# deepsphere/deepsphere-cosmo-tf2

Hardware: AMD Instinct MI355X
Metric: Mpix*channels/s Chebyshev-conv fwd, nside=1024 K=5 F=64; HBM roofline % (higher is better)
Workload: dtype f32 (recurrence f32; contraction 3-pass split-bf16 MFMA with f32 accumulate; precision 'bf16x3' = the layer default for 64 input channels)

## Files before the change

deepsphere-cosmo-tf2_amd/csrc/cheb_fused.hip:

```cpp
#include <stdio.h>
#include <stdlib.h>
#include <string.h>

#include <algorithm>

#include "cheb_istrip_kernel.h"
#include "cheb_tiles.h"

namespace dsph {

void fused_images_begin(const dsph_plan* plan, const void* ws, uint64_t key, bool keep) {
  FusedPlan* fp = plan->fused;
  if (!fp || !ws) return;
  std::lock_guard<std::mutex> lock(fp->img_mu);
  if (fp->images.size() > 16384 && fp->images.find(ws) == fp->images.end()) fp->images.clear();
  FusedPlan::Images& im = fp->images[ws];
  if (!keep || im.key != key) { im.key = key; im.mask = 0; }
}
bool fused_images_claim(const dsph_plan* plan, const void* ws, uint32_t bit) {
  FusedPlan* fp = plan->fused;
  if (!fp || !ws) return true;
  std::lock_guard<std::mutex> lock(fp->img_mu);
  auto it = fp->images.find(ws);
  if (it == fp->images.end()) return true;
  if (it->second.mask & bit) return false;
  it->second.mask |= bit;
  return true;
}
void fused_images_forget(const dsph_plan* plan, const void* ws) {
  FusedPlan* fp = plan->fused;
  if (!fp || !ws) return;
  std::lock_guard<std::mutex> lock(fp->img_mu);
  fp->images.erase(ws);
}
uint64_t fused_images_key(int32_t Fin, int32_t Fin_w, int32_t Fout, int32_t K, int32_t ld, int32_t precision, bool cheb, bool many, bool pack) {
  return ((uint64_t)(Fin & 0xfff)) | ((uint64_t)(Fin_w & 0xfff) << 12) | ((uint64_t)(Fout & 0xff) << 24) | ((uint64_t)(K & 0x3f) << 32) |
         ((uint64_t)(ld & 0xffff) << 38) | ((uint64_t)(precision & 3) << 54) | ((uint64_t)cheb << 56) | ((uint64_t)many << 57) |
         ((uint64_t)pack << 58) | (1ull << 63);
}

static bool side_stream_ready(const dsph_plan* plan, FusedPlan* fp, hipStream_t caller, bool may_create) {
  if (fp->side) return true;
  if (fp->side_failed || !may_create) return false;
  if (caller != nullptr) {
    hipStreamCaptureStatus cs = hipStreamCaptureStatusNone;
    if (hipStreamIsCapturing(caller, &cs) != hipSuccess || cs != hipStreamCaptureStatusNone) return false;
  }
  DeviceGuard guard(plan->device);
  hipStream_t st = nullptr;
  hipEvent_t e0 = nullptr, e1 = nullptr;
  if (!guard.ok || hipStreamCreateWithFlags(&st, hipStreamNonBlocking) != hipSuccess) { fp->side_failed = true; return false; }
  if (hipEventCreateWithFlags(&e0, hipEventDisableTiming) != hipSuccess ||
      hipEventCreateWithFlags(&e1, hipEventDisableTiming) != hipSuccess) {
    if (e0) (void)hipEventDestroy(e0);
    (void)hipStreamDestroy(st);
    fp->side_failed = true;
    return false;
  }
  fp->ev_fork = e0;
  fp->ev_join = e1;
  fp->side = st;
  return true;
}

static int plane_rows_for(int rmax, int emax, int wt) {
  if (rmax <= 576 && emax <= 512) return 576;
  if (rmax <= 768 && emax <= 768) return 768;
  if (rmax <= 928 && emax <= 928) return 928;
  if (rmax <= 1024 && emax <= 1024) return 1024;
  return (rmax <= 1168 && emax <= 1024 && wt == 9) ? 1168 : 0;
}

static int bfs_packs(int32_t Fin, int32_t Fout) { return Fin == 4 && Fout <= 16 ? 4 : (Fin == 8 && Fout <= 32 ? 2 : 0); }

struct WeightImages {
  size_t bfs = 0, structured, strip, istrip, qstrip, qstrip8, total;
  size_t bfs_bytes;
  WeightImages(int32_t Fin, int32_t Fout, int32_t K) {
    const int C = (Fin + FUSED_CH - 1) / FUSED_CH, NB = bfs_packs(Fin, Fout) ? 2 : (Fout + 31) / 32;
    bfs_bytes = (size_t)K * C * NB * 2048;
    structured = bfs + bfs_bytes;
    strip = structured + struct_wfrag_bytes(Fin, Fout, K);
    istrip = strip + strip_wimg_bytes(Fin, Fout, K);
    qstrip = istrip + 2 * istrip_wimg_bytes(K, DSPH_PREC_BF16X6);
    qstrip8 = qstrip + (qstrip_shape_ok(Fin, Fout, K) ? qstrip_wimg_bytes() : 0);
    total = qstrip8 + (qstrip8_shape_ok(Fin, Fout, K) ? qstrip8_wimg_bytes() : 0);
  }
};

struct LayerWorkspace {
  size_t block, padded_x, total;
  LayerWorkspace(const dsph_plan* plan, int64_t N, int32_t Fin, int32_t Fout, int32_t K) {
    const int32_t Fp = pad4(Fin);
    block = WeightImages(Fp, std::min(Fout, 64), K).total;
    padded_x = (size_t)((Fout + 63) / 64) * block;
    total = padded_x + (Fp != Fin ? (size_t)N * (size_t)plan->n_cols * (size_t)Fp * 4 : 0);
  }
};
size_t fused_workspace_bytes(const dsph_plan* plan, int64_t N, int32_t Fin, int32_t Fout, int32_t K, int32_t) {
  return LayerWorkspace(plan, N, Fin, Fout, K).total;
}

static bool want_full(const dsph_plan* plan, int32_t Fin, bool full) {
  return full || (uint64_t)plan->n_cols * (uint64_t)Fin * 4ull >= (1ull << 32);
}
static bool has_struct_tiles(const FusedTiles& ft) { return ft.r.n + ft.t.tiles.n > 0; }

static const FusedTiles* tiles_for(const dsph_plan* plan, int32_t Fin, int32_t Fout, int32_t K, bool full) {
  if (!plan->fused || plan->fused->wide) return nullptr;
  if (K < 2 || K - 1 > FUSED_DMAX) return nullptr;
  if (Fin % 4 != 0 || Fin < 4 || Fout < 1) return nullptr;
  const FusedTiles& ft = get_tiles(plan, K - 1, want_full(plan, Fin, full));
  if (!ft.ok) return nullptr;
  if (has_struct_tiles(ft) && !struct_shape_ok(Fin, std::min(Fout, 64), K)) return nullptr;
  if (ft.part.n == 0) return &ft;
  const int pr = plane_rows_for(ft.rmax, ft.emax, ft.width);
  if (pr == 0) return nullptr;
  return (size_t)2 * pr * FUSED_CH * 4 + FUSED_BIAS_BYTES <= (size_t)LDS_BYTES ? &ft : nullptr;
}

int fused_dmax() { return FUSED_DMAX; }
int fused_num_cu(const dsph_plan* plan) { return plan->fused ? plan->fused->num_cu : 256; }

bool fused_tstep_tables(const dsph_plan* plan, TStepTables* out) {
  if (!plan->fused || !plan->fused->wide || plan->n_cols != plan->n_rows || !plan->levels.empty()) return false;
  const FusedTiles& ft = get_tiles(plan, 1, true);
  if (!ft.ok || ft.rmax > 768 || ft.part.n != ft.ntiles) return false;
  out->tile_off = ft.d_tile_off;
  out->ring_end = ft.d_ring_end;
  out->ell_off = ft.d_ell_off;
  out->region = ft.d_region;
  out->lcols = ft.d_lcols;
  out->lvals = ft.d_lvals;
  out->ntiles = ft.ntiles;
  out->width = ft.width;
  return true;
}

bool fused_supported(const dsph_plan* plan, int32_t Fin, int32_t Fout, int32_t K) {
  return Fin >= 1 && tiles_for(plan, pad4(Fin), Fout, K, false) != nullptr;
}

bool fused_weights_resident(const dsph_plan* plan, int32_t Fin, int32_t Fout, int32_t K) {
  const FusedTiles* ft = Fin >= 1 ? tiles_for(plan, pad4(Fin), Fout, K, false) : nullptr;
  if (!ft) return false;
  if (ft->part.n == 0) return true;
  const int pr = plane_rows_for(ft->rmax, ft->emax, ft->width);
  return (size_t)2 * pr * FUSED_CH * 4 + WeightImages(pad4(Fin), std::min(Fout, 64), K).bfs_bytes + FUSED_BIAS_BYTES <= (size_t)LDS_BYTES;
}

int fused_prepare(const dsph_plan* plan, int32_t K, int32_t Fin, int32_t flags) {
  FusedPlan* fp = plan->fused;
  if (fp && fp->wide) {
    TStepTables tb;
    if (K >= 2) (void)fused_tstep_tables(plan, &tb);
  } else {
    if (!fp || K < 2 || K - 1 > FUSED_DMAX) return DSPH_OK;
    const FusedTiles& ftp = get_tiles(plan, K - 1, want_full(plan, pad4(std::max(Fin, 1)), false));
    if (ftp.ok && plan->opt.fork && has_struct_tiles(ftp) && ftp.part.n > 0) {
      std::lock_guard<std::mutex> lock(fp->fork_mu);
      (void)side_stream_ready(plan, fp, nullptr, true);
    }
    if (flags & DSPH_PREPARE_BACKWARD) {
      (void)get_tiles(plan, K - 1, true);
      (void)fused_symmetric(plan);
    }
  }
  if (flags & DSPH_PREPARE_RELEASE_HOST) {
    std::lock_guard<std::mutex> lock(fp->mu);
    std::vector<int32_t>().swap(fp->h_cols);
    std::vector<float>().swap(fp->h_vals);
    fp->host_released = true;
  }
  return DSPH_OK;
}


enum class Mode { forward, planes, wgrad };
enum class Strips { none, pairs, quad, input };

struct FusedRequest {
  Mode mode = Mode::forward;
  int64_t N = 1;
  int32_t Fin = 0;
  int32_t Fin_w = 0;
  int32_t Fout = 0;
  int32_t ld = 0;
  int32_t K = 0, precision = DSPH_PREC_BF16X3, act = DSPH_ACT_NONE, part = 0;
  float alpha_rest = 2.f, beta_rest = 1.f;
  const FusedPool* pool = nullptr;
  const TileList* only_tiles = nullptr;
  const dsph_plan* plan = nullptr;
  const float* x = nullptr; const float* w = nullptr; const float* bias = nullptr; float* y = nullptr;
  unsigned char* ws = nullptr;
  hipStream_t stream = nullptr;
};

struct Route {
  const FusedTiles& ft;
  bool has_struct, has_bfs;
  Strips strips;
  bool run_strips;
  const TileList* r;
  const TileTables* t;
  bool q8;
  const int32_t* bfs_tiles;
  int bfs_n;
  int pack;
  int pr;
};

static bool use_qstrips(const dsph_plan* plan, const FusedTiles& ft, const FusedRequest& q) {
  return plan->opt.strip_form == 0 && ft.q5.n > 0 && qstrip_shape_ok(q.Fin, q.Fout, q.K);
}
static bool strips_apply(const dsph_plan* plan, const FusedTiles& ft, const FusedRequest& q, bool quad) {
  if (!((quad || ft.n_pairs > 0) && (q.precision == DSPH_PREC_BF16X3 || (q.precision == DSPH_PREC_F16X3 && quad)) &&
        strip_shape_ok(q.Fin, q.Fout, q.K) && q.ld % 4 == 0 && plan->n_cols * (int64_t)std::max(q.Fin, q.ld) * 4 < (1ll << 32)))
    return false;
  if (ft.strip_forced) return true;
  FusedPlan* fp = plan->fused;
  const int64_t N = q.N;
  if (quad) {
    if (N < 1) return false;
    const int64_t span = qstrip_split(fp->num_cu, ft.q5.tape_rows, N, ft.q5.tape_rows / std::max(1, ft.q5.n), nullptr, nullptr, nullptr);
    return span * 28 * 103 < ft.q5.n_tiles * N * 187 / fp->num_cu * 100;
  }
  const std::vector<int32_t>& steps = ft.strip_steps;
  if (N < 1 || (int64_t)steps.size() * N > (1ll << 24)) return false;
  int64_t span;
  {
    std::lock_guard<std::mutex> lock(fp->mu);
    auto it = ft.strip_span.find(N);
    if (it == ft.strip_span.end()) it = ft.strip_span.emplace(N, strip_makespan(steps, N, fp->num_cu)).first;
    span = it->second;
  }
  return span * 30 * 103 < ft.n_strip_tiles * N * 187 / fp->num_cu * 100;
}

static bool q8_applies(const dsph_plan* plan, const FusedTiles& ft, const FusedRequest& q) {
  if (ft.q8.n == 0 || !qstrip8_shape_ok(q.Fin, q.Fout, q.K) || (q.precision != DSPH_PREC_BF16X3 && q.precision != DSPH_PREC_F16X3) ||
      q.ld != q.Fout || q.N < 1)
    return false;
  if (plan->opt.strips == 1) return true;
  const int64_t span = qstrip8_split(plan->fused->num_cu, ft.q8.tape_rows, q.N, ft.q8.tape_rows / std::max(1, ft.q8.n), nullptr, nullptr, nullptr);
  return span * 26 * 103 < ft.q8.n_tiles * q.N * 275 / plan->fused->num_cu * 100;
}

static bool istrips_apply(const dsph_plan* plan, const FusedTiles& ft, const FusedRequest& q) {
  return ft.n_ipairs > 0 && plan->opt.strips != 2 && istrip_shape_ok(q.Fin, q.K) && q.Fout % 4 == 0 && q.ld % 4 == 0;
}
static int istrip_nseg(const dsph_plan* plan, const FusedTiles& ft, int64_t N, int D, bool narrow) {
  FusedPlan* fp = plan->fused;
  std::lock_guard<std::mutex> lock(fp->mu);
  const int64_t key = 2 * N + (narrow ? 1 : 0);
  auto it = ft.iseg.find(key);
  if (it == ft.iseg.end()) it = ft.iseg.emplace(key, istrip_segments(ft.ipair_h, ft.ipair_second, N, fp->num_cu, D, narrow)).first;
  return it->second;
}

static Route make_route(const dsph_plan* plan, const FusedTiles& ft, const FusedRequest& q, bool forked) {
  const bool fwd = q.mode == Mode::forward, y_aligned = (reinterpret_cast<uintptr_t>(q.y) & 15) == 0;
  const bool plain_epilogue = q.act == DSPH_ACT_NONE || q.act == DSPH_ACT_RELU;
  Route rt{ft};
  rt.has_struct = fwd && has_struct_tiles(ft);
  rt.has_bfs = ft.part.count(q.part) > 0;
  const bool quad = use_qstrips(plan, ft, q);
  rt.strips = Strips::none;
  if (fwd && strips_apply(plan, ft, q, quad) && q.Fin_w == q.Fin && y_aligned) rt.strips = quad ? Strips::quad : Strips::pairs;
  else if (fwd && istrips_apply(plan, ft, q) && y_aligned) rt.strips = Strips::input;
  rt.run_strips = rt.strips != Strips::none && q.part != 2;
  rt.r = rt.strips == Strips::quad ? &ft.qrrest : (rt.strips != Strips::none ? &ft.rrest : &ft.r);
  rt.t = rt.strips == Strips::quad ? &ft.qt : &ft.t;
  rt.q8 = fwd && q.part != 2 && !q.pool && !forked && q.Fin_w == q.Fin && q.beta_rest != 0.f && plain_epilogue && y_aligned && q8_applies(plan, ft, q);
  rt.bfs_tiles = q.part == 0 && ft.part.n == ft.ntiles ? nullptr : ft.part.ptr(q.part);
  rt.bfs_n = ft.part.count(q.part);
  if (rt.q8) {
    rt.bfs_tiles = ft.q8rest.ptr(q.part);
    rt.bfs_n = ft.q8rest.count(q.part);
  }
  if (q.only_tiles) {
    rt.bfs_tiles = q.only_tiles->d;
    rt.bfs_n = q.only_tiles->n;
  }
  rt.pack = (plan->opt.pack && fwd && q.N >= 2) ? bfs_packs(q.Fin, q.Fout) : 0;
  rt.pr = plane_rows_for(ft.rmax, ft.emax, ft.width);
  return rt;
}

bool fused_pool_ok(const dsph_plan* plan, int64_t N, int32_t Fin, int32_t Fout, int32_t K, int32_t act) {
  if (!plan->fused || N < 1 || !(act == DSPH_ACT_NONE || act == DSPH_ACT_RELU)) return false;
  if (!plan->levels.empty() || plan->n_cols != plan->n_rows || plan->n_rows % FUSED_P != 0 || K < 2 || K - 1 > FUSED_DMAX) return false;
  const FusedTiles* ft = Fin >= 1 ? tiles_for(plan, pad4(Fin), Fout, K, false) : nullptr;
  if (!ft || Fout % 4 != 0) return false;
  FusedRequest q;
  q.N = N; q.Fin = q.Fin_w = pad4(Fin); q.Fout = std::min(Fout, 64); q.ld = Fout; q.K = K; q.precision = DSPH_PREC_BF16X3;
  const Strips s = make_route(plan, *ft, q, false).strips;
  return s != Strips::pairs && s != Strips::quad;
}

int64_t fused_strip_tiles(const dsph_plan* plan, int64_t N, int32_t Fin, int32_t Fout, int32_t K, int32_t precision) {
  if (!plan->fused || K < 2 || K - 1 > FUSED_DMAX) return 0;
  const FusedTiles& ft = get_tiles(plan, K - 1, want_full(plan, pad4(Fin), false));
  if (!ft.ok) return 0;
  FusedRequest q;
  q.N = N; q.Fin = pad4(Fin); q.Fin_w = Fin; q.Fout = std::min(Fout, 64); q.ld = Fout; q.K = K; q.precision = precision;
  const Route rt = make_route(plan, ft, q, false);
  if (rt.q8) return ft.q8.n_tiles;
  return rt.strips == Strips::quad ? ft.q5.n_tiles : (rt.strips != Strips::none ? ft.n_strip_tiles : 0);
}


__global__ __launch_bounds__(256) void fused_pad_kernel(const float* __restrict__ x, float4* __restrict__ out, int64_t rows,
                                                        int Fin, int Q) {
  for (int64_t i = (int64_t)blockIdx.x * 256 + threadIdx.x; i < rows * Q; i += (int64_t)gridDim.x * 256) {
    const int64_t r = i / Q;
    const int c = 4 * (int)(i - r * Q);
    const float* __restrict__ src = x + r * Fin + c;
    float4 v;
    v.x = src[0];
    v.y = c + 1 < Fin ? src[1] : 0.f;
    v.z = c + 2 < Fin ? src[2] : 0.f;
    v.w = c + 3 < Fin ? src[3] : 0.f;
    out[i] = v;
  }
}

__global__ __launch_bounds__(256) void fused_wprep_kernel(const float* __restrict__ w,
                                                          unsigned char* __restrict__ out, int Fin,
                                                          int Fout, int K, int C, int NB, int prec, int ld, int pack) {
  const int blk = blockIdx.x;
  const int nb = blk % NB, c = (blk / NB) % C, k = blk / (NB * C);
  for (int e = threadIdx.x; e < WF_ELEMS; e += 256) {
    const WfElem p = wf_elem32(e);
    wf_put(out + (size_t)blk * 2 * WF_FRAG, prec == DSPH_PREC_BF16X3 ? WF_BF16X3 : WF_FP32_STEPS, p.l, p.j,
           wf_gather_pack(w, c * FUSED_CH + p.inner, 32 * nb + p.col, Fin, Fout, K, k, ld, pack));
  }
}

__global__ __launch_bounds__(256) void fused_wgrad_reduce_kernel(const float* __restrict__ slabs, float* __restrict__ dw,
                                                                 int nslabs, int Fin, int Fout, int K, int C, int ld, int mirror_grid) {
  __shared__ float part[16][17];
  const int el = threadIdx.x & 15, p = threadIdx.x >> 4;
  const int e = blockIdx.x * 16 + el;
  const bool live = e < Fin * K * Fout;
  const int o = live ? e % Fout : 0, fk = live ? e / Fout : 0, k = fk % K, f = fk / K;
  const size_t slab = (size_t)C * K * 16 * 64;
  const size_t off = ((size_t)((f >> 4) * K + k) * 16 + (f & 15)) * 64 + o;
  float s = 0.f;
  if (live)
    for (int i = p; i < nslabs; i += 16) {
      const float v = slabs[(size_t)i * slab + off];
      s += (mirror_grid > 0 && (((i >> 1) % mirror_grid) & 1)) ? -v : v;
    }
  part[p][el] = s;
  __syncthreads();
  if (p == 0 && live) {
    float v[16];
#pragma unroll
    for (int q = 0; q < 16; ++q) v[q] = part[q][el];
#pragma unroll
    for (int h = 8; h >= 1; h >>= 1)
#pragma unroll
      for (int q = 0; q < h; ++q) v[q] += v[q + h];
    dw[(size_t)fk * ld + o] = v[0];
  }
}

int launch_fused_pad(const float* x, float* xp, int64_t rows, int32_t Fin, int32_t Fp, hipStream_t stream) {
  const int64_t work = rows * (Fp / 4);
  hipLaunchKernelGGL(fused_pad_kernel, dim3((unsigned)std::min<int64_t>((work + 255) / 256, 65536)), dim3(256), 0, stream, x,
                     reinterpret_cast<float4*>(xp), rows, (int)Fin, (int)(Fp / 4));
  DSPH_HIP(hipGetLastError());
  return DSPH_OK;
}


static int32_t struct_arithmetic(int32_t precision) { return precision == DSPH_PREC_F16X3 ? DSPH_PREC_BF16X6 : precision; }
static int32_t bfs_arithmetic(int32_t precision) {
  return struct_arithmetic(precision) == DSPH_PREC_BF16X6 ? DSPH_PREC_FP32 : precision;
}

static int check_request(const FusedRequest& rq, const FusedTiles* ft, size_t ws_bytes, size_t ws_need, const void* out) {
  if (!ft) {
    set_error("cheb_fused: plan/shape not supported");
    return DSPH_E_UNSUPPORTED;
  }
  if (ws_need > 0 && (!rq.ws || ws_bytes < ws_need)) {
    set_error("cheb_fused: workspace %zu < %zu", ws_bytes, ws_need);
    return DSPH_E_WORKSPACE;
  }
  if ((reinterpret_cast<uintptr_t>(rq.x) & 15) || (reinterpret_cast<uintptr_t>(rq.ws) & 15) || (reinterpret_cast<uintptr_t>(out) & 15)) {
    set_error("cheb_fused: x, workspace and planes must be 16-byte aligned");
    return DSPH_E_BADARG;
  }
  return DSPH_OK;
}

static LaunchBase launch_base(const FusedRequest& rq) {
  LaunchBase b;
  b.x = rq.x; b.w = rq.w; b.bias = rq.bias; b.y = rq.y;
  b.gvals8 = rq.plan->fused->d_gvals8;
  b.gdiag = rq.plan->fused->d_gdiag;
  b.x_rows = rq.plan->n_cols; b.y_rows = out_rows(rq.plan); b.N = rq.N;
  b.act = rq.act; b.ld = rq.ld; b.num_cu = rq.plan->fused->num_cu;
  b.cheb = rq.beta_rest != 0.f;
  if (rq.pool != nullptr) {
    b.pool = rq.pool->type;
    b.ypool = rq.pool->y;
    b.ypool_rows = rq.plan->n_rows / 4;
  }
  return b;
}

static int launch_strips(const FusedRequest& rq, const Route& rt, const WeightImages& img, const LaunchBase& base) {
  const dsph_plan* plan = rq.plan;
  const FusedTiles& ft = rt.ft;
  if (rt.strips == Strips::quad) {
    QStripLaunch qs;
    static_cast<LaunchBase&>(qs) = base;
    qs.wimg = rq.ws + img.qstrip;
    qs.strips = ft.q5.d_strips;
    qs.tab = ft.q5.d_tab;
    qs.prefix = ft.q5.d_prefix;
    qs.tape_rows = ft.q5.tape_rows;
    qs.nstrips = ft.q5.n; qs.Fin = rq.Fin; qs.Fout = rq.Fout;
    qs.f16 = rq.precision == DSPH_PREC_F16X3;
    qs.f16_xexp = plan->opt.f16_xexp;
    qs.prep_weights = fused_images_claim(plan, rq.ws, IMG_QSTRIP);
    return launch_cheb_qstrip(qs, rq.stream);
  }
  if (rt.strips == Strips::pairs) {
    StripLaunch st;
    static_cast<LaunchBase&>(st) = base;
    st.wimg = rq.ws + img.strip;
    st.pairs = ft.d_pairs;
    st.npairs = ft.n_pairs; st.Fin = rq.Fin; st.Fout = rq.Fout; st.K = rq.K; st.precision = struct_arithmetic(rq.precision);
    st.prep_weights = fused_images_claim(plan, rq.ws, IMG_STRIP);
    return launch_cheb_strip(st, rq.stream);
  }
  IStripLaunch is;
  static_cast<LaunchBase&>(is) = base;
  is.wimg = rq.ws + img.istrip;
  is.pairs = ft.d_ipairs;
  is.npairs = ft.n_ipairs; is.Fin = rq.Fin; is.Fin_w = rq.Fin_w; is.Fout = rq.Fout; is.K = rq.K; is.precision = struct_arithmetic(rq.precision);
  is.nseg = istrip_nseg(plan, ft, istrip_pairs(rq.Fin_w, rq.Fout) ? (rq.N + 1) / 2 : rq.N, rq.K - 1, istrip_narrow(rq.Fin_w));
  is.prep_weights = fused_images_claim(plan, rq.ws, IMG_ISTRIP);
  return launch_cheb_istrip(is, rq.stream);
}

static int forward_structured(const FusedRequest& rq, const Route& rt, const WeightImages& img) {
  const dsph_plan* plan = rq.plan;
  const LaunchBase base = launch_base(rq);
  if (rt.run_strips) {
    const int rc = launch_strips(rq, rt, img, base);
    if (rc != DSPH_OK) return rc;
  }
  StructLaunch sl;
  static_cast<LaunchBase&>(sl) = base;
  sl.wfrag = rq.ws + img.structured;
  sl.Fin = rq.Fin; sl.Fin_w = rq.Fin_w; sl.Fout = rq.Fout; sl.K = rq.K; sl.precision = struct_arithmetic(rq.precision);
  sl.allow_pack = plan->opt.pack;
  bool struct_prep = true;
  if (rt.r->count(rq.part) > 0) {
    sl.tiles = rt.r->ptr(rq.part);
    sl.ntiles = rt.r->count(rq.part);
    sl.prep_weights = fused_images_claim(plan, rq.ws, IMG_STRUCT);
    struct_prep = false;
    const int rc = launch_cheb_struct(sl, rq.stream);
    if (rc != DSPH_OK) return rc;
  }
  if (rt.t->tiles.count(rq.part) > 0) {
    sl.tiles = rt.t->tiles.ptr(rq.part);
    sl.tabrow = rt.t->rows(rq.part);
    sl.tabvals = rt.t->vals(rq.part);
    sl.ntiles = rt.t->tiles.count(rq.part);
    sl.prep_weights = struct_prep && fused_images_claim(plan, rq.ws, IMG_STRUCT);
    const int rc = launch_cheb_struct(sl, rq.stream);
    if (rc != DSPH_OK) return rc;
  }
  return DSPH_OK;
}

static int fused_grid(const dsph_plan* plan, int ntiles) { return std::max(8, std::min(plan->fused->num_cu, (ntiles + 7) / 8 * 8)); }

static FusedArgs fused_args(const FusedRequest& rq, const Route& rt) {
  const dsph_plan* plan = rq.plan;
  const FusedTiles& ft = rt.ft;
  const int C = (rq.Fin + FUSED_CH - 1) / FUSED_CH;
  FusedArgs args{};
  args.c_count = C;
  args.prow_stride = plan->n_cols;
  args.plane_stride = rq.N * plan->n_cols * (int64_t)rq.Fin;
  args.x = rq.x;
  args.bias = rq.bias;
  args.y = rq.y;
  args.wfrag = rq.ws;
  args.tile_off = ft.d_tile_off;
  args.ring_end = ft.d_ring_end;
  args.ell_off = ft.d_ell_off;
  args.region = ft.d_region;
  args.lcols = ft.d_lcols;
  args.lvals = ft.d_lvals;
  args.x_rows = plan->n_cols;
  args.y_rows = out_rows(plan);
  args.N = rt.pack ? (int)((rq.N + rt.pack - 1) / rt.pack) : (int)rq.N;
  args.n_maps = (int)rq.N;
  args.pack = rt.pack;
  args.num_cu = plan->fused->num_cu;
  args.pool = rq.pool ? rq.pool->type : 0;
  args.ypool = rq.pool ? rq.pool->y : nullptr;
  args.ypool_rows = plan->n_rows / 4;
  args.Fin = rq.Fin;
  args.Fout = rq.Fout;
  args.ld = rq.ld;
  args.K = rq.K;
  args.tile_list = rt.bfs_tiles;
  args.ntiles = rt.bfs_n;
  args.nchunks = C;
  args.act = rq.act;
  args.alpha_rest = rq.alpha_rest;
  args.beta_rest = rq.beta_rest;
  return args;
}

static int launch_fused_variant(int pr, int wt, const FusedArgs& a, int nb, int prec, int grid, size_t lds, hipStream_t stream) {
#define DSPH_FUSED_CASE(PR, WT) \
  if (pr == PR && wt == WT) return launch_fused_##PR##_##WT(a, nb, prec, grid, lds, stream);
  DSPH_FUSED_CASE(576, 9)
  DSPH_FUSED_CASE(768, 9)
  DSPH_FUSED_CASE(928, 9)
  DSPH_FUSED_CASE(1024, 9)
  DSPH_FUSED_CASE(1168, 9)
  DSPH_FUSED_CASE(576, 12)
  DSPH_FUSED_CASE(768, 12)
  DSPH_FUSED_CASE(928, 12)
  DSPH_FUSED_CASE(1024, 12)
#undef DSPH_FUSED_CASE
  set_error("cheb_fused: no kernel for plane rows %d, width %d", pr, wt);
  return DSPH_E_UNSUPPORTED;
}

static int launch_bfs_tiles(const FusedRequest& rq, const Route& rt, FusedArgs& args, int nb, size_t wfrag_bytes) {
  if (args.ntiles == 0) return DSPH_OK;
  args.wfrag_bytes = (int)wfrag_bytes;
  const size_t lds = (size_t)2 * rt.pr * FUSED_CH * 4 + wfrag_bytes;
  return launch_fused_variant(rt.pr, rt.ft.width, args, nb, bfs_arithmetic(rq.precision), fused_grid(rq.plan, args.ntiles), lds, rq.stream);
}

static int forward_bfs(const FusedRequest& rq, const Route& rt, const WeightImages& img) {
  const dsph_plan* plan = rq.plan;
  const int C = (rq.Fin + FUSED_CH - 1) / FUSED_CH;
  const int NB = rt.pack ? 2 : (rq.Fout + 31) / 32;
  if (fused_images_claim(plan, rq.ws, IMG_BFS)) {
    hipLaunchKernelGGL(fused_wprep_kernel, dim3(rq.K * C * NB), dim3(256), 0, rq.stream, rq.w, rq.ws + img.bfs, (int)rq.Fin_w, (int)rq.Fout,
                       (int)rq.K, C, NB, (int)bfs_arithmetic(rq.precision), (int)rq.ld, rt.pack);
    DSPH_HIP(hipGetLastError());
  }
  if (rt.q8) {
    QStrip8Launch q;
    static_cast<LaunchBase&>(q) = launch_base(rq);
    q.wimg = rq.ws + img.qstrip8;
    q.strips = rt.ft.q8.d_strips; q.tab = rt.ft.q8.d_tab; q.prefix = rt.ft.q8.d_prefix; q.tape_rows = rt.ft.q8.tape_rows;
    q.nstrips = rt.ft.q8.n; q.ld_w = rq.ld;
    q.f16 = rq.precision == DSPH_PREC_F16X3;
    q.f16_xexp = plan->opt.f16_xexp;
    q.prep_weights = fused_images_claim(plan, rq.ws, IMG_Q8);
    const int rc = launch_cheb_qstrip8(q, rq.stream);
    if (rc != DSPH_OK) return rc;
  }
  FusedArgs args = fused_args(rq, rt);
  return launch_bfs_tiles(rq, rt, args, NB, img.bfs_bytes);
}

static int forward_block(const FusedRequest& rq, const FusedTiles* ft, size_t ws_bytes) {
  const WeightImages img(rq.Fin, rq.Fout, rq.K);
  const int rc = check_request(rq, ft, ws_bytes, img.total, nullptr);
  if (rc != DSPH_OK) return rc;
  const Route rt = make_route(rq.plan, *ft, rq, false);
  if (rt.has_struct) {
    const int rc_s = forward_structured(rq, rt, img);
// ... 251 lines not shown
```

deepsphere-cosmo-tf2_amd/csrc/cheb_qstrip.hip:

```cpp
#include <math.h>
#include <stdio.h>
#include <stdlib.h>

#include <algorithm>
#include <vector>

#include "cheb_qstrip_kernel.h"
#include "dsphere_wfrag.h"

namespace dsph {

__global__ __launch_bounds__(256) void qstrip_wprep_kernel(const float* __restrict__ w, unsigned char* __restrict__ out, int Fin,
                                                           int Fout, int cheb, int ld, int f16) {
  constexpr int K = 5;
  const int blk = blockIdx.x;
  const int kb = blk & 1, lev = (blk >> 1) % 3, oq = ((blk >> 1) / 3) & 3, role = (blk >> 1) / 12;
  const int j = role == 0 ? K - 1 - lev : 1 - lev;
  const bool have = role == 0 || lev < 2;
  float sc = qs_wsign(cheb != 0, j) * ((cheb != 0 && j == 0) ? 2.f : 1.f);
  if (f16) {
    const float pw = qt_wimg_pow2(w, Fin * K, Fout, ld);
    sc *= pw;
    if (blk == 0 && threadIdx.x == 0) *reinterpret_cast<float*>(out + (size_t)2 * 4 * 3 * 2 * 2 * QS_FRAG) = 1.f / pw;
  }
  unsigned char* base = out + (size_t)blk * 2 * QS_FRAG;
  for (int e = threadIdx.x; e < WF_ELEMS; e += 256) {
    const WfElem p = wf_elem16(e);
    wf_put(base, f16 ? WF_F16X3 : WF_BF16X3, p.l, p.j, have ? wf_gather(w, 32 * kb + p.inner, 16 * oq + p.col, Fin, Fout, K, j, ld, sc) : 0.f);
  }
}

bool qstrip_shape_ok(int32_t Fin, int32_t Fout, int32_t K) { return K == 5 && Fin == 64 && Fout == 64; }

int64_t qtape_split(int num_cu, int64_t tape_rows, int64_t N, int64_t mean_height, int run_in, int* grid, int* pieces, int* wg_per_piece) {
  const int g = (int)std::max<int64_t>(8, std::min<int64_t>(num_cu / 8 * 8, tape_rows * N / 64 / 8 * 8));
  auto span_of = [&](int64_t w) {
    const int64_t P = std::max<int64_t>(1, g / w), share = (tape_rows + P - 1) / P, maps = (N + w - 1) / w;
    const int64_t runs = share / std::max<int64_t>(1, mean_height) + 2;
    return (share + runs * (run_in + 1)) * maps;
  };
  int64_t best_w = 1, best = -1;
  if (N <= g) { best_w = N; best = span_of(N); }
  else
    for (int64_t w = 1; w <= g; w *= 2) {
      const int64_t sp = span_of(w);
      if (best < 0 || sp < best) { best = sp; best_w = w; }
    }
  if (grid) *grid = g;
  if (pieces) *pieces = (int)std::max<int64_t>(1, g / best_w);
  if (wg_per_piece) *wg_per_piece = (int)best_w;
  return best;
}
int64_t qstrip_split(int num_cu, int64_t tape_rows, int64_t N, int64_t mean_height, int* grid, int* pieces, int* wg_per_piece) {
  return qtape_split(num_cu, tape_rows, N, mean_height, QS_RUNIN, grid, pieces, wg_per_piece);
}

size_t qstrip_wimg_bytes() { return (size_t)2 * 4 * 3 * 2 * 2 * QS_FRAG + 256; }

int launch_cheb_qstrip(const QStripLaunch& s, hipStream_t stream) {
  if (s.prep_weights) {
    hipLaunchKernelGGL(qstrip_wprep_kernel, dim3(2 * 4 * 3 * 2), dim3(256), 0, stream, s.w, s.wimg, (int)s.Fin, (int)s.Fout, s.cheb ? 1 : 0,
                       (int)s.ld, s.f16 ? 1 : 0);
    DSPH_HIP(hipGetLastError());
  }
  QStripArgs a;
  a.Fin = s.Fin;
  a.Fout = s.Fout;
  const int grid = qtape_forward_args(a, s, QS_RUNIN);
  void (*kern)(QStripArgs) = s.f16 ? (s.cheb ? cheb_qstrip5_kernel<true, true> : cheb_qstrip5_kernel<false, true>)
                                   : (s.cheb ? cheb_qstrip5_kernel<true, false> : cheb_qstrip5_kernel<false, false>);
#ifdef DSPH_QS_STAMPS
  static unsigned* d_stamps = nullptr;
  constexpr size_t NST = 8 * 4 * 10;
  if (!d_stamps) DSPH_HIP(hipMalloc(&d_stamps, NST * 4));
  DSPH_HIP(hipMemsetAsync(d_stamps, 0, NST * 4, stream));
  a.stamps = d_stamps;
#endif
  hipLaunchKernelGGL(kern, dim3(grid), dim3(QS_THREADS), 0, stream, a);
  DSPH_HIP(hipGetLastError());
#ifdef DSPH_QS_STAMPS
  if (getenv("DSPH_STAMPS_DUMP")) {
    std::vector<unsigned> h(NST);
    if (hipStreamSynchronize(stream) == hipSuccess && hipMemcpy(h.data(), d_stamps, NST * 4, hipMemcpyDeviceToHost) == hipSuccess)
      for (int w = 0; w < 8; ++w)
        for (int it = 0; it < 4; ++it) {
          const unsigned* r = &h[((size_t)w * 4 + it) * 10];
          fprintf(stderr, "QSSTAMP wave %d step %2d:", w, it);
          unsigned prev = r[0];
          for (int i = 1; i <= 8; ++i) {
            if (r[i] == 0) { fprintf(stderr, "      -"); continue; }
            fprintf(stderr, " %6u", r[i] - prev);
            prev = r[i];
          }
          fprintf(stderr, " | step %u | t0 %u\n", r[8] - r[0], r[0]);
        }
  }
#endif
  return DSPH_OK;
}

}
```

deepsphere-cosmo-tf2_amd/csrc/cheb_qstrip_kernel.h:

```cpp
#pragma once

#include <type_traits>

#include "cheb_qtape.h"

namespace dsph {

constexpr int QS_PX = 64;
constexpr int QS_D = 4;
constexpr int QS_USE = QS_PX - 2 * QS_D;
constexpr int QS_THREADS = 512;
constexpr int QS_RUNIN = 2 * QS_D + 1;

struct QStripArgs {
  const float* x;
  const float* bias;
  float* y;
  const unsigned char* wimg;
  const float* gvals8;
  const float* gdiag;
  const QStrip* strips;
  const int32_t* tab;
  const int32_t* prefix;
  int64_t x_rows, y_rows;
  int nstrips, N, Fin, Fout, ld, act;
  int pieces, wg_per_piece;
  float xsc, xsc_inv;
#ifdef DSPH_QS_STAMPS
  unsigned* stamps;
#endif
};

#ifdef DSPH_QS_STAMPS
#define QS_STAMP(id)                                                                                          \
  do {                                                                                                        \
    if (stamp_on) {                                                                                           \
      unsigned long long t_;                                                                                  \
      asm volatile("s_memtime %0\n\ts_waitcnt lgkmcnt(0)" : "=s"(t_)::"memory");                              \
      if (lane == 0) a.stamps[(wave * 4 + (stamp_step & 3)) * 10 + (id)] = (unsigned)t_;                      \
    }                                                                                                         \
  } while (0)
#define QS_STAMP_DECL                                                                                         \
  const int stamp_step = ytop - (st.y0 - D) - 60;                                                             \
  const bool stamp_on = blockIdx.x == 72 && stamp_step >= 0 && stamp_step < 4;
#else
#define QS_STAMP(id)
#define QS_STAMP_DECL
#endif

#ifdef DSPH_QS_ABL
#define QS_ABL DSPH_QS_ABL
#else
#define QS_ABL 0
#endif

#if QS_ABL & 64
#define QS_FD "v_fmac_f32_e32 "
#define QS_DPPL "\n\t"
#define QS_DPPR "\n\t"
#else
#define QS_FD "v_fmac_f32_dpp "
#define QS_DPPL " row_shr:1 row_mask:0xf bank_mask:0xf bound_ctrl:1\n\t"
#define QS_DPPR " row_shl:1 row_mask:0xf bank_mask:0xf bound_ctrl:1\n\t"
#endif

template <bool F16> __device__ __forceinline__ void qs_m(qs_f4& acc, const qs_bf8& wa, const qs_bf8& bb) {
  if (QS_ABL & 2) { asm volatile("" : "+v"(acc) : "v"(wa), "v"(bb) : "memory"); return; }
  if (F16) asm volatile("v_mfma_f32_16x16x32_f16 %0, %1, %2, %0" : "+v"(acc) : "v"(wa), "v"(bb) : "memory");
  else asm volatile("v_mfma_f32_16x16x32_bf16 %0, %1, %2, %0" : "+v"(acc) : "v"(wa), "v"(bb) : "memory");
}
template <bool F16> __device__ __forceinline__ void qs_m0(qs_f4& acc, const qs_bf8& wa, const qs_bf8& bb) {
  if (QS_ABL & 2) { acc = qs_f4{0.f, 0.f, 0.f, 0.f}; asm volatile("" : "+v"(acc) : "v"(wa), "v"(bb) : "memory"); return; }
  if (F16) asm volatile("v_mfma_f32_16x16x32_f16 %0, %1, %2, 0" : "=&v"(acc) : "v"(wa), "v"(bb) : "memory");
  else asm volatile("v_mfma_f32_16x16x32_bf16 %0, %1, %2, 0" : "=&v"(acc) : "v"(wa), "v"(bb) : "memory");
}
template <int N> __device__ __forceinline__ void qs_settle(QRow& r) {
  if (N == 9) asm volatile("s_nop 9" : "+v"(r.t[0]), "+v"(r.t[1]), "+v"(r.t[2]), "+v"(r.t[3]) : : "memory");
  else asm volatile("s_nop 1" : "+v"(r.t[0]), "+v"(r.t[1]), "+v"(r.t[2]), "+v"(r.t[3]) : : "memory");
}

template <bool INIT, bool NEG>
__device__ __forceinline__ void qs_u12(float& a0, float& a1, float& a2, float& a3, float s0, float s1, float s2, float s3,
                                       const qs_f4& cw, const qs_f4& cc, const qs_f4& ce) {
  if ((QS_ABL & 64) && NEG) { qs_u12<INIT, false>(a0, a1, a2, a3, s0, s1, s2, s3, cw, cc, ce); return; }
  const float w0 = cw[0], w1 = cw[1], w2 = cw[2], w3 = cw[3], c0 = cc[0], c1 = cc[1], c2 = cc[2], c3 = cc[3], e0 = ce[0], e1 = ce[1],
              e2 = ce[2], e3 = ce[3];
#define QS_OPS_IN "v"(s0), "v"(s1), "v"(s2), "v"(s3), "v"(w0), "v"(w1), "v"(w2), "v"(w3), "v"(c0), "v"(c1), "v"(c2), "v"(c3), "v"(e0), "v"(e1), "v"(e2), "v"(e3)
  if (!INIT && !NEG)
    asm volatile(
        "v_fmac_f32_e32 %0, %4, %12\n\tv_fmac_f32_e32 %1, %5, %13\n\tv_fmac_f32_e32 %2, %6, %14\n\tv_fmac_f32_e32 %3, %7, %15\n\t"
        "v_fmac_f32_e32 %1, %4, %9\n\tv_fmac_f32_e32 %2, %5, %10\n\tv_fmac_f32_e32 %3, %6, %11\n\t"
        "v_fmac_f32_e32 %0, %5, %16\n\tv_fmac_f32_e32 %1, %6, %17\n\tv_fmac_f32_e32 %2, %7, %18\n\t"
        QS_FD "%0, %7, %8" QS_DPPL QS_FD "%3, %4, %19" QS_DPPR
        : "+v"(a0), "+v"(a1), "+v"(a2), "+v"(a3)
        : QS_OPS_IN
        : "memory");
  else if (!INIT && NEG)
    asm volatile(
        "v_fma_f32 %0, %4, -%12, %0\n\tv_fma_f32 %1, %5, -%13, %1\n\tv_fma_f32 %2, %6, -%14, %2\n\tv_fma_f32 %3, %7, -%15, %3\n\t"
        "v_fma_f32 %1, %4, -%9, %1\n\tv_fma_f32 %2, %5, -%10, %2\n\tv_fma_f32 %3, %6, -%11, %3\n\t"
        "v_fma_f32 %0, %5, -%16, %0\n\tv_fma_f32 %1, %6, -%17, %1\n\tv_fma_f32 %2, %7, -%18, %2\n\t"
        QS_FD "%0, %7, -%8" QS_DPPL QS_FD "%3, %4, -%19" QS_DPPR
        : "+v"(a0), "+v"(a1), "+v"(a2), "+v"(a3)
        : QS_OPS_IN
        : "memory");
  else if (INIT && !NEG)
    asm volatile(
        "v_mul_f32_e32 %0, %4, %12\n\tv_mul_f32_e32 %1, %5, %13\n\tv_mul_f32_e32 %2, %6, %14\n\tv_mul_f32_e32 %3, %7, %15\n\t"
        "v_fmac_f32_e32 %1, %4, %9\n\tv_fmac_f32_e32 %2, %5, %10\n\tv_fmac_f32_e32 %3, %6, %11\n\t"
        "v_fmac_f32_e32 %0, %5, %16\n\tv_fmac_f32_e32 %1, %6, %17\n\tv_fmac_f32_e32 %2, %7, %18\n\t"
        QS_FD "%0, %7, %8" QS_DPPL QS_FD "%3, %4, %19" QS_DPPR
        : "=&v"(a0), "=&v"(a1), "=&v"(a2), "=&v"(a3)
        : QS_OPS_IN
        : "memory");
  else
    asm volatile(
        "v_mul_f32_e64 %0, %4, -%12\n\tv_mul_f32_e64 %1, %5, -%13\n\tv_mul_f32_e64 %2, %6, -%14\n\tv_mul_f32_e64 %3, %7, -%15\n\t"
        "v_fma_f32 %1, %4, -%9, %1\n\tv_fma_f32 %2, %5, -%10, %2\n\tv_fma_f32 %3, %6, -%11, %3\n\t"
        "v_fma_f32 %0, %5, -%16, %0\n\tv_fma_f32 %1, %6, -%17, %1\n\tv_fma_f32 %2, %7, -%18, %2\n\t"
        QS_FD "%0, %7, -%8" QS_DPPL QS_FD "%3, %4, -%19" QS_DPPR
        : "=&v"(a0), "=&v"(a1), "=&v"(a2), "=&v"(a3)
        : QS_OPS_IN
        : "memory");
#undef QS_OPS_IN
}
template <bool INIT, bool NEG>
__device__ __forceinline__ void qs_unit(QRow& acc, const QRow& src, int e, const qs_f4& cw, const qs_f4& cc, const qs_f4& ce) {
  if ((QS_ABL & 4) && !INIT) {
    asm volatile("" : "+v"(acc.t[0]), "+v"(acc.t[1]), "+v"(acc.t[2]), "+v"(acc.t[3]) : "v"(src.t[0]), "v"(src.t[3]), "v"(cw), "v"(cc), "v"(ce) : "memory");
    return;
  }
#define QS_UE(E)                                                                                                          \
  {                                                                                                                       \
    float a0 = 0.f, a1 = 0.f, a2 = 0.f, a3 = 0.f;                                                                         \
    if (!INIT) { a0 = acc.t[0][E]; a1 = acc.t[1][E]; a2 = acc.t[2][E]; a3 = acc.t[3][E]; }                                \
    qs_u12<INIT, NEG>(a0, a1, a2, a3, src.t[0][E], src.t[1][E], src.t[2][E], src.t[3][E], cw, cc, ce);                    \
    acc.t[0][E] = a0; acc.t[1][E] = a1; acc.t[2][E] = a2; acc.t[3][E] = a3;                                               \
  }
  if (e == 0) QS_UE(0)
  else if (e == 1) QS_UE(1)
  else if (e == 2) QS_UE(2)
  else QS_UE(3)
#undef QS_UE
}

#define QS_UPR 4
#define QS_UNIT qs_unit

__host__ __device__ constexpr float qs_wsign(bool cheb, int j) { return cheb && ((j & 3) >= 2) ? -1.f : 1.f; }

template <bool CHEB, bool F16>
__global__ __launch_bounds__(QS_THREADS, 2) void cheb_qstrip5_kernel(QStripArgs a) {
  constexpr int K = 5, D = QS_D, RING = K + 2;
#ifdef DSPH_QS_NOH1
  constexpr bool H1 = false;
#else
  constexpr bool H1 = CHEB;
#endif
  constexpr int ROWB = 2 * 2 * 4 * QS_FRAG;
  constexpr int RINGB = RING * ROWB;
  constexpr int HAND1 = 2 * 4 * QS_FRAG;
  constexpr int HANDB = 4 * HAND1;
  constexpr int CRING = K + 1;
  constexpr int CRINGB = CRING * QS_CROWB;
  constexpr int LDS_HAND = RINGB, LDS_C = RINGB + HANDB, LDS_FLAG = LDS_C + CRINGB;
  __shared__ __attribute__((aligned(16))) unsigned char smem[LDS_FLAG + 64];

  const int tid = threadIdx.x, lane = tid & 63;
  const int wave = __builtin_amdgcn_readfirstlane(tid >> 6);
  const bool roleL = wave >= 4;
  const int oq = wave & 3;
  const int p = lane & 15, q4 = lane >> 4;
  const unsigned lane16 = (unsigned)lane * 16u;
  const unsigned hand = (unsigned)LDS_HAND + (unsigned)oq * HAND1 + lane16;
  const unsigned flag_addr = (unsigned)LDS_FLAG + 4u * (unsigned)oq;
  auto flag_set = [&](int v) __attribute__((always_inline)) { qt_flag_set(flag_addr, v); };
  auto flag_get = [&]() __attribute__((always_inline)) -> int { return qt_flag_get(flag_addr); };
  for (int i = tid; i < (LDS_FLAG + 64) / 16; i += QS_THREADS) reinterpret_cast<qs_f4*>(smem)[i] = qs_f4{0.f, 0.f, 0.f, 0.f};

  const QTapePiece wg = qt_piece(a.wg_per_piece);
  if (wg.piece >= a.pieces) return;
  const QTapeRange tape = qt_tape_range(a.prefix, a.nstrips, wg.piece, a.pieces);
  auto locate = [&](int64_t r, int64_t r_end, QStrip& st) __attribute__((always_inline)) -> int {
    return qt_locate(a.prefix, a.strips, a.nstrips, r, r_end, st);
  };
  const unsigned xrowb = (unsigned)a.Fin * 4u, yrowb = (unsigned)a.ld * 4u;

#if defined(DSPH_QS_XALL)
  constexpr bool X_BY_H = false;
#elif defined(DSPH_QS_XBYH)
  constexpr bool X_BY_H = true;
#else
  constexpr bool X_BY_H = !H1;
#endif
  constexpr int XN = X_BY_H ? 4 : 2;
  const int xt = wave & 3, xpix = X_BY_H ? ((lane >> 1) & 15) : (((lane >> 1) & 7) + 8 * (wave >> 2));
  const unsigned x_goff = X_BY_H ? (unsigned)(2 * (lane >> 5) + (lane & 1)) * 16u
                                 : (unsigned)(lane >> 5) * 64u + (unsigned)(2 * ((lane >> 4) & 1) + (lane & 1)) * 16u;
  const unsigned x_loff = (unsigned)xt * QS_FRAG + (unsigned)(lane & 1) * 8u +
                          (X_BY_H ? (unsigned)(xpix + 16 * (lane >> 5)) * 16u : (unsigned)(xpix + 16 * (2 * (lane >> 5) + ((lane >> 4) & 1))) * 16u);
  auto tab_lane = [&](const QStrip& st, unsigned ci, int yrow) __attribute__((always_inline)) -> unsigned {
    return qt_tab_lane(a.tab, st, ci, min(max(yrow, st.ylo), st.yhi));
  };
  auto my_of = [&](int yrow) __attribute__((always_inline)) -> unsigned { return st_spread((unsigned)yrow & 15u) << 1; };
  auto my_next = [&](unsigned m) __attribute__((always_inline)) -> unsigned { return ((m | 0x55u) + 1u) & 0xaau; };
  auto xfetch = [&](const char* xmap, unsigned xrow, qs_f4 (&xv)[XN]) __attribute__((always_inline)) {
    if (QS_ABL & 8) {
#pragma unroll
      for (int i = 0; i < XN; ++i) xv[i] = qs_f4{0.f, 0.f, 0.f, 0.f};
      return;
    }
    const char* src = xmap + (size_t)(xrow * xrowb + x_goff);
#pragma unroll
    for (int i = 0; i < XN; ++i) xv[i] = *reinterpret_cast<const qs_f4*>(src + (X_BY_H ? 64 : 128) * i);
  };
  auto xw_wait = [&](qs_f4 (&xv)[XN]) __attribute__((always_inline)) {
    if (X_BY_H) asm volatile("" : "+v"(xv[0]), "+v"(xv[1]), "+v"(xv[XN - 2]), "+v"(xv[XN - 1]) : : "memory");
    else asm volatile("" : "+v"(xv[0]), "+v"(xv[1]) : : "memory");
  };
  auto xstore = [&](int slot, const qs_f4 (&xv)[XN]) __attribute__((always_inline)) {
    if (QS_ABL & 4096) {
#pragma unroll
      for (int i = 0; i < XN; ++i) asm volatile("" : : "v"(xv[i]));
      return;
    }
    unsigned char* q = smem + (unsigned)slot * ROWB + x_loff;
#pragma unroll
    for (int i = 0; i < XN; ++i) {
      const unsigned fo = X_BY_H ? (unsigned)(i >> 1) * (2 * 4 * QS_FRAG) + (unsigned)(i & 1) * (32u * 16u) : (unsigned)i * (2 * 4 * QS_FRAG);
      qs_u2 hi, lo;
#pragma unroll
      for (int j = 0; j < 2; ++j) {
        const float a0 = F16 ? xv[i][2 * j] * a.xsc : xv[i][2 * j], a1 = F16 ? xv[i][2 * j + 1] * a.xsc : xv[i][2 * j + 1];
        const qs_u2 hl = qt_split<F16>(a0, a1);
        hi[j] = hl[0];
        lo[j] = hl[1];
      }
      *reinterpret_cast<qs_u2*>(q + fo) = hi;
      *reinterpret_cast<qs_u2*>(q + fo + 4 * QS_FRAG) = lo;
    }
  };
  auto cfetch = [&](unsigned rid, qs_f4& cv, float& cd) __attribute__((always_inline)) { qt_cfetch(a.gvals8, a.gdiag, rid, q4, cv, cd); };
  auto cw_wait = [&](qs_f4& cv, float& cd) __attribute__((always_inline)) {
    asm volatile("" : "+v"(cv), "+v"(cd) : : "memory");
  };
  auto cstore = [&](int slot, qs_f4 cv, float cd) __attribute__((always_inline)) {
    if (CHEB) { cv = cv + cv; cd = cd + cd; }
    unsigned char* q = smem + LDS_C + (unsigned)slot * QS_CROWB + (unsigned)p * 16u + (unsigned)oq * 4u;
    if (q4 < 2) {
#pragma unroll
      for (int d = 0; d < 4; ++d) *reinterpret_cast<float*>(q + (unsigned)(1 + 4 * q4 + d) * 256u) = cv[d];
    }
    if (q4 == 2) *reinterpret_cast<float*>(q) = cd;
  };
  constexpr bool C_OFF = (QS_ABL & 1024) != 0;
  auto clo_read = [&](int slot) __attribute__((always_inline)) -> QCoefLo { return qt_clo_read<C_OFF>(smem + LDS_C, slot, p); };
  auto chi_read = [&](int slot) __attribute__((always_inline)) -> QCoefHi { return qt_chi_read<C_OFF>(smem + LDS_C, slot, p); };

#if QS_ABL & 512
#define QS_FRLOAD(P) (wr[0][0][0])
#else
#define QS_FRLOAD(P) (*reinterpret_cast<const qs_bf8*>(P))
#endif
#define QS_ORD_A(j) ((j) == 1 ? 1 : 0)
#define QS_ORD_B(j) ((j) == 0 ? 1 : 0)
#define QS_FR0(FADDR)                                                                                                     \
  _Pragma("unroll") for (int u = 0; u < 2; ++u) {                                                                         \
    fr[0][u][0] = QS_FRLOAD(smem + (FADDR) + (unsigned)u * QS_FRAG);                                                      \
    fr[0][u][1] = QS_FRLOAD(smem + (FADDR) + (unsigned)(4 + u) * QS_FRAG);                                                \
  }
#define QS_SETS(S0, S1, ROW, ZERO, WLEV, FADDR, NU, ...)                                                                  \
  _Pragma("unroll") for (int s = (S0); s < (S1); ++s) {                 \
    if (s + 1 < 4) {                                                                                                      \
      _Pragma("unroll") for (int u = 0; u < 2; ++u) {                                                                     \
        const unsigned fo = (unsigned)(((s + 1) >> 1) * 8 + ((s + 1) & 1) * 2 + u) * QS_FRAG;                             \
        fr[(s + 1) & 1][u][0] = QS_FRLOAD(smem + (FADDR) + fo);                                                           \
        fr[(s + 1) & 1][u][1] = QS_FRLOAD(smem + (FADDR) + fo + 4 * QS_FRAG);                                             \
      }                                                                                                                   \
    }                                                                                                                     \
    _Pragma("unroll") for (int j = 0; j < 3; ++j) {                                                                       \
      _Pragma("unroll") for (int u = 0; u < 2; ++u) {                                                                     \
        const int m = (s * 3 + j) * 2 + u;                                                                                \
        const int tt = (s & 1) * 2 + u;                                                                                   \
        const qs_bf8& wa_ = wr[WLEV][s >> 1][QS_ORD_A(j)];                                                                \
        const qs_bf8& bb_ = fr[s & 1][u][QS_ORD_B(j)];                                                                    \
        if ((ZERO) && s < 2 && j == 0) qs_m0<F16>((ROW).t[tt], wa_, bb_);                                                 \
        else qs_m<F16>((ROW).t[tt], wa_, bb_);                                                                            \
        _Pragma("unroll") for (int qq = (m * (NU)) / 18; qq < ((m + 1) * (NU)) / 18 && m < 18; ++qq) { __VA_ARGS__; }     \
      }                                                                                                                   \
    }                                                                                                                     \
  }
#define QS_CHAIN(ROW, ZERO, WLEV, FADDR, NU, TAIL, ...)                                                                   \
  {                                                                                                                       \
    QS_SETS(0, 3, ROW, ZERO, WLEV, FADDR, NU, __VA_ARGS__)                                                                \
    TAIL;                                                                                                                 \
    QS_SETS(3, 4, ROW, ZERO, WLEV, FADDR, NU, __VA_ARGS__)                                                                \
  }

  __syncthreads();

  if (!roleL) {
    qs_bf8 wr[4][2][2];
    if (H1) {
      const unsigned char* wp1 = a.wimg + ((size_t)(1 * 4 + oq) * 3) * (2 * 2 * QS_FRAG) + lane16;
#pragma unroll
      for (int kb = 0; kb < 2; ++kb)
#pragma unroll
        for (int h = 0; h < 2; ++h) wr[3][kb][h] = *reinterpret_cast<const qs_bf8*>(wp1 + (size_t)(kb * 2 + h) * QS_FRAG);
    }
    {
      const unsigned char* wp = a.wimg + ((size_t)(0 * 4 + oq) * 3) * (2 * 2 * QS_FRAG) + lane16;
#pragma unroll
      for (int l = 0; l < 3; ++l)
#pragma unroll
        for (int kb = 0; kb < 2; ++kb)
#pragma unroll
          for (int h = 0; h < 2; ++h) wr[l][kb][h] = *reinterpret_cast<const qs_bf8*>(wp + ((size_t)(l * 2 + kb) * 2 + h) * QS_FRAG);
    }
    int handed = 0;
    for (int64_t tr = tape.begin; tr < tape.end;) {
      QStrip st;
      tr += locate(tr, tape.end, st);
      for (int nq = wg.map0; nq < a.N; nq += a.wg_per_piece) {
      const int Xc = min(max(st.xs + 4 * p + oq, st.xlo), st.xhi);
      const int Xf = min(max(st.xs + 4 * xpix + xt, st.xlo), st.xhi);
      const int tc0 = max(st.xs, st.xlo) >> 4;
      const unsigned ciC = (unsigned)((Xc >> 4) - tc0), mXc = st_spread((unsigned)Xc & 15u);
      const unsigned ciF = (unsigned)((Xf >> 4) - tc0), mXf = st_spread((unsigned)Xf & 15u);
      const int T3 = ((st.y1 - st.y0) + 2 * D + 1 + 3) / 3;
      const char* __restrict__ xmap = reinterpret_cast<const char*>(a.x) + (size_t)nq * a.x_rows * xrowb;
      QRow R[2][3];
#pragma unroll
      for (int i = 0; i < 2; ++i)
#pragma unroll
        for (int s = 0; s < 3; ++s)
#pragma unroll
          for (int t = 0; t < 4; ++t) R[i][s].t[t] = qs_f4{0.f, 0.f, 0.f, 0.f};
      int ytop = st.y0 - D, slot_top = 0, cs_top = 0;
      qt_step_barrier();
      {
        qs_f4 cv, xv[XN];
        float cd;
        cfetch(qt_row_in(st, tab_lane(st, ciC, ytop - 1), mXc, ytop - 1), cv, cd);
        xfetch(xmap, qt_row_in(st, tab_lane(st, ciF, ytop), mXf, ytop), xv);
        cw_wait(cv, cd);
        cstore(CRING - 1, cv, cd);
        xw_wait(xv);
        xstore(0, xv);
      }
      unsigned bXf = tab_lane(st, ciF, ytop + 1), bXc = tab_lane(st, ciC, ytop);
      unsigned myX = my_of(ytop + 1), myC = my_of(ytop);
      qt_step_barrier();
      auto step = [&](auto ph_c) __attribute__((always_inline)) {
        constexpr int PH = decltype(ph_c)::value;
        constexpr int L0 = PH % 3, L1 = (PH + 1) % 3, L2 = (PH + 2) % 3;
        int snew = slot_top + 1;
        snew = snew == RING ? 0 : snew;
        auto slot_ix = [&](int back) __attribute__((always_inline)) -> int {
          int s = slot_top - back;
          s += s < 0 ? RING : 0;
          return s;
        };
        auto cslot_ix = [&](int back) __attribute__((always_inline)) -> int {
          int s = cs_top - back;
          s += s < 0 ? CRING : 0;
          return s;
        };
        QS_STAMP_DECL
        QS_STAMP(0);
        qs_f4 xv[XN];
        constexpr bool XLATE = H1;
        if (myX == 0) bXf = tab_lane(st, ciF, ytop + 1);
        if (myC == 0) bXc = tab_lane(st, ciC, ytop);
        if (!XLATE) xfetch(xmap, bXf + (mXf | myX), xv);
        const unsigned f0 = (unsigned)slot_top * ROWB + lane16, f1 = (unsigned)slot_ix(1) * ROWB + lane16, f2 = (unsigned)slot_ix(2) * ROWB + lane16;
        const unsigned f3 = (unsigned)slot_ix(3) * ROWB + lane16;
        constexpr bool N3 = CHEB;
        qs_bf8 fr[2][2][2];
        QCoefLo c3 = clo_read(cslot_ix(1));
        QS_FR0(f0)
        QCoefLo c2;
        QCoefHi c3h, c2h;
        qs_f4 cv;
        float cd;
        QS_CHAIN(R[0][L2], true, 0, f0, 2 * QS_UPR, { c2 = clo_read(cslot_ix(2)); QS_FR0(f1) },
                 { if (qq < QS_UPR) QS_UNIT<true, N3>(R[1][L2], R[0][L0], qq, QS_LO0(c3)); else QS_UNIT<false, N3>(R[1][L2], R[0][L1], qq - QS_UPR, QS_LO1(c3)); })
        qs_settle<9>(R[0][L2]);
        qs_settle<1>(R[1][L2]);
        QS_STAMP(1);
        QS_CHAIN(R[1][L2], false, 1, f1, 2 * QS_UPR, { c3h = chi_read(cslot_ix(1)); QS_FR0(f2) },
                 { if (qq < QS_UPR) QS_UNIT<!CHEB, false>(R[0][L0], R[1][L0], qq, QS_LO0(c2)); else QS_UNIT<false, false>(R[0][L0], R[1][L1], qq - QS_UPR, QS_LO1(c2)); })
        qs_settle<9>(R[1][L2]);
        qs_settle<1>(R[0][L0]);
        if (XLATE) xfetch(xmap, bXf + (mXf | myX), xv);
        QS_STAMP(2);
        QS_CHAIN(R[0][L0], false, 2, f2, QS_UPR, { c2h = chi_read(cslot_ix(2)); cfetch(bXc + (mXc | myC), cv, cd); if (H1) { QS_FR0(f3) } },
                 { QS_UNIT<false, N3>(R[1][L2], R[0][L2], qq, QS_HI(c3h)); })
        qs_settle<9>(R[0][L0]);
        qs_settle<1>(R[1][L2]);
        QS_STAMP(3);
        if (H1) {
          QS_CHAIN(R[1][L0], false, 3, f3, QS_UPR, {}, { QS_UNIT<false, false>(R[0][L0], R[1][L2], qq, QS_HI(c2h)); })
          qs_settle<9>(R[1][L0]);
        } else {
#pragma unroll
          for (int qq = 0; qq < QS_UPR; ++qq) QS_UNIT<false, false>(R[0][L0], R[1][L2], qq, QS_HI(c2h));
        }
        QS_STAMP(4);
        for (int spin = 0; flag_get() <= handed && spin < (1 << 22); ++spin) {}
        if (!(QS_ABL & 2048)) {
          unsigned char* hp = smem + hand;
#pragma unroll
          for (int t = 0; t < 4; ++t) {
            *reinterpret_cast<qs_f4*>(hp + t * QS_FRAG) = R[0][L0].t[t];
            if (CHEB) *reinterpret_cast<qs_f4*>(hp + (4 + t) * QS_FRAG) = R[1][L0].t[t];
          }
        }
        ++handed;
        QS_STAMP(5);
        xw_wait(xv);
        cw_wait(cv, cd);
        QS_STAMP(6);
        cstore(cs_top, cv, cd);
        xstore(snew, xv);
        QS_STAMP(7);
        slot_top = snew;
        cs_top = cs_top + 1 == CRING ? 0 : cs_top + 1;
        ++ytop;
        myX = my_next(myX);
        myC = my_next(myC);
        qt_step_barrier();
        QS_STAMP(8);
      };
      for (int t3 = 0; t3 < T3; ++t3) {
        step(std::integral_constant<int, 0>{});
        step(std::integral_constant<int, 1>{});
        step(std::integral_constant<int, 2>{});
      }
      }
    }
  } else {
    qs_bf8 wr[2][2][2];
    {
      const unsigned char* wp = a.wimg + ((size_t)(1 * 4 + oq) * 3) * (2 * 2 * QS_FRAG) + lane16;
#pragma unroll
      for (int l = 0; l < 2; ++l)
#pragma unroll
        for (int kb = 0; kb < 2; ++kb)
#pragma unroll
          for (int h = 0; h < 2; ++h) wr[l][kb][h] = *reinterpret_cast<const qs_bf8*>(wp + ((size_t)(l * 2 + kb) * 2 + h) * QS_FRAG);
    }
    const float floor_v = a.act == DSPH_ACT_RELU ? 0.f : -__builtin_huge_valf();
    const float ysc = (CHEB ? 0.5f : 1.f) * (F16 ? *reinterpret_cast<const float*>(a.wimg + 2 * 4 * 3 * 2 * 2 * QS_FRAG) * a.xsc_inv : 1.f);
#ifdef DSPH_QS_LPRIO
#define QS_STR2(x) #x
#define QS_STR(x) QS_STR2(x)
    asm volatile("s_setprio " QS_STR(DSPH_QS_LPRIO));
#endif
    qs_f4 bv = qs_f4{0.f, 0.f, 0.f, 0.f};
    if (a.bias != nullptr) bv = *reinterpret_cast<const qs_f4*>(a.bias + 16 * oq + 4 * q4);
    int taken = 0;
    for (int64_t tr = tape.begin; tr < tape.end;) {
      QStrip st;
      tr += locate(tr, tape.end, st);
      for (int nq = wg.map0; nq < a.N; nq += a.wg_per_piece) {
      const int Xf = min(max(st.xs + 4 * xpix + xt, st.xlo), st.xhi);
      const int tc0 = max(st.xs, st.xlo) >> 4;
      const unsigned ciF = (unsigned)((Xf >> 4) - tc0), mXf = st_spread((unsigned)Xf & 15u);
      const int Xg = st.xs + 4 * p;
      const unsigned ciY = (unsigned)((min(max(Xg, st.xlo), st.xhi) >> 4) - tc0), mXg = st_spread((unsigned)Xg & 12u);
      const int cfirst = st.x0 - st.xs, clast = cfirst + st.w;
      const int T3 = ((st.y1 - st.y0) + 2 * D + 1 + 3) / 3;
      const char* __restrict__ xmap = reinterpret_cast<const char*>(a.x) + (size_t)nq * a.x_rows * xrowb;
      char* __restrict__ ymap = reinterpret_cast<char*>(a.y) + (size_t)nq * a.y_rows * yrowb;
      QRow R[2][3], Y;
#pragma unroll
      for (int i = 0; i < 2; ++i)
#pragma unroll
        for (int s = 0; s < 3; ++s)
#pragma unroll
          for (int t = 0; t < 4; ++t) R[i][s].t[t] = qs_f4{0.f, 0.f, 0.f, 0.f};
#pragma unroll
      for (int t = 0; t < 4; ++t) Y.t[t] = qs_f4{0.f, 0.f, 0.f, 0.f};
      int ytop = st.y0 - D, slot_top = 0, cs_top = 0;
      qt_step_barrier();
      if (!X_BY_H) {
        qs_f4 xv[XN];
        xfetch(xmap, qt_row_in(st, tab_lane(st, ciF, ytop), mXf, ytop), xv);
        xw_wait(xv);
        xstore(0, xv);
      }
      unsigned bXf = X_BY_H ? 0u : tab_lane(st, ciF, ytop + 1), bY = tab_lane(st, ciY, st.y0);
      unsigned myX = my_of(ytop + 1), myY = my_of(ytop - K);
      qt_step_barrier();
      auto step = [&](auto ph_c) __attribute__((always_inline)) {
        constexpr int PH = decltype(ph_c)::value;
        constexpr int L0 = PH % 3, L1 = (PH + 1) % 3, L2 = (PH + 2) % 3;
        int snew = slot_top + 1;
        snew = snew == RING ? 0 : snew;
        auto slot_ix = [&](int back) __attribute__((always_inline)) -> int {
          int s = slot_top - back;
          s += s < 0 ? RING : 0;
          return s;
        };
        auto cslot_ix = [&](int back) __attribute__((always_inline)) -> int {
          int s = cs_top - back;
          s += s < 0 ? CRING : 0;
          return s;
        };
        QS_STAMP_DECL
        QS_STAMP(0);
        qs_f4 xv[XN];
        if (!X_BY_H && myX == 0) bXf = tab_lane(st, ciF, ytop + 1);
        if (myY == 0) bY = tab_lane(st, ciY, ytop - K);
        if (!X_BY_H) xfetch(xmap, bXf + (mXf | myX), xv);
#ifdef DSPH_QS_LEARLY
        constexpr bool LE = CHEB && H1;
#else
        constexpr bool LE = false;
#endif
        QCoefLo c0;
        QCoefHi c0h;
        if (LE) c0 = clo_read(cslot_ix(5));
        if (!(QS_ABL & 2048)) {
          const unsigned char* hp = smem + hand;
#pragma unroll
          for (int t = 0; t < 4; ++t) {
            R[0][L2].t[t] = *reinterpret_cast<const qs_f4*>(hp + t * QS_FRAG);
            if (CHEB) R[1][L2].t[t] = *reinterpret_cast<const qs_f4*>(hp + (4 + t) * QS_FRAG);
          }
        }
        ++taken;
        flag_set(taken);
        const unsigned f1 = (unsigned)slot_ix(4) * ROWB + lane16, f0 = (unsigned)slot_ix(5) * ROWB + lane16;
        constexpr bool N1 = CHEB;
        QS_STAMP(1);
        qs_bf8 fr[2][2][2];
        if (LE) {
#pragma unroll
          for (int t = 0; t < 4; ++t) Y.t[t] = R[0][L0].t[t] + R[0][L0].t[t];
          qs_settle<1>(Y);
#pragma unroll
          for (int qq = 0; qq < 2 * QS_UPR; ++qq) {
            if (qq < QS_UPR) QS_UNIT<false, false>(Y, R[1][L0], qq, QS_LO0(c0)); else QS_UNIT<false, false>(Y, R[1][L1], qq - QS_UPR, QS_LO1(c0));
          }
          qs_settle<1>(Y);
        }
        const QCoefLo c1 = clo_read(cslot_ix(4));
        const QCoefHi c1h = chi_read(cslot_ix(4));
        QS_FR0(f0)
#ifdef DSPH_QS_LBARE
        if (CHEB && H1) {
          c0 = clo_read(cslot_ix(5));
          c0h = chi_read(cslot_ix(5));
#pragma unroll
          for (int qq = 0; qq < 3 * QS_UPR; ++qq) {
            if (qq < QS_UPR) QS_UNIT<false, N1>(R[1][L2], R[0][L0], qq, QS_LO0(c1));
            else if (qq < 2 * QS_UPR) QS_UNIT<false, N1>(R[1][L2], R[0][L1], qq - QS_UPR, QS_LO1(c1));
            else QS_UNIT<false, N1>(R[1][L2], R[0][L2], qq - 2 * QS_UPR, QS_HI(c1h));
          }
#pragma unroll
          for (int t = 0; t < 4; ++t) Y.t[t] = R[0][L0].t[t] + R[0][L0].t[t];
          qs_settle<1>(Y);
#pragma unroll
          for (int qq = 0; qq < 2 * QS_UPR; ++qq) {
            if (qq < QS_UPR) QS_UNIT<false, false>(Y, R[1][L0], qq, QS_LO0(c0)); else QS_UNIT<false, false>(Y, R[1][L1], qq - QS_UPR, QS_LO1(c0));
          }
          qs_settle<1>(R[1][L2]);
#pragma unroll
          for (int qq = 0; qq < QS_UPR; ++qq) QS_UNIT<false, false>(Y, R[1][L2], qq, QS_HI(c0h));
          qs_settle<1>(Y);
          QS_STAMP(2);
          QS_CHAIN(Y, false, 1, f0, 0, {}, {})
          qs_settle<9>(Y);
          QS_STAMP(3);
        } else
// ... 78 lines not shown
```

deepsphere-cosmo-tf2_amd/csrc/cheb_qtape.h:

```cpp
#pragma once

#include <algorithm>

#include "cheb_struct_kernel.h"
#include "dsphere_common.h"

namespace dsph {

constexpr int QS_FRAG = 1024;
constexpr int QS_CROWB = 2304;

typedef float qs_f4 __attribute__((ext_vector_type(4)));
typedef int qs_i4 __attribute__((ext_vector_type(4)));
typedef __bf16 qs_bf8 __attribute__((ext_vector_type(8)));
typedef unsigned qs_u2 __attribute__((ext_vector_type(2)));

struct QRow {
  qs_f4 t[4];
};

struct QStrip {
  int32_t x0, w;
  int32_t xs;
  int32_t y0, y1;
  int32_t xlo, xhi;
  int32_t ylo, yhi;
  int32_t tab, tws;
  int32_t pad[1];
};

struct QTapePiece {
  int ord, piece, map0;
};
__device__ __forceinline__ QTapePiece qt_piece(int wg_per_piece) {
  QTapePiece c;
  const int G = gridDim.x;
  c.ord = (blockIdx.x & 7) * (G >> 3) + (blockIdx.x >> 3);
  c.piece = c.ord / wg_per_piece;
  c.map0 = c.ord - c.piece * wg_per_piece;
  return c;
}
struct QTapeRange {
  int64_t begin, end;
};
__device__ __forceinline__ QTapeRange qt_tape_range(const int32_t* prefix, int nstrips, int piece, int pieces) {
  const int64_t tape = (int64_t)prefix[nstrips];
  QTapeRange r;
  r.begin = piece < pieces ? tape * piece / pieces : 0;
  r.end = piece < pieces ? tape * (piece + 1) / pieces : 0;
  return r;
}
__device__ __forceinline__ int qt_locate(const int32_t* prefix, const QStrip* strips, int nstrips, int64_t r, int64_t r_end, QStrip& st) {
  int lo = 0, hi = nstrips;
  while (hi - lo > 1) {
    const int mid = (lo + hi) >> 1;
    if ((int64_t)prefix[mid] <= r) lo = mid; else hi = mid;
  }
  {
    const QStrip g = strips[lo];
#define QS_U(f) st.f = __builtin_amdgcn_readfirstlane(g.f)
    QS_U(x0); QS_U(w); QS_U(xs); QS_U(y0); QS_U(y1); QS_U(xlo); QS_U(xhi); QS_U(ylo); QS_U(yhi); QS_U(tab); QS_U(tws);
#undef QS_U
  }
  const int h = st.y1 - st.y0;
  const int off = (int)(r - (int64_t)prefix[lo]);
  const int len = (int)(((int64_t)(h - off) < r_end - r) ? (int64_t)(h - off) : r_end - r);
  st.y0 += off;
  st.y1 = st.y0 + len;
  return len;
}

__device__ __forceinline__ unsigned qt_tab_lane(const int32_t* tab, const QStrip& st, unsigned ci, int yc) {
  const int32_t* trow = tab + __builtin_amdgcn_readfirstlane(st.tab + (yc >> 4) * st.tws + (max(st.xs, st.xlo) >> 4));
  qs_i4 b;
  int b4;
  asm volatile("s_load_dwordx4 %0, %2, 0x0\n\ts_load_dword %1, %2, 0x10\n\ts_waitcnt lgkmcnt(0)" : "=&s"(b), "=&s"(b4) : "s"(trow) : "memory");
  return (unsigned)(ci == 0 ? b[0] : ci == 1 ? b[1] : ci == 2 ? b[2] : ci == 3 ? b[3] : b4);
}
__device__ __forceinline__ unsigned qt_row_in(const QStrip& st, unsigned base, unsigned mX, int yrow) {
  const int yc = min(max(yrow, st.ylo), st.yhi);
  return base + (mX | (st_spread((unsigned)yc & 15u) << 1));
}

__device__ __forceinline__ void qt_step_barrier() { asm volatile("s_waitcnt lgkmcnt(0)\n\ts_barrier" ::: "memory"); }
__device__ __forceinline__ void qt_flag_set(unsigned addr, int v) { asm volatile("ds_write_b32 %0, %1" : : "v"(addr), "v"(v) : "memory"); }
__device__ __forceinline__ int qt_flag_get(unsigned addr) {
  int v;
  asm volatile("ds_read_b32 %0, %1\n\ts_waitcnt lgkmcnt(0)" : "=v"(v) : "v"(addr) : "memory");
  return v;
}

template <bool F16> __device__ __forceinline__ qs_u2 qt_split(float a0, float a1) {
  typedef __bf16 bf16x2 __attribute__((ext_vector_type(2)));
  typedef _Float16 f16x2 __attribute__((ext_vector_type(2)));
  typedef float f32x2 __attribute__((ext_vector_type(2)));
  qs_u2 r;
  if (F16) {
    const f16x2 h = __builtin_convertvector(f32x2{a0, a1}, f16x2);
    const f32x2 hf = __builtin_convertvector(h, f32x2);
    const f16x2 l = __builtin_convertvector(f32x2{a0 - hf[0], a1 - hf[1]}, f16x2);
    r[0] = __builtin_bit_cast(unsigned, h);
    r[1] = __builtin_bit_cast(unsigned, l);
  } else {
    const bf16x2 h = __builtin_convertvector(f32x2{a0, a1}, bf16x2);
    const unsigned hu = __builtin_bit_cast(unsigned, h);
    const float h0 = __builtin_bit_cast(float, hu << 16), h1 = __builtin_bit_cast(float, hu & 0xffff0000u);
    const bf16x2 l = __builtin_convertvector(f32x2{a0 - h0, a1 - h1}, bf16x2);
    r[0] = hu;
    r[1] = __builtin_bit_cast(unsigned, l);
  }
  return r;
}

struct QCoef3 {
  qs_f4 w, c, e;
};
struct QCoefLo {
  qs_f4 sw, s, se, w, dg, e;
};
struct QCoefHi {
  qs_f4 nw, n, ne;
};
#define QS_LO0(c) (c).sw, (c).s, (c).se
#define QS_LO1(c) (c).w, (c).dg, (c).e
#define QS_HI(c) (c).nw, (c).n, (c).ne

__device__ __forceinline__ void qt_cfetch(const float* gvals8, const float* gdiag, size_t rid, int q4, qs_f4& cv, float& cd) {
  const char* pv = reinterpret_cast<const char*>(gvals8) + rid * 32u + (unsigned)(q4 & 1) * 16u;
  const char* pd = reinterpret_cast<const char*>(gdiag) + rid * 4u;
  cv = *reinterpret_cast<const qs_f4*>(pv);
  cd = *reinterpret_cast<const float*>(pd);
}
template <bool DOUBLE>
__device__ __forceinline__ void qt_cstore(unsigned char* ring, int slot, int p, int q4, int res, qs_f4 cv, float cd) {
  if (DOUBLE) { cv = cv + cv; cd = cd + cd; }
  unsigned char* q = ring + (unsigned)slot * QS_CROWB + (unsigned)p * 16u + (unsigned)res * 4u;
  if (q4 < 2) {
#pragma unroll
    for (int d = 0; d < 4; ++d) *reinterpret_cast<float*>(q + (unsigned)(1 + 4 * q4 + d) * 256u) = cv[d];
  }
  if (q4 == 2) *reinterpret_cast<float*>(q) = cd;
}
__device__ __forceinline__ const unsigned char* qt_crow(const unsigned char* ring, int slot, int p) {
  return ring + (unsigned)slot * QS_CROWB + (unsigned)p * 16u;
}
template <bool NOREAD = false> __device__ __forceinline__ qs_f4 qt_cvec(const unsigned char* q, int v) {
  if (NOREAD) { qs_f4 c = qs_f4{0.1f, 0.1f, 0.1f, 0.1f}; asm volatile("" : "+v"(c)); return c; }
  return *reinterpret_cast<const qs_f4*>(q + (unsigned)v * 256u);
}
template <bool NOREAD = false> __device__ __forceinline__ QCoef3 qt_cvec3(const unsigned char* q, int which) {
  QCoef3 r;
  if (which == 0) { r.w = qt_cvec<NOREAD>(q, 8); r.c = qt_cvec<NOREAD>(q, 7); r.e = qt_cvec<NOREAD>(q, 6); }
  else if (which == 1) { r.w = qt_cvec<NOREAD>(q, 1); r.c = qt_cvec<NOREAD>(q, 0); r.e = qt_cvec<NOREAD>(q, 5); }
  else { r.w = qt_cvec<NOREAD>(q, 2); r.c = qt_cvec<NOREAD>(q, 3); r.e = qt_cvec<NOREAD>(q, 4); }
  return r;
}
template <bool NOREAD = false> __device__ __forceinline__ QCoefLo qt_clo_read(const unsigned char* ring, int slot, int p) {
  const unsigned char* q = qt_crow(ring, slot, p);
  QCoefLo c;
  c.sw = qt_cvec<NOREAD>(q, 8); c.s = qt_cvec<NOREAD>(q, 7); c.se = qt_cvec<NOREAD>(q, 6);
  c.w = qt_cvec<NOREAD>(q, 1); c.dg = qt_cvec<NOREAD>(q, 0); c.e = qt_cvec<NOREAD>(q, 5);
  return c;
}
template <bool NOREAD = false> __device__ __forceinline__ QCoefHi qt_chi_read(const unsigned char* ring, int slot, int p) {
  const unsigned char* q = qt_crow(ring, slot, p);
  QCoefHi c;
  c.nw = qt_cvec<NOREAD>(q, 2); c.n = qt_cvec<NOREAD>(q, 3); c.ne = qt_cvec<NOREAD>(q, 4);
  return c;
}

__device__ __forceinline__ float qt_wimg_pow2(const float* __restrict__ w, int nrows, int ncols, int ld) {
  __shared__ float smax[256];
  float m = 0.f;
  for (int e = threadIdx.x; e < nrows * ncols; e += 256) m = fmaxf(m, fabsf(w[(int64_t)(e / ncols) * ld + e % ncols]));
  smax[threadIdx.x] = m;
  __syncthreads();
  for (int st = 128; st > 0; st >>= 1) {
    if ((int)threadIdx.x < st) smax[threadIdx.x] = fmaxf(smax[threadIdx.x], smax[threadIdx.x + st]);
    __syncthreads();
  }
  int ex = 0;
  const float mx = smax[0];
  float pw = 1.f;
  if (mx > 0.f && mx < 3.0e38f) { (void)frexpf(mx, &ex); pw = ldexpf(1.f, 12 - ex); }
  return pw;
}

template <class Args, class Launch> int qtape_args(Args& a, const Launch& s, int run_in) {
  a.x = s.x;
  a.gvals8 = s.gvals8;
  a.gdiag = s.gdiag;
  a.strips = s.strips;
  a.tab = s.tab;
  a.prefix = s.prefix;
  a.x_rows = s.x_rows;
  a.nstrips = s.nstrips;
  a.N = (int)s.N;
  int grid;
  (void)qtape_split(s.num_cu, s.tape_rows, s.N, s.tape_rows / std::max(1, s.nstrips), run_in, &grid, &a.pieces, &a.wg_per_piece);
  return grid;
}
template <class Args> int qtape_forward_args(Args& a, const QTapeLaunch& s, int run_in) {
  a.bias = s.bias;
  a.y = s.y;
  a.wimg = s.wimg;
  a.y_rows = s.y_rows;
  a.ld = s.ld;
  a.act = s.act;
  a.xsc = s.f16 ? ldexpf(1.f, s.f16_xexp) : 1.f;
  a.xsc_inv = s.f16 ? ldexpf(1.f, -s.f16_xexp) : 1.f;
  return qtape_args(a, s, run_in);
}

}
```

deepsphere-cosmo-tf2_amd/csrc/cheb_tiles.h:

```cpp
#pragma once

#include <map>
#include <mutex>
#include <unordered_map>
#include <vector>

#include "cheb_fused_kernel.h"
#include "cheb_qstrip8_kernel.h"
#include "cheb_qstrip_kernel.h"
#include "cheb_strip_kernel.h"
#include "cheb_struct_kernel.h"

namespace dsph {

struct TileList {
  int32_t* d = nullptr;
  int n = 0, n_interior = 0;
  const int32_t* ptr(int part) const { return part == 2 ? d + n_interior : d; }
  int count(int part) const { return part == 0 ? n : (part == 1 ? n_interior : n - n_interior); }
};

struct TileTables {
  TileList tiles;
  int32_t* d_row = nullptr;
  float* d_vals = nullptr;
  size_t first(int part) const { return part == 2 ? (size_t)tiles.n_interior : 0; }
  const int32_t* rows(int part) const { return d_row + first(part) * ST_CELLS; }
  const float* vals(int part) const { return d_vals + first(part) * ST_CELLS * ST_TABV; }
};

struct QStripSet {
  QStrip* d_strips = nullptr;
  int32_t* d_prefix = nullptr;
  int32_t* d_tab = nullptr;
  int n = 0;
  int64_t tape_rows = 0;
  int64_t n_tiles = 0;
  std::vector<QStrip> h_strips;
  std::vector<int32_t> h_tab;
};

struct FusedTiles {
  int D = 0;
  int width = 0;
  int ntiles = 0;
  int rmax = 0;
  int emax = 0;
  bool ok = false;
  int32_t* d_tile_off = nullptr;
  int32_t* d_ring_end = nullptr;
  int64_t* d_ell_off = nullptr;
  int32_t* d_region = nullptr;
  uint16_t* d_lcols = nullptr;
  float* d_lvals = nullptr;
  TileList part;
  TileList r;
  TileTables t;
  StripPair* d_pairs = nullptr;
  int n_pairs = 0;
  int64_t n_strip_tiles = 0;
  std::vector<int32_t> strip_steps;
  std::vector<StripPair> h_pairs;
  mutable std::map<int64_t, int64_t> strip_span;
  bool strip_forced = false;
  TileList rrest;
  QStripSet q5;
  TileList qrrest;
  TileTables qt;
  QStripSet q8;
  TileList q8rest;
  StripPair* d_ipairs = nullptr;
  int n_ipairs = 0;
  std::vector<int32_t> ipair_h;
  std::vector<unsigned char> ipair_second;
  mutable std::map<int64_t, int> iseg;
  TileList all;
  TileList nonq;
  std::vector<void*> dev;
  void release();
};

struct FusedPlan {
  std::vector<int32_t> h_cols;
  std::vector<float> h_vals;
  std::mutex mu;
  std::map<int, FusedTiles> by_depth;
  int num_cu = 256;
  float* d_gvals8 = nullptr;
  float* d_gdiag = nullptr;
  unsigned char* d_rowflag = nullptr;
  bool rows_tried = false;
  bool host_released = false;
  int symmetric = -1;
  bool wide = false;
  hipStream_t side = nullptr;
  hipEvent_t ev_fork = nullptr, ev_join = nullptr;
  bool side_failed = false;
  std::mutex fork_mu;
  struct Images { uint64_t key = 0; uint32_t mask = 0; };
  std::mutex img_mu;
  std::unordered_map<const void*, Images> images;
};

const FusedTiles& get_tiles(const dsph_plan* plan, int D, bool full = false);
bool fused_symmetric(const dsph_plan* plan);
int64_t strip_makespan(const std::vector<int32_t>& steps, int64_t N, int num_cu);

}
```

deepsphere-cosmo-tf2_amd/csrc/cheb_tiles.hip:

```cpp
#include <stdio.h>
#include <stdlib.h>
#include <string.h>

#include <algorithm>
#include <initializer_list>

#include "cheb_tiles.h"

namespace dsph {

static const int ddx[8] = {-1, -1, 0, 1, 1, 1, 0, -1}, ddy[8] = {0, 1, 1, 1, 0, -1, -1, -1};

static int template_width(int w) {
  if (w <= 9) return 9;
  if (w <= 12) return 12;
  return 0;
}

void FusedTiles::release() {
  for (void* p : dev) (void)hipFree(p);
  *this = FusedTiles();
}

FusedPlan* fused_plan_build(const dsph_plan* plan, const int32_t* h_cols, const float* h_vals) {
  if (template_width(plan->width) == 0 && tstep_width(plan->width) == 0) return nullptr;
  FusedPlan* fp = new FusedPlan();
  fp->wide = template_width(plan->width) == 0;
  const size_t nnz = (size_t)plan->n_rows * plan->width;
  fp->h_cols.assign(h_cols, h_cols + nnz);
  fp->h_vals.assign(h_vals, h_vals + nnz);
  hipDeviceProp_t prop;
  if (hipGetDeviceProperties(&prop, plan->device) == hipSuccess && prop.multiProcessorCount > 0)
    fp->num_cu = prop.multiProcessorCount;
  return fp;
}

void fused_plan_destroy(FusedPlan* fp) {
  if (!fp) return;
  for (auto& kv : fp->by_depth) kv.second.release();
  if (fp->d_gvals8) (void)hipFree(fp->d_gvals8);
  if (fp->d_gdiag) (void)hipFree(fp->d_gdiag);
  if (fp->d_rowflag) (void)hipFree(fp->d_rowflag);
  if (fp->side) {
    (void)hipStreamSynchronize(fp->side);
    (void)hipEventDestroy(fp->ev_fork);
    (void)hipEventDestroy(fp->ev_join);
    (void)hipStreamDestroy(fp->side);
  }
  delete fp;
}

bool fused_host_released(FusedPlan* fp) {
  std::lock_guard<std::mutex> lock(fp->mu);
  return fp->host_released;
}

void fused_plan_invalidate(FusedPlan* fp) {
  if (!fp) return;
  std::lock_guard<std::mutex> lock(fp->mu);
  for (auto& kv : fp->by_depth) kv.second.release();
  fp->by_depth.clear();
}

static bool embed_tile(const dsph_plan* plan, const int32_t* cols, const float* vals, int W, int t, int D, int64_t out_rows,
                       int32_t* row, float* val, bool* interior, std::vector<int32_t>& key, std::vector<int32_t>& slot) {
  const int64_t r0 = (int64_t)t * FUSED_P;
  if (r0 + FUSED_P > out_rows) return false;
  constexpr int S = ST_S;
  int32_t A[S][S];
  for (int y = 0; y < S; ++y)
    for (int x = 0; x < S; ++x) A[x][y] = -1;
  constexpr int HN = 2048;
  key.assign(HN, -1);
  slot.assign(HN, 0);
  auto hput = [&](int32_t r, int cell) {
    unsigned h = ((unsigned)r * 2654435761u) >> 21;
    while (key[h] != -1) h = (h + 1) & (HN - 1);
    key[h] = r;
    slot[h] = cell;
  };
  auto hget = [&](int32_t r) -> int {
    unsigned h = ((unsigned)r * 2654435761u) >> 21;
    while (key[h] != -1) {
      if (key[h] == r) return slot[h];
      h = (h + 1) & (HN - 1);
    }
    return -1;
  };
  for (unsigned y = 0; y < 16; ++y)
    for (unsigned x = 0; x < 16; ++x) {
      const int32_t r = (int32_t)(r0 + st_morton(x, y));
      A[ST_DMAX + x][ST_DMAX + y] = r;
      hput(r, (ST_DMAX + x) + S * (ST_DMAX + y));
    }
  auto propose = [&](int x, int y) -> int32_t {
    int32_t cand[16];
    int nc = -1;
    for (int dy = -1; dy <= 1; ++dy)
      for (int dx = -1; dx <= 1; ++dx) {
        const int ax = x + dx, ay = y + dy;
        if ((dx == 0 && dy == 0) || ax < 0 || ay < 0 || ax >= S || ay >= S || A[ax][ay] < 0) continue;
        const int32_t ar = A[ax][ay];
        if (ar >= plan->n_rows) continue;
        const int32_t* c = cols + (size_t)ar * W;
        const float* v = vals + (size_t)ar * W;
        if (nc < 0) {
          nc = 0;
          for (int j = 0; j < W; ++j)
            if (v[j] != 0.f && c[j] != ar && hget(c[j]) < 0 && nc < 16) cand[nc++] = c[j];
        } else {
          int m = 0;
          for (int i = 0; i < nc; ++i) {
            bool in = false;
            for (int j = 0; j < W && !in; ++j) in = v[j] != 0.f && c[j] == cand[i];
            if (in) cand[m++] = cand[i];
          }
          nc = m;
        }
      }
    return nc == 1 ? cand[0] : (nc > 1 ? -1 : -2);
  };
  auto place = [&](int x, int y) -> bool {
    const int32_t r = propose(x, y);
    if (r == -1) return false;
    if (r == -2) { A[x][y] = -2; return true; }
    A[x][y] = r;
    hput(r, x + S * y);
    return true;
  };
  for (int rho = 1; rho <= D; ++rho) {
    const int lo = ST_DMAX - rho, hi = ST_DMAX + ST_TILE - 1 + rho;
    const int mid = (lo + hi) / 2;
    for (int k = 0; k <= hi - lo; ++k) {
      const int off = (k + 1) / 2 * ((k & 1) ? 1 : -1);
      const int u = mid + off;
      if (u <= lo || u >= hi) continue;
      if (!place(u, hi) || !place(u, lo) || !place(lo, u) || !place(hi, u)) return false;
    }
    if (!place(lo, lo) || !place(hi, lo) || !place(lo, hi) || !place(hi, hi)) return false;
  }
  const int blo = ST_DMAX - D, bhi = ST_DMAX + ST_TILE - 1 + D;
  for (int p = 0; p < ST_CELLS; ++p) {
    row[p] = (int32_t)r0;
    for (int j = 0; j < ST_TABV; ++j) val[(size_t)p * ST_TABV + j] = 0.f;
  }
  *interior = true;
  for (int y = blo; y <= bhi; ++y)
    for (int x = blo; x <= bhi; ++x) {
      const int32_t r = A[x][y];
      const unsigned p = st_cell_off((unsigned)x, (unsigned)y) / 64u;
      if (r < 0) continue;
      row[p] = r;
      if (r >= out_rows) *interior = false;
      if (x == blo || x == bhi || y == blo || y == bhi) continue;
      if (r >= plan->n_rows) return false;
      const int32_t* c = cols + (size_t)r * W;
      const float* v = vals + (size_t)r * W;
      float* o = val + (size_t)p * ST_TABV;
      unsigned seen = 0;
      for (int j = 0; j < W; ++j) {
        if (v[j] == 0.f) continue;
        int d = -1;
        if (c[j] == r) d = 0;
        else {
          const int cell = hget(c[j]);
          if (cell < 0) return false;
          const int dx = cell % S - x, dy = cell / S - y;
          for (int q = 0; q < 8; ++q)
            if (ddx[q] == dx && ddy[q] == dy) d = q + 1;
          if (d < 0) return false;
        }
        if (seen & (1u << d)) return false;
        seen |= 1u << d;
        o[d] = v[j];
      }
    }
  return true;
}

static int strip_grid(int num_cu, int64_t n_items) { return (int)std::max<int64_t>(8, std::min<int64_t>(num_cu, (n_items + 7) / 8 * 8)); }
int64_t strip_makespan(const std::vector<int32_t>& steps, int64_t N, int num_cu) {
  const int64_t Q = (int64_t)steps.size() * N;
  const int G = strip_grid(num_cu, Q);
  int64_t worst = 0;
  std::vector<int64_t> load;
  for (int xcd = 0; xcd < 8; ++xcd) {
    const int nslots = (G + 7 - xcd) / 8;
    const int64_t q0 = Q * xcd / 8, q1 = Q * (xcd + 1) / 8;
    if (nslots <= 0 || q1 <= q0) continue;
    load.assign((size_t)nslots, 0);
    for (int64_t q = q0; q < q1; ++q) load[(size_t)((q - q0) % nslots)] += steps[(size_t)(q / N)];
    for (int64_t v : load) worst = std::max(worst, v);
  }
  return worst;
}

struct TileRect { int tx, ty, wt, ht; };
static void cut_strip_pairs(const std::vector<TileRect>& take, int D, int h, std::vector<StripPair>& out) {
  out.clear();
  for (const TileRect& r : take) {
    const int X0 = 16 * r.tx, X1 = 16 * (r.tx + r.wt), Y0 = 16 * r.ty, Y1 = 16 * (r.ty + r.ht);
    const int ns = (X1 - X0 + SP_USE - 1) / SP_USE;
    const int H = Y1 - Y0, nseg = (H + h - 1) / h;
    for (int sg = 0; sg < nseg; ++sg) {
      const int ya = Y0 + (int)((int64_t)H * sg / nseg), yb = Y0 + (int)((int64_t)H * (sg + 1) / nseg);
      for (int s0 = 0; s0 < ns; s0 += 2) {
        StripPair p;
        for (int e = 0; e < 2; ++e) {
          const int s = s0 + e;
          if (s < ns) {
            p.x0[e] = X0 + SP_USE * s;
            p.w[e] = std::min(SP_USE, X1 - p.x0[e]);
          } else {
            p.x0[e] = p.x0[0];
// ... 540 lines not shown
      continue;
    }
    if (try_tables && em.run(g, t, D)) {
      (em.interior ? c.t_in : c.t_bd).add(t, em.row.data(), em.val.data());
      continue;
    }
    bool inner = false;
    if (!bfs_tile(g, t, D, WT, wide, b, &inner)) return false;
    (inner ? c.g_in : c.g_bd).push_back(t);
  }
  b.tile_off[g.ntiles] = (int32_t)b.region.size();
  return true;
}

static void merge_small_map(const Graph& g, int D, int num_cu, Embedding& em, Classes& c) {
  if ((c.r_in.empty() && c.r_bd.empty()) ||
      c.r_in.size() + c.r_bd.size() + c.t_in.tiles.size() + c.t_bd.tiles.size() > (size_t)SMALL_MAP_TILES)
    return;
  int64_t taken = 0;
  if (g.plan->opt.strips != 2) {
    std::vector<StripPair> p0, ip0;
    std::vector<int32_t> rest0, steps0;
    build_strips(c.r_in, D, num_cu, g.plan->opt, p0, rest0, &taken, steps0, ip0);
  }
  if (taken != 0) return;
  std::vector<int32_t> keep_i, keep_b;
  for (int pass = 0; pass < 2; ++pass)
    for (int32_t t : pass == 0 ? c.r_in : c.r_bd) {
      if (em.run(g, t, D)) (pass == 0 ? c.t_in : c.t_bd).add(t, em.row.data(), em.val.data());
      else (pass == 0 ? keep_i : keep_b).push_back(t);
    }
  c.r_in.swap(keep_i);
  c.r_bd.swap(keep_b);
}

static void pair_strips(const Graph& g, int D, int num_cu, bool full, const Classes& c, FusedTiles& ft, HostTables& h) {
  std::vector<int32_t> rest = c.r_in;
  ft.strip_forced = g.plan->opt.strips == 1;
  if (!full && D <= SP_DMAX && g.plan->opt.strips != 2)
    build_strips(c.r_in, D, num_cu, g.plan->opt, h.pairs, rest, &ft.n_strip_tiles, ft.strip_steps, h.ipairs);
  h.rrest = joined(std::move(rest), c.r_bd);
  ft.n_pairs = (int)h.pairs.size();
  ft.h_pairs = h.pairs;
  ft.n_ipairs = (int)h.ipairs.size();
  for (const StripPair& ip : h.ipairs) {
    ft.ipair_h.push_back(ip.y1 - ip.y0);
    ft.ipair_second.push_back(ip.w[1] > 0 ? 1 : 0);
  }
}

static QCand morton_cand(int32_t t, int ntiles) {
  QCand c{};
  c.tile = t; c.tix = -1; c.taken = false;
  const int tx = (int)st_compress((unsigned)t), ty = (int)st_compress((unsigned)t >> 1);
  for (int d = 0; d < 8; ++d) {
    const int nx = tx + ddx[d], ny = ty + ddy[d];
    const int64_t nt = nx < 0 || ny < 0 ? -1 : (int64_t)st_morton((unsigned)nx, (unsigned)ny);
    c.nbr[d] = nt >= 0 && nt < ntiles ? (int32_t)nt : -1;
  }
  return c;
}

static void quad_strips5(const Graph& g, int D, const Classes& c, FusedTiles& ft, HostTables& h) {
  std::vector<QCand> cands;
  cands.reserve(c.r_in.size() + c.t_in.tiles.size());
  for (int32_t t : c.r_in) cands.push_back(morton_cand(t, g.ntiles));
  const size_t n_rc = cands.size();
  const int32_t ragged = g.out_rows % FUSED_P != 0 ? g.ntiles - 1 : -1;
  auto beside_ragged = [&](const QCand& q) {
    if (ragged < 0) return false;
    if (q.tile == ragged) return true;
    for (int d = 0; d < 8; ++d)
      if (q.nbr[d] == ragged) return true;
    return false;
  };
  for (size_t i = 0; i < c.t_in.tiles.size(); ++i) {
    QCand q{};
    q.tile = c.t_in.tiles[i]; q.tix = (int32_t)i; q.taken = false;
    if (links_from_table(&c.t_in.rows[i * ST_CELLS], D, g.ntiles, q.nbr)) cands.push_back(q);
  }
  for (QCand& q : cands) q.barred = beside_ragged(q);
  build_qtstrips(cands, g.ntiles, D, ft.q5.h_strips, ft.q5.h_tab, &ft.q5.n_tiles);
  std::vector<int32_t> r_rest;
  std::vector<unsigned char> t_taken(c.t_in.tiles.size(), 0);
  for (size_t i = 0; i < cands.size(); ++i) {
    if (i < n_rc) { if (!cands[i].taken) r_rest.push_back(cands[i].tile); }
    else if (cands[i].taken) t_taken[(size_t)cands[i].tix] = 1;
  }
  h.qrrest = joined(std::move(r_rest), c.r_bd);
  TTabs t_rest;
  for (size_t i = 0; i < c.t_in.tiles.size(); ++i) {
    if (!t_taken[i]) {
      t_rest.add(c.t_in, i);
      continue;
    }
    const int blo = ST_DMAX - D + 1, bhi = ST_DMAX + ST_TILE - 1 + D - 1;
    for (int y = blo; y <= bhi; ++y)
      for (int x = blo; x <= bhi; ++x) {
        const size_t cell = i * ST_CELLS + st_cell_off((unsigned)x, (unsigned)y) / 64u;
        h.patch_rows.push_back(c.t_in.rows[cell]);
        h.patch_vals.insert(h.patch_vals.end(), c.t_in.vals.begin() + cell * ST_TABV, c.t_in.vals.begin() + cell * ST_TABV + 9);
      }
  }
  h.qt = joined(std::move(t_rest), c.t_bd);
}

static void quad_strips8(const Graph& g, int D, const std::vector<unsigned char>& cls8, FusedTiles& ft, HostTables& h) {
  std::vector<QCand> cands;
  for (int32_t t = 0; t < g.ntiles; ++t)
    if ((cls8[(size_t)t] & 3) == 3) cands.push_back(morton_cand(t, g.ntiles));
  build_qtstrips(cands, g.ntiles, D, ft.q8.h_strips, ft.q8.h_tab, &ft.q8.n_tiles);
  std::vector<unsigned char> took((size_t)g.ntiles, 0);
  for (const QCand& q : cands)
    if (q.taken) took[(size_t)q.tile] = 1;
  std::vector<int32_t> rest[2];
  for (size_t i = 0; i < h.part.v.size(); ++i)
    if (!took[(size_t)h.part.v[i]]) rest[i < (size_t)h.part.n_interior ? 0 : 1].push_back(h.part.v[i]);
  h.q8rest = joined(std::move(rest[0]), rest[1]);
}

static std::vector<int32_t> cat(std::initializer_list<const std::vector<int32_t>*> lists) {
  std::vector<int32_t> v;
  for (const std::vector<int32_t>* l : lists) v.insert(v.end(), l->begin(), l->end());
  return v;
}

static void complements(const Classes& c, const FusedTiles& ft, HostTables& h) {
  h.all = joined(cat({&c.r_in, &c.t_in.tiles, &c.g_in}), cat({&c.r_bd, &c.t_bd.tiles, &c.g_bd}));
  h.nonq.v = ft.q5.n_tiles == 0 ? cat({&c.r_in, &c.r_bd, &c.t_in.tiles, &c.t_bd.tiles, &h.part.v}) : cat({&h.qrrest.v, &h.qt.tiles, &h.part.v});
}

template <class T> static bool upload(FusedTiles& ft, T*& dst, std::vector<T>& v) {
  if (v.empty()) v.emplace_back();
  void* p = nullptr;
  if (hipMalloc(&p, v.size() * sizeof(T)) != hipSuccess) return false;
  ft.dev.push_back(p);
  dst = static_cast<T*>(p);
  return hipMemcpy(p, v.data(), v.size() * sizeof(T), hipMemcpyHostToDevice) == hipSuccess;
}
static bool upload(FusedTiles& ft, TileList& dst, HostList& h) {
  dst.n = (int)h.v.size();
  dst.n_interior = h.n_interior;
  return upload(ft, dst.d, h.v);
}
static bool upload(FusedTiles& ft, TileTables& dst, TTabs& h) {
  dst.tiles.n = (int)h.tiles.size();
  dst.tiles.n_interior = h.n_interior;
  return upload(ft, dst.tiles.d, h.tiles) && upload(ft, dst.d_row, h.rows) && upload(ft, dst.d_vals, h.vals);
}
static bool upload(FusedTiles& ft, QStripSet& s) {
  std::vector<QStrip> strips = s.h_strips;
  std::vector<int32_t> prefix(1, 0), tab = s.h_tab;
  for (const QStrip& q : strips) prefix.push_back(prefix.back() + (q.y1 - q.y0));
  s.n = (int)strips.size();
  s.tape_rows = prefix.back();
  tab.resize(tab.size() + 8, 0);
  return upload(ft, s.d_strips, strips) && upload(ft, s.d_prefix, prefix) && upload(ft, s.d_tab, tab);
}
static bool upload_tables(FusedTiles& ft, HostTables& h) {
  BfsTables& b = h.bfs;
  return upload(ft, ft.t, h.t) && upload(ft, ft.d_tile_off, b.tile_off) && upload(ft, ft.d_ring_end, b.ring_end) &&
         upload(ft, ft.d_ell_off, b.ell_off) && upload(ft, ft.d_region, b.region) && upload(ft, ft.d_lcols, b.lcols) &&
         upload(ft, ft.d_lvals, b.lvals) && upload(ft, ft.part, h.part) && upload(ft, ft.r, h.r) && upload(ft, ft.rrest, h.rrest) &&
         upload(ft, ft.nonq, h.nonq) && upload(ft, ft.all, h.all) && upload(ft, ft.d_pairs, h.pairs) && upload(ft, ft.q5) &&
         upload(ft, ft.q8) && upload(ft, ft.q8rest, h.q8rest) && upload(ft, ft.qrrest, h.qrrest) && upload(ft, ft.qt, h.qt) &&
         upload(ft, ft.d_ipairs, h.ipairs);
}

static bool build_tiles(const dsph_plan* plan, FusedPlan* fp, int D, bool full, FusedTiles& ft) {
  const int64_t out_rows = plan->levels.empty() ? plan->n_rows : plan->levels[0];
  const int64_t nt64 = (out_rows + FUSED_P - 1) / FUSED_P;
  if (D < 1 || D > FUSED_DMAX || nt64 > (1 << 30)) return false;
  const Graph g{plan, fp->h_cols.data(), fp->h_vals.data(), plan->width, out_rows, (int)nt64};
  std::vector<unsigned char> cls, cls8;
  classify(g, fp, D, full, cls, cls8);
  const bool try_tables = !full && D <= ST_DMAX && plan->opt.use_struct && plan->opt.use_tables && fp->d_rowflag != nullptr;
  Embedding em;
  Classes c;
  HostTables h;
  if (!sort_tiles(g, D, ft.width, fp->wide, cls, try_tables, em, c, h.bfs)) return false;
  ft.ntiles = g.ntiles;
  ft.rmax = std::max((h.bfs.rmax + 15) / 16 * 16, FUSED_P);
  ft.emax = h.bfs.emax;
  if (try_tables && D <= SP_DMAX) merge_small_map(g, D, fp->num_cu, em, c);
  h.part = joined(c.g_in, c.g_bd);
  pair_strips(g, D, fp->num_cu, full, c, ft, h);
  if (!full && D == QS_D && plan->opt.strips != 2 && plan->opt.strip_form == 0 && fp->d_gvals8 != nullptr)
    quad_strips5(g, D, c, ft, h);
  if (!cls8.empty()) quad_strips8(g, D, cls8, ft, h);
  complements(c, ft, h);
  h.r = joined(c.r_in, c.r_bd);
  h.t = joined(c.t_in, c.t_bd);
  bool good = upload_tables(ft, h);
  if (good && !h.patch_rows.empty())
    good = struct_patch_rows(plan, fp->d_gvals8, fp->d_gdiag, h.patch_rows.data(), h.patch_vals.data(), (int64_t)h.patch_rows.size()) == DSPH_OK;
  if (!good) {
    ft.release();
    ft.D = D;
  }
  return good;
}

const FusedTiles& get_tiles(const dsph_plan* plan, int D, bool full) {
  FusedPlan* fp = plan->fused;
  std::lock_guard<std::mutex> lock(fp->mu);
  DeviceGuard guard(plan->device);
  const int key = 2 * D + (full ? 1 : 0);
  auto it = fp->by_depth.find(key);
  if (it != fp->by_depth.end()) return it->second;
  static const FusedTiles none;
  if (fp->host_released || (fp->wide && !(D == 1 && full))) return none;
  FusedTiles& ft = fp->by_depth[key];
  ft.D = D;
  ft.width = fp->wide ? tstep_width(plan->width) : template_width(plan->width);
  ft.ok = build_tiles(plan, fp, D, full, ft);
  return ft;
}

bool fused_tile_counts(const dsph_plan* plan, int32_t K, int64_t* n_struct, int64_t* n_bfs) {
  if (!plan->fused || K < 2 || K - 1 > FUSED_DMAX) return false;
  const FusedTiles& ft = get_tiles(plan, K - 1, false);
  if (!ft.ok) return false;
  *n_struct = ft.r.n + ft.t.tiles.n;
  *n_bfs = ft.part.n;
  return true;
}

static const QStripSet* record_strips(const dsph_plan* plan, const FusedTiles& ft, int32_t K) {
  const QStripSet* s = K == 5 ? &ft.q5 : (K == Q8_K ? &ft.q8 : nullptr);
  return plan->opt.strip_form == 0 && s && !s->h_strips.empty() ? s : nullptr;
}

int64_t fused_strip_pairs(const dsph_plan* plan, int32_t K, int32_t* out, int64_t cap) {
  if (!plan->fused || K < 2 || K - 1 > FUSED_DMAX) return -1;
  const FusedTiles& ft = get_tiles(plan, K - 1, false);
  if (!ft.ok) return -1;
  static_assert(sizeof(StripPair) == 12 * sizeof(int32_t), "StripPair is twelve int32");
  if (const QStripSet* s = record_strips(plan, ft, K)) {
    const int64_t n = (int64_t)s->h_strips.size();
    for (int64_t i = 0; i < n && i < cap; ++i) {
      const QStrip& q = s->h_strips[(size_t)i];
      const int32_t rec[12] = {q.x0, q.x0, q.w, 0, q.xs, q.xs, q.y0, q.y1, q.xlo, q.xhi, q.ylo, q.yhi};
      memcpy(out + 12 * i, rec, sizeof(rec));
    }
    return n;
  }
  const int64_t n = (int64_t)ft.h_pairs.size();
  for (int64_t i = 0; i < n && i < cap; ++i) memcpy(out + 12 * i, &ft.h_pairs[(size_t)i], sizeof(StripPair));
  return n;
}

int64_t fused_strip_rows(const dsph_plan* plan, int32_t K, int64_t strip, int64_t n, const int32_t* xy, int64_t* rows) {
  if (!plan->fused || K < 2 || K - 1 > FUSED_DMAX) return -1;
  const FusedTiles& ft = get_tiles(plan, K - 1, false);
  if (!ft.ok || strip < 0) return -1;
  if (const QStripSet* s = record_strips(plan, ft, K)) {
    if (strip >= (int64_t)s->h_strips.size()) return -1;
    const QStrip& q = s->h_strips[(size_t)strip];
    const int ya = K == 5 ? q.ylo - 1 : q.ylo, yb = K == 5 ? q.yhi + 6 : q.yhi;
    for (int64_t i = 0; i < n; ++i) {
      const int x = std::min(std::max(xy[2 * i], q.xlo), q.xhi), y = std::min(std::max(xy[2 * i + 1], ya), yb);
      rows[i] = (int64_t)s->h_tab[(size_t)(q.tab + (y >> 4) * q.tws + (x >> 4))] + (int64_t)st_morton((unsigned)x & 15u, (unsigned)y & 15u);
    }
    return n;
  }
  if (strip >= (int64_t)ft.h_pairs.size()) return -1;
  for (int64_t i = 0; i < n; ++i) rows[i] = (int64_t)st_morton((unsigned)xy[2 * i], (unsigned)xy[2 * i + 1]);
  return n;
}

bool fused_strip_split(const dsph_plan* plan, int64_t N, int32_t* grid, int32_t* pieces, int32_t* wg_per_piece, int64_t* tape_rows) {
  if (!plan->fused || N < 1) return false;
  const FusedTiles& ft = get_tiles(plan, QS_D, false);
  if (!ft.ok || ft.q5.n == 0) return false;
  int g = 0, p = 0, w = 0;
  (void)qstrip_split(plan->fused->num_cu, ft.q5.tape_rows, N, ft.q5.tape_rows / std::max(1, ft.q5.n), &g, &p, &w);
  *grid = g; *pieces = p; *wg_per_piece = w; *tape_rows = ft.q5.tape_rows;
  return true;
}

bool fused_symmetric(const dsph_plan* plan) {
  FusedPlan* fp = plan->fused;
  std::lock_guard<std::mutex> lock(fp->mu);
  if (fp->symmetric >= 0) return fp->symmetric == 1;
  if (fp->host_released || plan->n_rows != plan->n_cols) return false;
  const int W = plan->width;
  const int64_t n = plan->n_rows;
  const int32_t* cols = fp->h_cols.data();
  const float* vals = fp->h_vals.data();
  bool sym = true;
  for (int64_t r = 0; r < n && sym; ++r)
    for (int j = 0; j < W; ++j) {
      const int64_t c = cols[r * W + j];
      const float v = vals[r * W + j];
      if (v == 0.f || c == r) continue;
      if (c < 0 || c >= n) { sym = false; break; }
      float back = 0.f;
      for (int i = 0; i < W; ++i)
        if (cols[c * W + i] == r) back += vals[c * W + i];
      if (fabsf(back - v) > 2.4e-7f * fmaxf(fabsf(back), fabsf(v))) { sym = false; break; }
    }
  fp->symmetric = sym ? 1 : 0;
  return sym;
}

}
```

deepsphere-cosmo-tf2_amd/csrc/dsphere_api.hip:

```cpp
#include <stdarg.h>
#include <stdio.h>
#include <string.h>

#include <new>

#include "dsphere_common.h"

namespace dsph {

static thread_local char g_err[512] = "";

void set_error(const char* fmt, ...) {
  va_list ap;
  va_start(ap, fmt);
  vsnprintf(g_err, sizeof(g_err), fmt, ap);
  va_end(ap);
}

int hip_fail(hipError_t e, const char* what) {
  set_error("HIP error %d (%s) in %s", (int)e, hipGetErrorString(e), what);
  return DSPH_E_HIP;
}

static size_t align_up(size_t v, size_t a) { return (v + a - 1) / a * a; }

static int64_t step_rows(const dsph_plan* p, int K, int k) {
  if (p->levels.empty()) return p->n_rows;
  const int lvl = K - 1 - k;
  const int last = (int)p->levels.size() - 1;
  return p->levels[lvl < last ? lvl : last];
}

struct Recurrence { float alpha_rest, beta_rest; };
static Recurrence recurrence_of(int32_t basis) {
  return basis == DSPH_BASIS_CHEBYSHEV ? Recurrence{2.f, 1.f} : Recurrence{1.f, 0.f};
}

}

using namespace dsph;

extern "C" {

int dsph_abi_version(void) { return DSPH_ABI_VERSION; }

const char* dsph_last_error(void) { return g_err; }

int dsph_plan_create(dsph_plan** out, int64_t n_rows, int64_t n_cols, int32_t ell_width,
                     const int32_t* cols, const float* vals, int device) {
  if (!out) { set_error("plan_create: out is NULL"); return DSPH_E_BADARG; }
  *out = nullptr;
  if (n_rows <= 0 || n_cols < n_rows || ell_width <= 0 || !cols || !vals) {
    set_error("plan_create: bad shape n_rows=%lld n_cols=%lld width=%d or NULL arrays",
              (long long)n_rows, (long long)n_cols, (int)ell_width);
    return DSPH_E_BADARG;
  }
  if (n_cols > 0x7fffffffLL) {
    set_error("plan_create: n_cols=%lld exceeds int32 column indices", (long long)n_cols);
    return DSPH_E_UNSUPPORTED;
  }
  const int64_t nnz = n_rows * (int64_t)ell_width;
  for (int64_t i = 0; i < nnz; ++i) {
    if (cols[i] < 0 || (int64_t)cols[i] >= n_cols) {
      set_error("plan_create: column %d at row %lld slot %lld outside [0, %lld)", (int)cols[i],
                (long long)(i / ell_width), (long long)(i % ell_width), (long long)n_cols);
      return DSPH_E_BADARG;
    }
  }
  int ndev = 0;
  DSPH_HIP(hipGetDeviceCount(&ndev));
  if (device < 0 || device >= ndev) {
    set_error("plan_create: device %d not in [0, %d)", device, ndev);
    return DSPH_E_BADARG;
  }
  DeviceGuard guard(device);
  if (!guard.ok) { set_error("plan_create: cannot select device %d", device); return DSPH_E_HIP; }
  dsph_plan* p = new (std::nothrow) dsph_plan();
  if (!p) { set_error("plan_create: out of host memory"); return DSPH_E_BADARG; }
  p->device = device;
  p->n_rows = n_rows;
  p->n_cols = n_cols;
  p->width = ell_width;
  hipError_t e = hipMalloc((void**)&p->d_cols, (size_t)nnz * sizeof(int32_t));
  if (e == hipSuccess) e = hipMalloc((void**)&p->d_vals, (size_t)nnz * sizeof(float));
  if (e == hipSuccess) e = hipMemcpy(p->d_cols, cols, (size_t)nnz * sizeof(int32_t), hipMemcpyHostToDevice);
  if (e == hipSuccess) e = hipMemcpy(p->d_vals, vals, (size_t)nnz * sizeof(float), hipMemcpyHostToDevice);
  if (e != hipSuccess) {
    dsph_plan_destroy(p);
    return hip_fail(e, "plan_create upload");
  }
  p->fused = fused_plan_build(p, cols, vals);
  *out = p;
  return DSPH_OK;
}

void dsph_plan_destroy(dsph_plan* p) {
  if (!p) return;
  DeviceGuard guard(p->device);
  if (p->fused) fused_plan_destroy(p->fused);
  if (p->d_cols) (void)hipFree(p->d_cols);
  if (p->d_vals) (void)hipFree(p->d_vals);
  delete p;
}

int dsph_plan_set_levels(dsph_plan* p, int32_t n_levels, const int64_t* rows_at_level) {
  if (!p || n_levels <= 0 || !rows_at_level) { set_error("set_levels: bad arguments"); return DSPH_E_BADARG; }
  int64_t prev = 0;
  for (int i = 0; i < n_levels; ++i) {
    if (rows_at_level[i] < prev || rows_at_level[i] > p->n_rows || rows_at_level[i] <= 0) {
      set_error("set_levels: level %d = %lld not in non-decreasing (0, %lld]", i,
                (long long)rows_at_level[i], (long long)p->n_rows);
      return DSPH_E_BADARG;
    }
    prev = rows_at_level[i];
  }
  if (p->fused && fused_host_released(p->fused)) {
    set_error("set_levels: the plan's host copy of L~ was released (DSPH_PREPARE_RELEASE_HOST); set the levels before preparing");
    return DSPH_E_UNSUPPORTED;
  }
  p->levels.assign(rows_at_level, rows_at_level + n_levels);
  if (p->fused) {
    DeviceGuard guard(p->device);
    fused_plan_invalidate(p->fused);
  }
  return DSPH_OK;
}

int dsph_plan_set_option(dsph_plan* p, int32_t option, int64_t value) {
  if (!p) { set_error("plan_set_option: plan is NULL"); return DSPH_E_BADARG; }
  PlanOptions o = p->opt;
  bool tables = true;
  switch (option) {
    case DSPH_OPT_STRIPS:
      if (value < 0 || value > 2) { set_error("plan_set_option: DSPH_OPT_STRIPS takes 0 (cost rule), 1 (always), 2 (never)"); return DSPH_E_BADARG; }
      o.strips = (int)value;
      break;
    case DSPH_OPT_STRUCT: o.use_struct = value != 0; break;
    case DSPH_OPT_TABLES: o.use_tables = value != 0; break;
    case DSPH_OPT_FORK: o.fork = value != 0; tables = false; break;
    case DSPH_OPT_STRIP_MINROWS:
      if (value < 4 || value > (1 << 20)) { set_error("plan_set_option: DSPH_OPT_STRIP_MINROWS takes tiles, at least 4"); return DSPH_E_BADARG; }
      o.strip_min_rows = (int)value;
      break;
    case DSPH_OPT_SPLIT:
      if (value < 0 || value > 2) { set_error("plan_set_option: DSPH_OPT_SPLIT takes 0 (automatic), 1 (always), 2 (never)"); return DSPH_E_BADARG; }
      o.split_order = (int)value;
      tables = false;
      break;
    case DSPH_OPT_TSTEP: o.tstep = value != 0; tables = false; break;
    case DSPH_OPT_PACK: o.pack = value != 0; tables = false; break;
    case DSPH_OPT_STRIP_FORM:
      if (value < 0 || value > 1) { set_error("plan_set_option: DSPH_OPT_STRIP_FORM takes 0 (quad strips) or 1 (strip pairs)"); return DSPH_E_BADARG; }
      o.strip_form = (int)value;
      break;
    case DSPH_OPT_F16_XEXP:
      if (value < -100 || value > 100) { set_error("plan_set_option: DSPH_OPT_F16_XEXP takes a binary exponent in [-100, 100]"); return DSPH_E_BADARG; }
      o.f16_xexp = (int)value;
      tables = false;
      break;
    default: set_error("plan_set_option: unknown option %d", (int)option); return DSPH_E_BADARG;
  }
  if (tables && p->fused) {
    if (fused_host_released(p->fused)) {
      set_error("plan_set_option: the plan's host copy of L~ was released (DSPH_PREPARE_RELEASE_HOST); set options before preparing");
      return DSPH_E_UNSUPPORTED;
    }
    DeviceGuard guard(p->device);
    fused_plan_invalidate(p->fused);
  }
  p->opt = o;
  return DSPH_OK;
}

int dsph_plan_strip_pairs(const dsph_plan* p, int32_t K, int32_t* out, int64_t capacity, int64_t* n_pairs) {
  if (!p || !n_pairs || capacity < 0 || (capacity > 0 && !out)) { set_error("plan_strip_pairs: bad arguments"); return DSPH_E_BADARG; }
  const int64_t n = fused_strip_pairs(p, K, out, capacity);
  if (n < 0) { *n_pairs = 0; set_error("plan_strip_pairs: the plan has no fused tables for K = %d", (int)K); return DSPH_E_UNSUPPORTED; }
  *n_pairs = n;
  return DSPH_OK;
}

int dsph_plan_strip_rows(const dsph_plan* p, int32_t K, int64_t strip, int64_t n, const int32_t* xy, int64_t* rows) {
  if (!p || n < 0 || (n > 0 && (!xy || !rows))) { set_error("plan_strip_rows: bad arguments"); return DSPH_E_BADARG; }
  DeviceGuard guard(p->device);
  if (fused_strip_rows(p, K, strip, n, xy, rows) < 0) { set_error("plan_strip_rows: no strip record %lld for K = %d", (long long)strip, (int)K); return DSPH_E_UNSUPPORTED; }
  return DSPH_OK;
}

static bool use_split(const dsph_plan* p, int32_t Fin, int32_t Fout, int32_t K, int32_t algo, int32_t part);

int dsph_plan_strip_split(const dsph_plan* p, int64_t N, int32_t* grid, int32_t* pieces, int32_t* wg_per_piece, int64_t* tape_rows) {
  if (!p || !grid || !pieces || !wg_per_piece || !tape_rows) { set_error("plan_strip_split: NULL argument"); return DSPH_E_BADARG; }
  *grid = *pieces = *wg_per_piece = 0;
  *tape_rows = 0;
  DeviceGuard guard(p->device);
  if (!fused_strip_split(p, N, grid, pieces, wg_per_piece, tape_rows)) { set_error("plan_strip_split: the plan holds no quad strips"); return DSPH_E_UNSUPPORTED; }
  return DSPH_OK;
}

int dsph_plan_prepare_layer(dsph_plan* p, int32_t K, int32_t Fin, int32_t Fout, int32_t flags) {
  if (!p || K <= 0 || Fin <= 0 || Fout <= 0 || (flags & ~(DSPH_PREPARE_BACKWARD | DSPH_PREPARE_RELEASE_HOST))) {
    set_error("plan_prepare: bad arguments (plan %p, K %d, Fin %d, Fout %d, flags %d)", (void*)p, K, Fin, Fout, flags);
    return DSPH_E_BADARG;
  }
  DeviceGuard guard(p->device);
  if (!guard.ok) { set_error("plan_prepare: cannot select device %d", p->device); return DSPH_E_HIP; }
  if (use_split(p, Fin, Fout, K, DSPH_ALGO_AUTO, DSPH_PART_ALL)) return split_prepare(p, K, Fin, Fout, flags);
  return fused_prepare(p, K, Fin, flags);
}

int dsph_plan_prepare(dsph_plan* p, int32_t K, int32_t Fin, int32_t flags) { return dsph_plan_prepare_layer(p, K, Fin, Fin, flags); }

static bool needs_levels(const dsph_plan* p, int32_t K) { return p->n_cols > p->n_rows && K > 2 && p->levels.empty(); }
static bool levels_ok(const dsph_plan* p, int32_t K, const char* who) {
  if (!p->levels.empty() && (int)p->levels.size() < K - 1) {
    set_error("%s: plan has %d levels, K = %d needs %d", who, (int)p->levels.size(), K, K - 1);
    return false;
  }
  if (needs_levels(p, K)) set_error("%s: the plan has halo columns and no levels: K = %d is not computable", who, K);
  return !needs_levels(p, K);
}

int64_t dsph_plan_rows(const dsph_plan* p) { return p ? p->n_rows : 0; }
int64_t dsph_plan_cols(const dsph_plan* p) { return p ? p->n_cols : 0; }
int32_t dsph_plan_ell_width(const dsph_plan* p) { return p ? p->width : 0; }
int64_t dsph_plan_out_rows(const dsph_plan* p, int32_t K) { (void)K; return p ? out_rows(p) : 0; }

int dsph_plan_fused_ok(const dsph_plan* p, int32_t Fin, int32_t Fout, int32_t K) {
  return (p && (fused_supported(p, Fin, Fout, K) || use_split(p, Fin, Fout, K, DSPH_ALGO_AUTO, DSPH_PART_ALL))) ? 1 : 0;
}

int dsph_plan_uses_chain(const dsph_plan* p, int32_t Fin, int32_t Fout, int32_t K) {
  return (p && Fin >= 1 && Fout >= 1 && use_split(p, Fin, Fout, K, DSPH_ALGO_AUTO, DSPH_PART_ALL)) ? 1 : 0;
}

int dsph_plan_tile_counts(const dsph_plan* p, int32_t K, int64_t* n_struct, int64_t* n_bfs) {
  if (!p || !n_struct || !n_bfs) { set_error("plan_tile_counts: NULL argument"); return DSPH_E_BADARG; }
  *n_struct = *n_bfs = 0;
  if (!fused_tile_counts(p, K, n_struct, n_bfs)) { set_error("plan_tile_counts: the fused kernels cannot run this plan with K = %d", K); return DSPH_E_UNSUPPORTED; }
  return DSPH_OK;
}

int dsph_plan_strip_tiles(const dsph_plan* p, int64_t N, int32_t Fin, int32_t Fout, int32_t K, int32_t precision, int64_t* n_tiles) {
  if (!p || !n_tiles) { set_error("plan_strip_tiles: NULL argument"); return DSPH_E_BADARG; }
  *n_tiles = fused_supported(p, Fin, Fout, K) ? fused_strip_tiles(p, N, Fin, Fout, K, precision) : 0;
  return DSPH_OK;
}

static bool use_split(const dsph_plan* p, int32_t Fin, int32_t Fout, int32_t K, int32_t algo, int32_t part) {
  if (K <= 5 || algo == DSPH_ALGO_UNFUSED || part != DSPH_PART_ALL || p->opt.split_order == 2) return false;
  if (p->opt.split_order == 0 && K - 1 <= fused_dmax() && fused_weights_resident(p, Fin, Fout, K)) return false;
  if (p->opt.split_order == 0 && K - 1 == fused_dmax() && fused_supported(p, Fin, Fout, K)) return false;
  return split_applicable(p, Fin, Fout, K);
}

static int resolve_algo(const dsph_plan* p, int32_t Fin, int32_t Fout, int32_t K, int32_t algo) {
  if (algo == DSPH_ALGO_UNFUSED) return DSPH_ALGO_UNFUSED;
  if (fused_supported(p, Fin, Fout, K)) return DSPH_ALGO_FUSED;
  return algo == DSPH_ALGO_FUSED ? -1 : DSPH_ALGO_UNFUSED;
}

int dsph_plan_pool_fusable(const dsph_plan* p, int64_t N, int32_t Fin, int32_t Fout, int32_t K, int32_t act) {
  if (!p || N <= 0 || Fin <= 0 || Fout <= 0 || K <= 0) return 0;
  DeviceGuard guard(p->device);
  return (!use_split(p, Fin, Fout, K, DSPH_ALGO_AUTO, DSPH_PART_ALL) && fused_pool_ok(p, N, Fin, Fout, K, act)) ? 1 : 0;
}

int dsph_poly_forward_pool(const dsph_plan* p, const float* x, const float* w, const float* bias, float* y_scratch,
                           float* y_pooled, int64_t N, int32_t Fin, int32_t Fout, int32_t K, int32_t basis, int32_t act,
                           int32_t precision, int32_t pool_type, int32_t flags, void* workspace, size_t workspace_bytes,
                           void* hip_stream) {
  if (flags & ~DSPH_FWD_KEEP_WEIGHTS) { set_error("poly_forward_pool: unknown flags %d", flags); return DSPH_E_BADARG; }
  if (basis != DSPH_BASIS_CHEBYSHEV && basis != DSPH_BASIS_MONOMIAL) { set_error("poly_forward_pool: unknown basis %d", basis); return DSPH_E_BADARG; }
  if (pool_type != DSPH_POOL_MAX && pool_type != DSPH_POOL_AVG) { set_error("poly_forward_pool: unknown pool type %d", pool_type); return DSPH_E_BADARG; }
  if (!p || !x || !w || !y_pooled || N <= 0 || Fin <= 0 || Fout <= 0 || K <= 0) {
    set_error("poly_forward_pool: bad arguments (NULL pointer or non-positive size)");
    return DSPH_E_BADARG;
  }
  if (precision < DSPH_PREC_FP32 || precision > DSPH_PREC_F16X3) { set_error("poly_forward_pool: unknown precision %d", precision); return DSPH_E_BADARG; }
  if (precision == DSPH_PREC_F16X3) precision = DSPH_PREC_BF16X6;
  if (!dsph_plan_pool_fusable(p, N, Fin, Fout, K, act)) {
    set_error("poly_forward_pool: no fused pooling for this plan / shape (dsph_plan_pool_fusable)");
    return DSPH_E_UNSUPPORTED;
  }
  const size_t need = dsph_workspace_bytes(p, N, Fin, Fout, K, precision, DSPH_ALGO_FUSED);
  if (need > 0 && (!workspace || workspace_bytes < need)) {
    set_error("poly_forward_pool: workspace %zu bytes, need %zu", workspace_bytes, need);
    return DSPH_E_WORKSPACE;
  }
  DeviceGuard guard(p->device);
  const FusedPool fp{y_pooled, pool_type == DSPH_POOL_MAX ? 1 : 2};
  const Recurrence rec = recurrence_of(basis);
  return launch_cheb_fused(p, x, w, bias, y_scratch, N, Fin, Fout, K, act, precision, rec.alpha_rest, rec.beta_rest, workspace, workspace_bytes,
                           (hipStream_t)hip_stream, DSPH_PART_ALL, (flags & DSPH_FWD_KEEP_WEIGHTS) != 0, &fp);
}

size_t dsph_workspace_bytes(const dsph_plan* p, int64_t N, int32_t Fin, int32_t Fout, int32_t K,
                            int32_t precision, int32_t algo) {
  if (!p || N <= 0 || Fin <= 0 || K <= 0) return 0;
  if (use_split(p, Fin, Fout, K, algo, DSPH_PART_ALL)) return split_workspace_bytes(p, N, Fin, Fout, K, precision);
  const int a = resolve_algo(p, Fin, Fout, K, algo);
  if (a == DSPH_ALGO_FUSED) return fused_workspace_bytes(p, N, Fin, Fout, K, precision);
  const size_t plane = align_up((size_t)N * (size_t)p->n_cols * (size_t)Fin * sizeof(float), 256);
  return plane * (size_t)(K > 1 ? K - 1 : 0);
}

int dsph_cheb_step(const dsph_plan* p, const float* in, const float* prev, float* out, int64_t N,
                   int32_t F, float alpha, float beta, int64_t rows, void* hip_stream) {
  if (!p || !in || !out || N < 0 || F <= 0) { set_error("cheb_step: bad arguments"); return DSPH_E_BADARG; }
  if (rows <= 0) rows = p->n_rows;
  if (rows > p->n_rows) { set_error("cheb_step: rows %lld > plan rows %lld", (long long)rows, (long long)p->n_rows); return DSPH_E_BADARG; }
  DeviceGuard guard(p->device);
  return launch_cheb_step(p, in, p->n_cols, prev, p->n_cols, out, p->n_cols, N, F, alpha, beta,
                          rows, (hipStream_t)hip_stream);
}

int dsph_cheb_contract(const float* const* planes, int64_t plane_rows, const float* w,
                       const float* bias, float* y, int64_t N, int64_t rows, int32_t Fin,
                       int32_t Fout, int32_t K, int32_t act, int32_t precision, int device,
                       void* hip_stream) {
  if (!planes || !w || !y || N < 0 || rows < 0 || rows > plane_rows || Fin <= 0 || Fout <= 0 || K <= 0) {
    set_error("cheb_contract: bad arguments");
    return DSPH_E_BADARG;
  }
  for (int k = 0; k < K; ++k)
    if (!planes[k]) { set_error("cheb_contract: plane %d is NULL", k); return DSPH_E_BADARG; }
  DeviceGuard guard(device);
  return launch_cheb_contract(planes, plane_rows, w, bias, y, N, rows, Fin, Fout, K, act,
                              precision == DSPH_PREC_F16X3 ? DSPH_PREC_BF16X6 : precision, (hipStream_t)hip_stream);
}

int dsph_cheb_forward(const dsph_plan* p, const float* x, const float* w, const float* bias,
                      float* y, int64_t N, int32_t Fin, int32_t Fout, int32_t K, int32_t act,
                      int32_t precision, int32_t algo, void* workspace, size_t workspace_bytes,
                      void* hip_stream) {
  return dsph_poly_forward(p, x, w, bias, y, N, Fin, Fout, K, DSPH_BASIS_CHEBYSHEV, act, precision, algo,
                           workspace, workspace_bytes, hip_stream);
}
// ... 240 lines not shown
```

deepsphere-cosmo-tf2_amd/csrc/dsphere_common.h:

```cpp
#pragma once

#include <hip/hip_runtime.h>
#include <stdint.h>

#include <vector>

#include "dsphere.h"

namespace dsph {

void set_error(const char* fmt, ...);
int hip_fail(hipError_t e, const char* what);

#define DSPH_HIP(call)                                           \
  do {                                                           \
    hipError_t e__ = (call);                                     \
    if (e__ != hipSuccess) return ::dsph::hip_fail(e__, #call);  \
  } while (0)

struct DeviceGuard {
  int prev = -1;
  bool ok = true;
  explicit DeviceGuard(int dev) {
    if (hipGetDevice(&prev) != hipSuccess) { ok = false; return; }
    if (prev != dev && hipSetDevice(dev) != hipSuccess) ok = false;
  }
  ~DeviceGuard() {
    if (prev >= 0) (void)hipSetDevice(prev);
  }
};

struct FusedPlan;

struct PlanOptions {
  int strips = 0;
  bool use_struct = true;
  bool use_tables = true;
  bool fork = true;
  int strip_min_rows = 4;
  int split_order = 0;
  bool tstep = true;
  int strip_form = 0;
  bool pack = true;
  int f16_xexp = 0;
};

}

struct dsph_plan {
  int device = 0;
  int64_t n_rows = 0;
  int64_t n_cols = 0;
  int32_t width = 0;
  int32_t* d_cols = nullptr;
  float* d_vals = nullptr;
  std::vector<int64_t> levels;
  dsph::PlanOptions opt;
  dsph::FusedPlan* fused = nullptr;
};

namespace dsph {

inline int64_t out_rows(const dsph_plan* p) { return p->levels.empty() ? p->n_rows : p->levels[0]; }
inline int32_t pad4(int32_t Fin) { return (Fin + 3) & ~3; }

int launch_cheb_step(const dsph_plan* plan, const float* in, int64_t in_rows, const float* prev,
                     int64_t prev_rows, float* out, int64_t out_rows, int64_t N, int32_t F,
                     float alpha, float beta, int64_t rows, hipStream_t stream);

int launch_cheb_contract(const float* const* planes, int64_t plane_rows, const float* w,
                         const float* bias, float* y, int64_t N, int64_t rows, int32_t Fin,
                         int32_t Fout, int32_t K, int32_t act, int32_t precision,
                         hipStream_t stream);

bool launch_cheb_tcontract(const float* const* planes, int64_t plane_rows, const float* w, const float* bias, float* y, int64_t N,
                           int64_t rows, int32_t Fin, int32_t Fout, int32_t K, int32_t act, int32_t precision, int num_cu,
                           hipStream_t stream, int* rc);

size_t wgrad_workspace_bytes(int64_t N, int64_t rows, int32_t Fin, int32_t Fout, int32_t K);
int launch_cheb_wgrad(const float* const* planes, int64_t plane_rows, const float* dy, float* dw,
                      int64_t N, int64_t rows, int32_t Fin, int32_t Fout, int32_t K, void* workspace,
                      size_t workspace_bytes, hipStream_t stream);

int launch_rows_pack(const float* src, int64_t src_rows, const int32_t* idx, int64_t n_idx,
                     float* buf, int64_t N, int32_t F, bool unpack, hipStream_t stream);

FusedPlan* fused_plan_build(const dsph_plan* plan, const int32_t* h_cols, const float* h_vals);
void fused_plan_destroy(FusedPlan* fp);
void fused_plan_invalidate(FusedPlan* fp);
bool fused_host_released(FusedPlan* fp);
int fused_prepare(const dsph_plan* plan, int32_t K, int32_t Fin, int32_t flags);
bool fused_supported(const dsph_plan* plan, int32_t Fin, int32_t Fout, int32_t K);
bool fused_weights_resident(const dsph_plan* plan, int32_t Fin, int32_t Fout, int32_t K);
bool fused_tile_counts(const dsph_plan* plan, int32_t K, int64_t* n_struct, int64_t* n_bfs);
int64_t fused_strip_tiles(const dsph_plan* plan, int64_t N, int32_t Fin, int32_t Fout, int32_t K, int32_t precision);
int64_t fused_strip_pairs(const dsph_plan* plan, int32_t K, int32_t* out, int64_t cap);
int64_t fused_strip_rows(const dsph_plan* plan, int32_t K, int64_t strip, int64_t n, const int32_t* xy, int64_t* rows);
bool fused_strip_split(const dsph_plan* plan, int64_t N, int32_t* grid, int32_t* pieces, int32_t* wg_per_piece, int64_t* tape_rows);
struct FusedPool {
  float* y;
  int32_t type;
};
bool fused_pool_ok(const dsph_plan* plan, int64_t N, int32_t Fin, int32_t Fout, int32_t K, int32_t act);
int launch_cheb_fused(const dsph_plan* plan, const float* x, const float* w, const float* bias,
                      float* y, int64_t N, int32_t Fin, int32_t Fout, int32_t K, int32_t act,
                      int32_t precision, float alpha_rest, float beta_rest, void* workspace,
                      size_t workspace_bytes, hipStream_t stream, int32_t part = 0, bool keep_weights = false,
                      const FusedPool* pool = nullptr);
bool fused_planes_supported(const dsph_plan* plan, int32_t Fin, int32_t K);
int launch_cheb_fused_planes(const dsph_plan* plan, const float* x, float* planes_out, int64_t N, int32_t Fin,
                             int32_t K, float alpha_rest, float beta_rest, hipStream_t stream);
bool fused_wgrad_supported(const dsph_plan* plan, int32_t Fin, int32_t Fout, int32_t K);
size_t fused_wgrad_workspace_bytes(const dsph_plan* plan, int32_t Fin, int32_t Fout, int32_t K);
int launch_fused_pad(const float* x, float* xp, int64_t rows, int32_t Fin, int32_t Fp, hipStream_t stream);
bool fused_qwgrad_applies(const dsph_plan* plan, int64_t N, int32_t Fin, int32_t Fout, int32_t K, int32_t precision);
size_t fused_qwgrad_workspace_bytes(const dsph_plan* plan);
int launch_cheb_fused_qwgrad(const dsph_plan* plan, const float* x, const float* dy, float* dw, int64_t N, int32_t Fin, int32_t Fout,
                             int32_t K, float alpha_rest, float beta_rest, void* workspace, size_t bfs_slab_bytes, hipStream_t stream);
int launch_cheb_fused_wgrad(const dsph_plan* plan, const float* x, const float* dy, float* dw, int64_t N,
                            int32_t Fin, int32_t Fout, int32_t K, int32_t precision, float alpha_rest, float beta_rest,
                            void* workspace, size_t workspace_bytes, hipStream_t stream, int32_t Fin_w = 0);
size_t fused_workspace_bytes(const dsph_plan* plan, int64_t N, int32_t Fin, int32_t Fout, int32_t K,
                             int32_t precision);
enum : uint32_t { IMG_BFS = 1, IMG_STRUCT = 2, IMG_STRIP = 4, IMG_ISTRIP = 8, IMG_QSTRIP = 16, IMG_SPLIT = 32, IMG_Q8 = 64 };
void fused_images_begin(const dsph_plan* plan, const void* ws, uint64_t key, bool keep);
bool fused_images_claim(const dsph_plan* plan, const void* ws, uint32_t bit);
void fused_images_forget(const dsph_plan* plan, const void* ws);
uint64_t fused_images_key(int32_t Fin, int32_t Fin_w, int32_t Fout, int32_t K, int32_t ld, int32_t precision, bool cheb, bool many, bool pack);

int fused_dmax();
bool split_applicable(const dsph_plan* plan, int32_t Fin, int32_t Fout, int32_t K);
size_t split_workspace_bytes(const dsph_plan* plan, int64_t N, int32_t Fin, int32_t Fout, int32_t K, int32_t precision);
int split_prepare(const dsph_plan* plan, int32_t K, int32_t Fin, int32_t Fout, int32_t flags);
int launch_split_forward(const dsph_plan* plan, const float* x, const float* w, const float* bias, float* y, int64_t N, int32_t Fin,
                         int32_t Fout, int32_t K, int32_t basis, int32_t act, int32_t precision, void* workspace,
                         size_t workspace_bytes, hipStream_t stream, bool keep_weights = false);

struct TStepTables {
  const int32_t* tile_off; const int32_t* ring_end; const int64_t* ell_off; const int32_t* region;
  const uint16_t* lcols; const float* lvals;
  int ntiles = 0, width = 0;
};
int tstep_width(int ell_width);
bool fused_tstep_tables(const dsph_plan* plan, TStepTables* out);
int launch_cheb_tstep(const TStepTables& tb, const float* in, const float* prev, float* out, int64_t rows, int64_t N, int32_t F, float alpha,
                      float beta, int num_cu, hipStream_t stream);
int fused_num_cu(const dsph_plan* plan);

struct LaunchBase {
  const float* x; const float* w; const float* bias; float* y;
  const float* gvals8; const float* gdiag;
  int64_t x_rows, y_rows, N;
  int32_t act, ld, num_cu;
  bool cheb;
  float* ypool = nullptr;
  int64_t ypool_rows = 0;
  int32_t pool = 0;
};

struct StructLaunch : LaunchBase {
  unsigned char* wfrag;
  const int32_t* tiles;
  int32_t ntiles, Fin, Fout, K, precision;
  int32_t Fin_w;
  const int32_t* tabrow = nullptr;
  const float* tabvals = nullptr;
  bool prep_weights = true;
  bool allow_pack = true;
};
int struct_build_rows(const dsph_plan* plan, float** gvals8, float** gdiag, unsigned char** flag);
int struct_patch_rows(const dsph_plan* plan, float* gvals8, float* gdiag, const int32_t* rows, const float* vals, int64_t n);
int struct_classify_tiles(const dsph_plan* plan, const unsigned char* d_flag, int ntiles, int D, int64_t out_rows,
                          unsigned char* h_cls, int dlimit = 4 );
bool struct_shape_ok(int32_t Fin, int32_t Fout, int32_t K);
size_t struct_wfrag_bytes(int32_t Fin, int32_t Fout, int32_t K);
int launch_cheb_struct(const StructLaunch& s, hipStream_t stream);
int launch_struct_act(float* y, int64_t rows, int32_t cols, int32_t ld, int32_t act, hipStream_t stream);
int launch_struct_act_tiles(float* y, const int32_t* d_tiles, int ntiles, int64_t N, int64_t y_rows, int32_t cols, int32_t ld,
                            int32_t act, hipStream_t stream);
int launch_residual_epilogue(float* y, const float* skip, int64_t n, float alpha, int32_t act, bool before, hipStream_t stream);

struct StripPair;
struct StripLaunch : LaunchBase {
  unsigned char* wimg;
  const StripPair* pairs;
  int32_t npairs, Fin, Fout, K, precision;
  bool prep_weights = true;
};
bool strip_shape_ok(int32_t Fin, int32_t Fout, int32_t K);
size_t strip_wimg_bytes(int32_t Fin, int32_t Fout, int32_t K);
int launch_cheb_strip(const StripLaunch& s, hipStream_t stream);

struct QStrip;
struct QTapeLaunch : LaunchBase {
  unsigned char* wimg;
  const QStrip* strips;
  const int32_t* tab = nullptr;
  const int32_t* prefix;
  int64_t tape_rows;
  int32_t nstrips;
  bool f16 = false;
  int f16_xexp = 0;
  bool prep_weights = true;
};
int64_t qtape_split(int num_cu, int64_t tape_rows, int64_t N, int64_t mean_height, int run_in, int* grid, int* pieces, int* wg_per_piece);

struct QStripLaunch : QTapeLaunch {
  int32_t Fin, Fout;
};
bool qstrip_shape_ok(int32_t Fin, int32_t Fout, int32_t K);
size_t qstrip_wimg_bytes();
int64_t qstrip_split(int num_cu, int64_t tape_rows, int64_t N, int64_t mean_height, int* grid, int* pieces, int* wg_per_piece);
int launch_cheb_qstrip(const QStripLaunch& s, hipStream_t stream);

struct QStrip8Launch : QTapeLaunch {
  int32_t ld_w;
};
bool qstrip8_shape_ok(int32_t Fin, int32_t Fout, int32_t K);
size_t qstrip8_wimg_bytes();
int64_t qstrip8_split(int num_cu, int64_t tape_rows, int64_t N, int64_t mean_height, int* grid, int* pieces, int* wg_per_piece);
int launch_cheb_qstrip8(const QStrip8Launch& s, hipStream_t stream);

struct QWgradLaunch {
  const float* x; const float* dy;
  float* dw;
  float* slabs;
  const QStrip* strips; const int32_t* prefix;
  const int32_t* tab = nullptr;
  int64_t tape_rows;
  const float* gvals8; const float* gdiag;
  int64_t x_rows, dy_rows, N;
  int32_t nstrips, lddy, lddw, num_cu;
  bool cheb;
  bool accumulate = false;
};
bool qwgrad_shape_ok(int32_t Fin, int32_t Fout, int32_t K);
size_t qwgrad_slab_bytes(int num_cu);
int launch_cheb_qwgrad(const QWgradLaunch& s, hipStream_t stream);

struct IStripLaunch : LaunchBase {
  unsigned char* wimg;
  const StripPair* pairs;
  int32_t npairs, Fin, Fin_w, Fout, K, precision;
  int32_t nseg = 1;
  bool prep_weights = true;
};
int istrip_segments(const std::vector<int32_t>& heights, const std::vector<unsigned char>& second, int64_t N, int num_cu, int D,
                    bool narrow);
bool istrip_narrow(int32_t Fin_w);
bool istrip_pairs(int32_t Fin_w, int32_t Fout);
bool istrip_shape_ok(int32_t Fin, int32_t K);
size_t istrip_wimg_bytes(int32_t K, int32_t precision);
int launch_cheb_istrip(const IStripLaunch& s, hipStream_t stream);

__device__ __forceinline__ float apply_act(float v, int act) {
  switch (act) {
    case DSPH_ACT_RELU: return v > 0.f ? v : 0.f;
    case DSPH_ACT_ELU: return v > 0.f ? v : expm1f(v);
    case DSPH_ACT_SIGMOID: return 1.f / (1.f + expf(-v));
    case DSPH_ACT_TANH: return tanhf(v);
    default: return v;
  }
}
__device__ __forceinline__ float act_grad(float z, int act) {
  switch (act) {
    case DSPH_ACT_RELU: return z > 0.f ? 1.f : 0.f;
    case DSPH_ACT_ELU: return z > 0.f ? 1.f : z + 1.f;
    case DSPH_ACT_SIGMOID: return z * (1.f - z);
    case DSPH_ACT_TANH: return 1.f - z * z;
    default: return 1.f;
  }
}

__device__ __forceinline__ unsigned xcd_remap(unsigned bid, unsigned nblk) {
  const unsigned q = nblk >> 3, r = nblk & 7u, xcd = bid & 7u, i = bid >> 3;
  return (xcd < r ? xcd * (q + 1) : r * (q + 1) + (xcd - r) * q) + i;
}

}
```

deepsphere-cosmo-tf2_amd/deepsphere/_native.py:

```python

import ctypes
import os

import numpy as np

_LIB_PATH = os.path.join(os.path.dirname(os.path.abspath(__file__)), "_lib", "libdsphere_hip.so")
_lib = None

OK = 0
ACT_NONE, ACT_RELU, ACT_ELU, ACT_SIGMOID, ACT_TANH = 0, 1, 2, 3, 4
PREC_FP32, PREC_BF16X3, PREC_BF16X6, PREC_F16X3 = 0, 1, 2, 3
ALGO_AUTO, ALGO_UNFUSED, ALGO_FUSED = 0, 1, 2
PART_ALL, PART_INTERIOR, PART_BOUNDARY = 0, 1, 2
FWD_KEEP_WEIGHTS = 1
ABI_VERSION = 3
POOL_MAX, POOL_AVG = 0, 1
PREPARE_BACKWARD, PREPARE_RELEASE_HOST = 1, 2
BASIS_CHEBYSHEV, BASIS_MONOMIAL = 0, 1
OPT_STRIPS, OPT_STRUCT, OPT_TABLES, OPT_FORK, OPT_STRIP_MINROWS, OPT_SPLIT, OPT_TSTEP = 1, 2, 3, 4, 6, 8, 9
OPT_PACK = 10
OPT_STRIP_FORM = 11
OPT_F16_XEXP = 12
STRIP_FORM_QUAD, STRIP_FORM_PAIRS = 0, 1
STRIPS_AUTO, STRIPS_ALWAYS, STRIPS_NEVER = 0, 1, 2
SPLIT_AUTO, SPLIT_ALWAYS, SPLIT_NEVER = 0, 1, 2

_c_i64 = ctypes.c_int64
_c_i32 = ctypes.c_int32
_c_vp = ctypes.c_void_p

SIGNATURES = {
    "dsph_abi_version": (ctypes.c_int, []),
    "dsph_last_error": (ctypes.c_char_p, []),
    "dsph_plan_create": (ctypes.c_int, [ctypes.POINTER(_c_vp), _c_i64, _c_i64, _c_i32, _c_vp, _c_vp, ctypes.c_int]),
    "dsph_plan_destroy": (None, [_c_vp]),
    "dsph_plan_set_levels": (ctypes.c_int, [_c_vp, _c_i32, _c_vp]),
    "dsph_plan_set_option": (ctypes.c_int, [_c_vp, _c_i32, _c_i64]),
    "dsph_plan_strip_pairs": (ctypes.c_int, [_c_vp, _c_i32, _c_vp, _c_i64, ctypes.POINTER(_c_i64)]),
    "dsph_plan_strip_split": (ctypes.c_int, [_c_vp, _c_i64, ctypes.POINTER(_c_i32), ctypes.POINTER(_c_i32), ctypes.POINTER(_c_i32),
                                             ctypes.POINTER(_c_i64)]),
    "dsph_plan_strip_rows": (ctypes.c_int, [_c_vp, _c_i32, _c_i64, _c_i64, _c_vp, _c_vp]),
    "dsph_plan_rows": (_c_i64, [_c_vp]),
    "dsph_plan_cols": (_c_i64, [_c_vp]),
    "dsph_plan_ell_width": (_c_i32, [_c_vp]),
    "dsph_plan_out_rows": (_c_i64, [_c_vp, _c_i32]),
    "dsph_plan_fused_ok": (ctypes.c_int, [_c_vp, _c_i32, _c_i32, _c_i32]),
    "dsph_plan_uses_chain": (ctypes.c_int, [_c_vp, _c_i32, _c_i32, _c_i32]),
    "dsph_plan_prepare": (ctypes.c_int, [_c_vp, _c_i32, _c_i32, _c_i32]),
    "dsph_plan_prepare_layer": (ctypes.c_int, [_c_vp, _c_i32, _c_i32, _c_i32, _c_i32]),
    "dsph_plan_tile_counts": (ctypes.c_int, [_c_vp, _c_i32, ctypes.POINTER(_c_i64), ctypes.POINTER(_c_i64)]),
    "dsph_plan_strip_tiles": (ctypes.c_int, [_c_vp, _c_i64, _c_i32, _c_i32, _c_i32, _c_i32, ctypes.POINTER(_c_i64)]),
    "dsph_workspace_bytes": (ctypes.c_size_t, [_c_vp, _c_i64, _c_i32, _c_i32, _c_i32, _c_i32, _c_i32]),
    "dsph_cheb_forward": (
        ctypes.c_int,
        [_c_vp, _c_vp, _c_vp, _c_vp, _c_vp, _c_i64, _c_i32, _c_i32, _c_i32, _c_i32, _c_i32, _c_i32, _c_vp,
         ctypes.c_size_t, _c_vp],
    ),
    "dsph_poly_forward": (
        ctypes.c_int,
        [_c_vp, _c_vp, _c_vp, _c_vp, _c_vp, _c_i64, _c_i32, _c_i32, _c_i32, _c_i32, _c_i32, _c_i32, _c_i32, _c_vp,
         ctypes.c_size_t, _c_vp],
    ),
    "dsph_poly_forward_part": (
        ctypes.c_int,
        [_c_vp, _c_vp, _c_vp, _c_vp, _c_vp, _c_i64, _c_i32, _c_i32, _c_i32, _c_i32, _c_i32, _c_i32, _c_i32, _c_i32,
         _c_vp, ctypes.c_size_t, _c_vp],
    ),
    "dsph_poly_forward_ex": (
        ctypes.c_int,
        [_c_vp, _c_vp, _c_vp, _c_vp, _c_vp, _c_i64, _c_i32, _c_i32, _c_i32, _c_i32, _c_i32, _c_i32, _c_i32, _c_i32, _c_i32,
         _c_vp, ctypes.c_size_t, _c_vp],
    ),
    "dsph_cheb_step": (
        ctypes.c_int,
        [_c_vp, _c_vp, _c_vp, _c_vp, _c_i64, _c_i32, ctypes.c_float, ctypes.c_float, _c_i64, _c_vp],
    ),
    "dsph_cheb_contract": (
        ctypes.c_int,
        [_c_vp, _c_i64, _c_vp, _c_vp, _c_vp, _c_i64, _c_i64, _c_i32, _c_i32, _c_i32, _c_i32, _c_i32, ctypes.c_int,
         _c_vp],
    ),
    "dsph_wgrad_workspace_bytes": (ctypes.c_size_t, [_c_i64, _c_i64, _c_i32, _c_i32, _c_i32]),
    "dsph_cheb_planes": (
        ctypes.c_int,
        [_c_vp, _c_vp, _c_vp, _c_i64, _c_i32, _c_i32, _c_i32, _c_i32, _c_vp],
    ),
    "dsph_backward_weights_workspace_bytes": (ctypes.c_size_t, [_c_vp, _c_i64, _c_i32, _c_i32, _c_i32, _c_i32]),
    "dsph_cheb_backward_weights": (
        ctypes.c_int,
        [_c_vp, _c_vp, _c_vp, _c_vp, _c_i64, _c_i32, _c_i32, _c_i32, _c_i32, _c_i32, _c_i32, _c_vp, ctypes.c_size_t,
         _c_vp],
    ),
    "dsph_cheb_wgrad": (
        ctypes.c_int,
        [_c_vp, _c_i64, _c_vp, _c_vp, _c_i64, _c_i64, _c_i32, _c_i32, _c_i32, _c_vp, ctypes.c_size_t, ctypes.c_int,
         _c_vp],
    ),
    "dsph_rows_pack": (ctypes.c_int, [_c_vp, _c_i64, _c_vp, _c_i64, _c_vp, _c_i64, _c_i32, ctypes.c_int, _c_vp]),
    "dsph_rows_unpack": (ctypes.c_int, [_c_vp, _c_i64, _c_vp, _c_i64, _c_vp, _c_i64, _c_i32, ctypes.c_int, _c_vp]),
    "dsph_plan_pool_fusable": (ctypes.c_int, [_c_vp, _c_i64, _c_i32, _c_i32, _c_i32, _c_i32]),
    "dsph_poly_forward_pool": (ctypes.c_int, [_c_vp, _c_vp, _c_vp, _c_vp, _c_vp, _c_vp, _c_i64, _c_i32, _c_i32, _c_i32, _c_i32, _c_i32,
                                               _c_i32, _c_i32, _c_i32, _c_vp, ctypes.c_size_t, _c_vp]),
    "dsph_healpix_pool": (ctypes.c_int, [_c_vp, _c_vp, _c_i64, _c_i64, _c_i32, _c_i32, _c_i32, ctypes.c_int, _c_vp]),
    "dsph_healpix_pool_backward": (ctypes.c_int, [_c_vp, _c_vp, _c_vp, _c_i64, _c_i64, _c_i32, _c_i32, _c_i32, ctypes.c_int, _c_vp]),
    "dsph_healpix_reorder": (ctypes.c_int, [_c_vp, _c_vp, _c_i64, _c_i32, _c_i32, _c_i32, ctypes.c_int, _c_vp]),
    "dsph_healpix_knn": (ctypes.c_int, [_c_i32, _c_i32, _c_vp, _c_vp, _c_i64, _c_vp, _c_vp, _c_vp, ctypes.c_int, _c_vp]),
    "dsph_healpix_disc_count": (ctypes.c_int, [_c_i32, ctypes.c_double, _c_vp, _c_vp, _c_i64, _c_vp, _c_vp, ctypes.c_int, _c_vp]),
    "dsph_healpix_gauss_table": (ctypes.c_int, [_c_i32, _c_i32, ctypes.c_double, ctypes.c_double, _c_vp, _c_vp, _c_i64, _c_vp, _c_vp, _c_vp, _c_vp,
                                                 ctypes.c_int, _c_vp]),
    "dsph_residual_epilogue": (ctypes.c_int, [_c_vp, _c_vp, _c_i64, ctypes.c_float, _c_i32, _c_i32, ctypes.c_int, _c_vp]),
    "dsph_nbr_attention_forward": (ctypes.c_int, [_c_vp, _c_vp, _c_vp, _c_i64, _c_vp, _c_vp, _c_vp, _c_i32, _c_i64, _c_i64, _c_i32, _c_i32,
                                                   ctypes.c_int, _c_vp]),
    "dsph_nbr_attention_backward": (ctypes.c_int, [_c_vp, _c_vp, _c_vp, _c_i64, _c_vp, _c_vp, _c_vp, _c_vp, _c_i32, _c_vp, _c_i32, _c_vp,
                                                    _c_vp, _c_vp, _c_vp, _c_i64, _c_i64, _c_i64, _c_i32, _c_i32, ctypes.c_int, _c_vp]),
    "dsph_dense_attention_forward": (ctypes.c_int, [_c_vp, _c_vp, _c_vp, _c_i64, _c_vp, _c_vp, _c_i64, _c_i64, _c_i32, _c_i32, ctypes.c_int,
                                                     _c_vp]),
    "dsph_dense_attention_backward": (ctypes.c_int, [_c_vp, _c_vp, _c_vp, _c_i64, _c_vp, _c_vp, _c_vp, _c_vp, _c_vp, _c_vp, _c_vp, _c_i64,
                                                      _c_i64, _c_i64, _c_i32, _c_i32, ctypes.c_int, _c_vp]),
    "dsph_dense_attention_forward_prec": (ctypes.c_int, [_c_vp, _c_vp, _c_vp, _c_i64, _c_vp, _c_vp, _c_i64, _c_i64, _c_i32, _c_i32,
                                                          _c_i32, ctypes.c_int, _c_vp]),
    "dsph_dense_attention_backward_prec": (ctypes.c_int, [_c_vp, _c_vp, _c_vp, _c_i64, _c_vp, _c_vp, _c_vp, _c_vp, _c_vp, _c_vp, _c_vp,
                                                           _c_i64, _c_i64, _c_i64, _c_i32, _c_i32, _c_i32, ctypes.c_int, _c_vp]),
    "dsph_dense_attention_forward_masked": (ctypes.c_int, [_c_vp, _c_vp, _c_vp, _c_i64, _c_vp, _c_vp, _c_vp, _c_i64, _c_i64, _c_i64, _c_i64,
                                                            _c_i64, _c_i32, _c_i32, _c_i32, ctypes.c_int, _c_vp]),
    "dsph_dense_attention_backward_masked": (ctypes.c_int, [_c_vp, _c_vp, _c_vp, _c_i64, _c_vp, _c_vp, _c_vp, _c_i64, _c_i64, _c_i64, _c_vp,
                                                             _c_vp, _c_vp, _c_vp, _c_vp, _c_i64, _c_i64, _c_i64, _c_i32, _c_i32, _c_i32,
                                                             ctypes.c_int, _c_vp]),
    "dsph_ell_smooth": (ctypes.c_int, [_c_vp, _c_vp, _c_i64, _c_i32, _c_vp, _c_vp, _c_i64, _c_i32, _c_vp, _c_i32, _c_vp, _c_i32,
                                        ctypes.c_int, _c_vp]),
    "dsph_basis_change": (ctypes.c_int, [_c_vp, _c_vp, _c_vp, _c_i32, _c_i32, _c_i32, _c_i32, ctypes.c_int, _c_vp]),
    "dsph_bn_workspace_bytes": (ctypes.c_size_t, [_c_i64, _c_i32]),
    "dsph_bn_stats": (ctypes.c_int, [_c_vp, _c_i64, _c_i32, ctypes.c_float, _c_vp, _c_vp, _c_vp, _c_vp, _c_vp, _c_vp, _c_vp, ctypes.c_float, _c_vp,
                                      ctypes.c_size_t, ctypes.c_int, _c_vp]),
    "dsph_bn_apply": (ctypes.c_int, [_c_vp, _c_vp, _c_i64, _c_i32, _c_vp, _c_vp, _c_vp, _c_vp, _c_i32, ctypes.c_int, _c_vp]),
    "dsph_bn_backward": (ctypes.c_int, [_c_vp, _c_vp, _c_vp, _c_vp, _c_vp, _c_vp, _c_vp, _c_vp, _c_vp, _c_vp, _c_vp, _c_i64, _c_i32, _c_i32, _c_vp,
                                         ctypes.c_size_t, ctypes.c_int, _c_vp]),
    "dsph_ln_workspace_bytes": (ctypes.c_size_t, [_c_i64, _c_i32]),
    "dsph_ln_forward": (ctypes.c_int, [_c_vp, _c_vp, _c_vp, _c_vp, _c_i64, _c_i32, ctypes.c_float, _c_vp, _c_vp, ctypes.c_int, _c_vp]),
    "dsph_ln_backward": (ctypes.c_int, [_c_vp, _c_vp, _c_vp, _c_vp, ctypes.c_float, _c_vp, _c_vp, _c_vp, _c_i64, _c_i32, _c_vp, ctypes.c_size_t,
                                         ctypes.c_int, _c_vp]),
    "dsph_patch_gemm": (ctypes.c_int, [_c_vp, _c_vp, _c_vp, _c_vp, _c_i64, _c_i32, _c_i32, _c_i32, _c_i32, _c_i32, ctypes.c_int, _c_vp]),
    "dsph_patch_backward_workspace_bytes": (ctypes.c_size_t, [_c_i64, _c_i32, _c_i32]),
    "dsph_patch_epilogue_backward": (ctypes.c_int, [_c_vp, _c_vp, _c_vp, _c_vp, _c_i64, _c_i32, _c_i32, _c_i32, _c_vp, ctypes.c_size_t, ctypes.c_int,
                                                    _c_vp]),
}


def library_path():
    return _LIB_PATH


def lib():
    global _lib
    if _lib is None:
        if not os.path.exists(_LIB_PATH):
            raise RuntimeError(
                f"HIP library not found at {_LIB_PATH}: build it with "
                "`make -C deepsphere-cosmo-tf2_amd/csrc` (there is no CPU fallback)"
            )
        handle = ctypes.CDLL(_LIB_PATH)
        for name, (res, args) in SIGNATURES.items():
            fn = getattr(handle, name)
            fn.restype = res
            fn.argtypes = args
        if handle.dsph_abi_version() != ABI_VERSION:
            raise RuntimeError("libdsphere_hip.so has an unexpected ABI version")
        _lib = handle
    return _lib


def last_error():
    msg = lib().dsph_last_error()
    return msg.decode("utf-8", "replace") if msg else ""


def check(rc, what):
    if rc == OK:
        return
    msg = f"{what} failed ({rc}): {last_error()}"
    if rc == -1:
        raise ValueError(msg)
    raise RuntimeError(msg)


def require_gpu():
    import torch

    if not torch.cuda.is_available():
        raise RuntimeError(
            "the Chebyshev forward runs only on a HIP device (MI355X); no GPU is visible and there is no CPU fallback"
        )


class LaplacianPlan:

    def __init__(self, ell_cols, ell_vals, n_cols=None, device=0, levels=None, options=None):
        cols = np.ascontiguousarray(ell_cols, dtype=np.int32)
        vals = np.ascontiguousarray(ell_vals, dtype=np.float32)
        if cols.ndim != 2 or cols.shape != vals.shape:
            raise ValueError("ELL cols/vals must be 2-D arrays of equal shape [rows, width]")
        self.n_rows, self.width = int(cols.shape[0]), int(cols.shape[1])
        self.n_cols = int(n_cols) if n_cols is not None else self.n_rows
        self.device = int(device)
        self._h = _c_vp()
        require_gpu()
        rc = lib().dsph_plan_create(
            ctypes.byref(self._h), self.n_rows, self.n_cols, self.width, cols.ctypes.data, vals.ctypes.data,
            self.device,
        )
        check(rc, "dsph_plan_create")
        self.levels = None
        if levels is not None:
            self.set_levels(levels)
        for opt, value in (options or {}).items():
            self.set_option(opt, value)

    def set_option(self, option, value):
        check(lib().dsph_plan_set_option(self.handle, int(option), int(value)), "dsph_plan_set_option")

    def set_levels(self, levels):
        lv = np.ascontiguousarray(levels, dtype=np.int64)
        check(lib().dsph_plan_set_levels(self._h, int(lv.shape[0]), lv.ctypes.data), "dsph_plan_set_levels")
        self.levels = lv.copy()

    @property
    def handle(self):
        if not self._h:
            raise RuntimeError("plan already destroyed")
        return self._h

    @property
    def out_rows(self):
        return int(lib().dsph_plan_out_rows(self.handle, 1))

    def fused_ok(self, Fin, Fout, K):
        return bool(lib().dsph_plan_fused_ok(self.handle, int(Fin), int(Fout), int(K)))

    def uses_chain(self, Fin, Fout, K):
        return bool(lib().dsph_plan_uses_chain(self.handle, int(Fin), int(Fout), int(K)))

    def prepare(self, K, Fin, backward=False, release_host=False, Fout=None):
        flags = (PREPARE_BACKWARD if backward else 0) | (PREPARE_RELEASE_HOST if release_host else 0)
        check(lib().dsph_plan_prepare_layer(self.handle, int(K), int(Fin), int(Fin if Fout is None else Fout), flags),
              "dsph_plan_prepare_layer")

    def tile_counts(self, K):
        a, b = _c_i64(0), _c_i64(0)
        check(lib().dsph_plan_tile_counts(self.handle, int(K), ctypes.byref(a), ctypes.byref(b)), "dsph_plan_tile_counts")
        return int(a.value), int(b.value)

    def strip_tiles(self, Fin, Fout, K, precision=PREC_BF16X3, N=1):
        n = _c_i64(0)
        check(lib().dsph_plan_strip_tiles(self.handle, int(N), int(Fin), int(Fout), int(K), int(precision), ctypes.byref(n)),
              "dsph_plan_strip_tiles")
        return int(n.value)

    def strip_pairs(self, K):
        n = _c_i64(0)
        check(lib().dsph_plan_strip_pairs(self.handle, int(K), _c_vp(), 0, ctypes.byref(n)), "dsph_plan_strip_pairs")
        out = np.zeros((int(n.value), 12), dtype=np.int32)
        if n.value:
            check(lib().dsph_plan_strip_pairs(self.handle, int(K), out.ctypes.data, int(n.value), ctypes.byref(n)),
                  "dsph_plan_strip_pairs")
        return out

    def strip_rows(self, K, strip, xs, ys):
        xy = np.ascontiguousarray(np.stack([np.asarray(xs), np.asarray(ys)], axis=1), dtype=np.int32)
        rows = np.zeros(xy.shape[0], dtype=np.int64)
        check(lib().dsph_plan_strip_rows(self.handle, int(K), int(strip), int(xy.shape[0]), xy.ctypes.data, rows.ctypes.data),
              "dsph_plan_strip_rows")
        return rows

    def strip_split(self, N):
        g, p, w, r = _c_i32(0), _c_i32(0), _c_i32(0), _c_i64(0)
        check(lib().dsph_plan_strip_split(self.handle, int(N), ctypes.byref(g), ctypes.byref(p), ctypes.byref(w), ctypes.byref(r)),
              "dsph_plan_strip_split")
        return int(g.value), int(p.value), int(w.value), int(r.value)

    def workspace_bytes(self, N, Fin, Fout, K, precision=PREC_FP32, algo=ALGO_AUTO):
        return int(lib().dsph_workspace_bytes(self.handle, int(N), int(Fin), int(Fout), int(K), int(precision),
                                              int(algo)))

    def close(self):
        if getattr(self, "_h", None):
            lib().dsph_plan_destroy(self._h)
            self._h = _c_vp()

    def __del__(self):
        try:
            self.close()
        except Exception:
            pass


def _ptr(t):
    return _c_vp(t.data_ptr()) if t is not None else _c_vp()


def _stream_ptr(device):
    import torch

    return _c_vp(torch.cuda.current_stream(device).cuda_stream)


def _check_dev(t, plan, name):
    import torch

    if not t.is_cuda or t.device.index != plan.device:
        raise ValueError(f"{name} must live on cuda:{plan.device}")
    if t.dtype != torch.float32 or not t.is_contiguous():
        raise ValueError(f"{name} must be a contiguous float32 tensor")


def _nbytes(t):
    return t.numel() * t.element_size()


def _ensure_workspace(need, device, workspace, floor=0, same_device=False):
    import torch

    if workspace is not None and _nbytes(workspace) >= need and (not same_device or workspace.device == device):
        return workspace, False
    return torch.empty(max(need, floor), dtype=torch.uint8, device=device), True


def cheb_forward(plan, x, w, bias, K, act=ACT_NONE, precision=PREC_FP32, algo=ALGO_AUTO, workspace=None, out=None,
                 basis=BASIS_CHEBYSHEV, part=PART_ALL, keep_weights=False):
    import torch

    _check_dev(x, plan, "x")
    _check_dev(w, plan, "w")
    N, rows, Fin = x.shape
    if rows != plan.n_cols:
        raise ValueError(f"x has {rows} rows, the plan multiplies vectors of {plan.n_cols} rows")
    if w.shape[0] != Fin * K:
        raise ValueError(f"w has {w.shape[0]} rows, expected Fin*K = {Fin * K}")
    Fout = int(w.shape[1])
    if bias is not None:
        _check_dev(bias, plan, "bias")
        if bias.numel() != Fout:
            raise ValueError("bias must have Fout elements")
    need = plan.workspace_bytes(N, Fin, Fout, K, precision, algo)
    if need > 0:
        workspace, replaced = _ensure_workspace(need, x.device, workspace)
        keep_weights = keep_weights and not replaced
    orows = plan.out_rows
    if out is None:
        out = torch.empty((N, orows, Fout), dtype=torch.float32, device=x.device)
    else:
        _check_dev(out, plan, "out")
        if tuple(out.shape) != (N, orows, Fout):
            raise ValueError("out has the wrong shape")
    rc = lib().dsph_poly_forward_ex(
        plan.handle, _ptr(x), _ptr(w), _ptr(bias), _ptr(out), int(N), int(Fin), Fout, int(K), int(basis), int(act),
        int(precision), int(algo), int(part), FWD_KEEP_WEIGHTS if (keep_weights and need > 0) else 0,
        _ptr(workspace) if need > 0 else _c_vp(),
        _nbytes(workspace) if need > 0 else 0, _stream_ptr(x.device),
    )
    check(rc, "dsph_poly_forward_ex")
    return out, workspace


def pool_fusable(plan, N, Fin, Fout, K, act=ACT_NONE):
    return bool(lib().dsph_plan_pool_fusable(plan.handle, int(N), int(Fin), int(Fout), int(K), int(act)))


def cheb_forward_pool(plan, x, w, bias, K, pool_type=POOL_MAX, act=ACT_NONE, precision=PREC_FP32, workspace=None,
                      basis=BASIS_CHEBYSHEV, keep_weights=False):
    import torch

    _check_dev(x, plan, "x")
    _check_dev(w, plan, "w")
    N, rows, Fin = x.shape
    Fout = int(w.shape[1])
    need = plan.workspace_bytes(N, Fin, Fout, K, precision, ALGO_FUSED)
    if need > 0:
        workspace, replaced = _ensure_workspace(need, x.device, workspace)
        keep_weights = keep_weights and not replaced
    out = torch.empty((N, rows // 4, Fout), dtype=torch.float32, device=x.device)
    rc = lib().dsph_poly_forward_pool(
        plan.handle, _ptr(x), _ptr(w), _ptr(bias), _c_vp(), _ptr(out), int(N), int(Fin), Fout, int(K), int(basis), int(act),
        int(precision), int(pool_type), FWD_KEEP_WEIGHTS if (keep_weights and need > 0) else 0,
        _ptr(workspace) if need > 0 else _c_vp(), _nbytes(workspace) if need > 0 else 0, _stream_ptr(x.device))
    check(rc, "dsph_poly_forward_pool")
    return out, workspace


def cheb_step(plan, inp, prev, alpha, beta, rows=0, out=None):
    import torch

    _check_dev(inp, plan, "in")
    N, r, F = inp.shape
    if r != plan.n_cols:
        raise ValueError("plane row count must equal the plan's n_cols")
    if prev is not None:
        _check_dev(prev, plan, "prev")
    if out is None:
        full = plan.n_cols == plan.n_rows and (rows <= 0 or rows == plan.n_rows)
        out = torch.empty_like(inp) if full else torch.zeros_like(inp)
    rc = lib().dsph_cheb_step(plan.handle, _ptr(inp), _ptr(prev), _ptr(out), int(N), int(F), float(alpha),
                              float(beta), int(rows), _stream_ptr(inp.device))
    check(rc, "dsph_cheb_step")
    return out


def cheb_contract(planes, w, bias, rows, K, act=ACT_NONE, precision=PREC_FP32):
    import torch

    p0 = planes[0]
    N, plane_rows, Fin = p0.shape
    Fout = int(w.shape[1])
    arr = (_c_vp * K)(*[p.data_ptr() for p in planes])
    out = torch.empty((N, rows, Fout), dtype=torch.float32, device=p0.device)
    rc = lib().dsph_cheb_contract(ctypes.cast(arr, _c_vp), int(plane_rows), _ptr(w), _ptr(bias), _ptr(out), int(N),
                                  int(rows), int(Fin), Fout, int(K), int(act), int(precision), p0.device.index,
                                  _stream_ptr(p0.device))
    check(rc, "dsph_cheb_contract")
    return out


def cheb_planes(plan, x, K, basis=BASIS_CHEBYSHEV, algo=ALGO_AUTO):
    import torch

    _check_dev(x, plan, "x")
    if x.dim() != 3 or x.shape[1] != plan.n_cols:
# ... 700 lines not shown
```

include/dsphere.h:

```cpp
#ifndef DSPHERE_H
#define DSPHERE_H

#include <stddef.h>
#include <stdint.h>

#ifdef __cplusplus
extern "C" {
#endif

#define DSPH_ABI_VERSION 3

#define DSPH_OK 0
#define DSPH_E_BADARG (-1)
#define DSPH_E_HIP (-2)
#define DSPH_E_UNSUPPORTED (-3)
#define DSPH_E_WORKSPACE (-4)

#define DSPH_ACT_NONE 0
#define DSPH_ACT_RELU 1
#define DSPH_ACT_ELU 2
#define DSPH_ACT_SIGMOID 3
#define DSPH_ACT_TANH 4

#define DSPH_PREC_FP32 0
#define DSPH_PREC_BF16X3 1
#define DSPH_PREC_BF16X6 2
#define DSPH_PREC_F16X3 3

#define DSPH_BASIS_CHEBYSHEV 0
#define DSPH_BASIS_MONOMIAL 1

#define DSPH_ALGO_AUTO 0
#define DSPH_ALGO_UNFUSED 1
#define DSPH_ALGO_FUSED 2

typedef struct dsph_plan dsph_plan;

int dsph_plan_create(dsph_plan** out, int64_t n_rows, int64_t n_cols, int32_t ell_width,
                     const int32_t* cols, const float* vals, int device);

void dsph_plan_destroy(dsph_plan* plan);

int dsph_plan_set_levels(dsph_plan* plan, int32_t n_levels, const int64_t* rows_at_level);

#define DSPH_PREPARE_BACKWARD 1
#define DSPH_PREPARE_RELEASE_HOST 2
int dsph_plan_prepare(dsph_plan* plan, int32_t K, int32_t Fin, int32_t flags);
int dsph_plan_prepare_layer(dsph_plan* plan, int32_t K, int32_t Fin, int32_t Fout, int32_t flags);

#define DSPH_OPT_STRIPS 1
#define DSPH_OPT_STRUCT 2
#define DSPH_OPT_TABLES 3
#define DSPH_OPT_FORK 4
#define DSPH_OPT_STRIP_MINROWS 6
#define DSPH_OPT_SPLIT 8
#define DSPH_OPT_TSTEP 9
#define DSPH_OPT_PACK 10
#define DSPH_OPT_STRIP_FORM 11
#define DSPH_OPT_F16_XEXP 12
int dsph_plan_set_option(dsph_plan* plan, int32_t option, int64_t value);

int64_t dsph_plan_rows(const dsph_plan* plan);
int64_t dsph_plan_cols(const dsph_plan* plan);
int32_t dsph_plan_ell_width(const dsph_plan* plan);
int64_t dsph_plan_out_rows(const dsph_plan* plan, int32_t K);
int dsph_plan_fused_ok(const dsph_plan* plan, int32_t Fin, int32_t Fout, int32_t K);
int dsph_plan_uses_chain(const dsph_plan* plan, int32_t Fin, int32_t Fout, int32_t K);

int dsph_plan_tile_counts(const dsph_plan* plan, int32_t K, int64_t* n_struct, int64_t* n_bfs);

int dsph_plan_strip_tiles(const dsph_plan* plan, int64_t N, int32_t Fin, int32_t Fout, int32_t K, int32_t precision,
                          int64_t* n_tiles);

int dsph_plan_strip_pairs(const dsph_plan* plan, int32_t K, int32_t* out, int64_t capacity, int64_t* n_pairs);
int dsph_plan_strip_split(const dsph_plan* plan, int64_t N, int32_t* grid, int32_t* pieces, int32_t* wg_per_piece, int64_t* tape_rows);
int dsph_plan_strip_rows(const dsph_plan* plan, int32_t K, int64_t strip, int64_t n, const int32_t* xy, int64_t* rows);

size_t dsph_workspace_bytes(const dsph_plan* plan, int64_t N, int32_t Fin, int32_t Fout,
                            int32_t K, int32_t precision, int32_t algo);

int dsph_cheb_forward(const dsph_plan* plan, const float* x, const float* w, const float* bias,
                      float* y, int64_t N, int32_t Fin, int32_t Fout, int32_t K, int32_t act,
                      int32_t precision, int32_t algo, void* workspace, size_t workspace_bytes,
                      void* hip_stream);

int dsph_poly_forward(const dsph_plan* plan, const float* x, const float* w, const float* bias,
                      float* y, int64_t N, int32_t Fin, int32_t Fout, int32_t K, int32_t basis,
                      int32_t act, int32_t precision, int32_t algo, void* workspace,
                      size_t workspace_bytes, void* hip_stream);

#define DSPH_PART_ALL 0
#define DSPH_PART_INTERIOR 1
#define DSPH_PART_BOUNDARY 2
int dsph_poly_forward_part(const dsph_plan* plan, const float* x, const float* w, const float* bias,
                           float* y, int64_t N, int32_t Fin, int32_t Fout, int32_t K, int32_t basis,
                           int32_t act, int32_t precision, int32_t algo, int32_t part, void* workspace,
                           size_t workspace_bytes, void* hip_stream);

#define DSPH_FWD_KEEP_WEIGHTS 1
int dsph_poly_forward_ex(const dsph_plan* plan, const float* x, const float* w, const float* bias,
                         float* y, int64_t N, int32_t Fin, int32_t Fout, int32_t K, int32_t basis,
                         int32_t act, int32_t precision, int32_t algo, int32_t part, int32_t flags, void* workspace,
                         size_t workspace_bytes, void* hip_stream);

int dsph_plan_pool_fusable(const dsph_plan* plan, int64_t N, int32_t Fin, int32_t Fout, int32_t K, int32_t act);
int dsph_poly_forward_pool(const dsph_plan* plan, const float* x, const float* w, const float* bias, float* y_scratch,
                           float* y_pooled, int64_t N, int32_t Fin, int32_t Fout, int32_t K, int32_t basis, int32_t act,
                           int32_t precision, int32_t pool_type, int32_t flags, void* workspace, size_t workspace_bytes,
                           void* hip_stream);

int dsph_cheb_step(const dsph_plan* plan, const float* in, const float* prev, float* out,
                   int64_t N, int32_t F, float alpha, float beta, int64_t rows, void* hip_stream);

int dsph_cheb_contract(const float* const* planes, int64_t plane_rows, const float* w,
                       const float* bias, float* y, int64_t N, int64_t rows, int32_t Fin,
                       int32_t Fout, int32_t K, int32_t act, int32_t precision, int device,
                       void* hip_stream);

int dsph_cheb_planes(const dsph_plan* plan, const float* x, float* planes, int64_t N, int32_t Fin,
                     int32_t K, int32_t basis, int32_t algo, void* hip_stream);

size_t dsph_backward_weights_workspace_bytes(const dsph_plan* plan, int64_t N, int32_t Fin, int32_t Fout,
                                             int32_t K, int32_t algo);
int dsph_cheb_backward_weights(const dsph_plan* plan, const float* x, const float* dy, float* dw, int64_t N,
                               int32_t Fin, int32_t Fout, int32_t K, int32_t basis, int32_t precision, int32_t algo,
                               void* workspace, size_t workspace_bytes, void* hip_stream);

size_t dsph_wgrad_workspace_bytes(int64_t N, int64_t rows, int32_t Fin, int32_t Fout, int32_t K);
int dsph_cheb_wgrad(const float* const* planes, int64_t plane_rows, const float* dy, float* dw,
                    int64_t N, int64_t rows, int32_t Fin, int32_t Fout, int32_t K, void* workspace,
                    size_t workspace_bytes, int device, void* hip_stream);

int dsph_rows_pack(const float* src, int64_t src_rows, const int32_t* idx, int64_t n_idx,
                   float* buf, int64_t N, int32_t F, int device, void* hip_stream);
int dsph_rows_unpack(float* dst, int64_t dst_rows, const int32_t* idx, int64_t n_idx,
                     const float* buf, int64_t N, int32_t F, int device, void* hip_stream);

int dsph_residual_epilogue(float* y, const float* skip, int64_t n, float alpha, int32_t act, int32_t act_before,
                           int device, void* hip_stream);

#define DSPH_POOL_MAX 0
#define DSPH_POOL_AVG 1
int dsph_healpix_pool(const float* x, float* y, int64_t N, int64_t rows_out, int32_t F, int32_t group, int32_t type, int device,
                      void* hip_stream);
int dsph_healpix_pool_backward(const float* x, const float* dy, float* dx, int64_t N, int64_t rows_out, int32_t F, int32_t group,
                               int32_t type, int device, void* hip_stream);

int dsph_healpix_reorder(const float* x, float* y, int64_t N, int32_t nside, int32_t F, int32_t to_nest, int device, void* hip_stream);

int dsph_healpix_knn(int32_t nside, int32_t k, const int64_t* indices, const int32_t* lut, int64_t M, int32_t* nbr, double* d2,
                     uint8_t* ok, int device, void* hip_stream);

int dsph_healpix_disc_count(int32_t nside, double r2, const int64_t* indices, const int32_t* lut, int64_t M, int32_t* count,
                            uint8_t* ok, int device, void* hip_stream);
int dsph_healpix_gauss_table(int32_t nside, int32_t W, double sigma_rad, double rho, const int64_t* indices, const int32_t* lut,
                             int64_t M, int32_t* cols, float* vals, float* raw, uint8_t* ok, int device, void* hip_stream);

int dsph_nbr_attention_forward(const float* q, const float* k, const float* v, int64_t ld, float* out, float* lse,
                               const int32_t* nbr, int32_t width, int64_t N, int64_t M, int32_t heads, int32_t depth, int device,
                               void* hip_stream);
int dsph_nbr_attention_backward(const float* q, const float* k, const float* v, int64_t ld, const float* out, const float* lse,
                                const float* dout, const int32_t* nbr, int32_t width, const int32_t* nbrT, int32_t widthT,
                                float* delta, float* dq, float* dk, float* dv, int64_t ld_grad, int64_t N, int64_t M, int32_t heads,
                                int32_t depth, int device, void* hip_stream);

int dsph_dense_attention_forward(const float* q, const float* k, const float* v, int64_t ld, float* out, float* lse, int64_t N,
                                 int64_t M, int32_t heads, int32_t depth, int device, void* hip_stream);
int dsph_dense_attention_backward(const float* q, const float* k, const float* v, int64_t ld, const float* out, const float* lse,
                                  const float* dout, float* delta, float* dq, float* dk, float* dv, int64_t ld_grad, int64_t N,
                                  int64_t M, int32_t heads, int32_t depth, int device, void* hip_stream);

int dsph_dense_attention_forward_prec(const float* q, const float* k, const float* v, int64_t ld, float* out, float* lse, int64_t N,
                                      int64_t M, int32_t heads, int32_t depth, int32_t precision, int device, void* hip_stream);
int dsph_dense_attention_backward_prec(const float* q, const float* k, const float* v, int64_t ld, const float* out, const float* lse,
                                       const float* dout, float* delta, float* dq, float* dk, float* dv, int64_t ld_grad, int64_t N,
                                       int64_t M, int32_t heads, int32_t depth, int32_t precision, int device, void* hip_stream);

int dsph_dense_attention_forward_masked(const float* q, const float* k, const float* v, int64_t ld, float* out, float* stat,
                                        const float* mask, int64_t mask_stride_batch, int64_t mask_stride_head,
                                        int64_t mask_stride_query, int64_t N, int64_t M, int32_t heads, int32_t depth,
                                        int32_t precision, int device, void* hip_stream);
int dsph_dense_attention_backward_masked(const float* q, const float* k, const float* v, int64_t ld, const float* out,
                                         const float* stat, const float* mask, int64_t mask_stride_batch, int64_t mask_stride_head,
                                         int64_t mask_stride_query, const float* dout, float* delta, float* dq, float* dk, float* dv,
                                         int64_t ld_grad, int64_t N, int64_t M, int32_t heads, int32_t depth, int32_t precision,
                                         int device, void* hip_stream);

int dsph_ell_smooth(const int32_t* cols, const float* vals, int64_t M, int32_t W, const float* x, float* y, int64_t N, int32_t C,
                    const int32_t* reps, int32_t pass, const float* mask, int32_t mask_C, int device, void* hip_stream);

int dsph_basis_change(const float* w, const float* coeff, float* w_out, int32_t Fin, int32_t Fout, int32_t Kp, int32_t transpose,
                      int device, void* hip_stream);

size_t dsph_bn_workspace_bytes(int64_t rows, int32_t F);
int dsph_bn_stats(const float* y, int64_t rows, int32_t F, float eps, float* mean, float* var, float* rstd, float* mean_lo, float* rstd_lo,
                  float* running_mean, float* running_var, float momentum, void* workspace, size_t workspace_bytes, int device, void* hip_stream);
int dsph_bn_apply(const float* y, float* z, int64_t rows, int32_t F, const float* mean, const float* rstd, const float* gamma,
                  const float* shift, int32_t act, int device, void* hip_stream);
int dsph_bn_backward(const float* y, const float* z, const float* dz, const float* mean, const float* rstd, const float* mean_lo,
                     const float* rstd_lo, const float* gamma, float* dy,
                     float* dgamma, float* dshift, int64_t rows, int32_t F, int32_t act, void* workspace, size_t workspace_bytes, int device,
                     void* hip_stream);

int dsph_ln_forward(const float* x, const float* res, float* sum, float* z, int64_t rows, int32_t d, float eps, const float* gamma,
                    const float* beta, int device, void* hip_stream);
size_t dsph_ln_workspace_bytes(int64_t rows, int32_t d);
int dsph_ln_backward(const float* a, const float* dz, const float* dsum, const float* gamma, float eps, float* da, float* dgamma,
                     float* dbeta, int64_t rows, int32_t d, void* workspace, size_t workspace_bytes, int device, void* hip_stream);

int dsph_patch_gemm(const float* x, const float* w, const float* bias, float* y, int64_t R, int32_t Kd, int32_t C, int32_t P, int32_t act,
                    int32_t precision, int device, void* hip_stream);
size_t dsph_patch_backward_workspace_bytes(int64_t R, int32_t C, int32_t P);
int dsph_patch_epilogue_backward(const float* y, const float* dy, float* dz, float* dbias, int64_t R, int32_t C, int32_t P, int32_t act,
                                 void* workspace, size_t workspace_bytes, int device, void* hip_stream);

const char* dsph_last_error(void);
int dsph_abi_version(void);

#ifdef __cplusplus
}
#endif
#endif
```

Measured before the change: 301,700.

## Precompute per-strip Laplacian coefficient image and stream it via direct-to-LDS DMA

Builds a one-time device image of the graph Laplacian coefficients laid out in strip row order, cached per plan for each basis. The quad-strip kernel then copies each coefficient row straight into LDS with global-to-LDS loads, replacing the per-row table gather, register staging and LDS store. This removes index translation and a register round trip from the inner step. In exchange it costs extra device memory and a synchronous build on first use, and it forces the X-by-H pixel mapping. It also adds an option to control the image and a debug API to read it back.

```diff
diff --git a/deepsphere-cosmo-tf2_amd/csrc/cheb_fused.hip b/deepsphere-cosmo-tf2_amd/csrc/cheb_fused.hip
--- a/deepsphere-cosmo-tf2_amd/csrc/cheb_fused.hip
+++ b/deepsphere-cosmo-tf2_amd/csrc/cheb_fused.hip
@@ -161,6 +161,7 @@
       std::lock_guard<std::mutex> lock(fp->fork_mu);
       (void)side_stream_ready(plan, fp, nullptr, true);
     }
+    if (ftp.ok && qstrip_shape_ok(Fin, 64, K) && plan->opt.strip_form == 0) (void)qstrip_cimage(plan, ftp, true, nullptr);
     if (flags & DSPH_PREPARE_BACKWARD) {
       (void)get_tiles(plan, K - 1, true);
       (void)fused_symmetric(plan);
@@ -426,6 +427,11 @@
     qs.nstrips = ft.q5.n; qs.Fin = rq.Fin; qs.Fout = rq.Fout;
     qs.f16 = rq.precision == DSPH_PREC_F16X3;
     qs.f16_xexp = plan->opt.f16_xexp;
+    qs.cimg = qstrip_cimage(plan, ft, base.cheb, rq.stream);
+    if (!qs.cimg && plan->opt.qstrip_image == 1 && ft.q5.cimg_failed) {
+      set_error("cheb_fused: DSPH_OPT_QSTRIP_IMAGE = on, and no memory for the image (%lld bytes)", (long long)ft.q5.cimg_rows * QS_CROWB);
+      return DSPH_E_HIP;
+    }
     qs.prep_weights = fused_images_claim(plan, rq.ws, IMG_QSTRIP);
     return launch_cheb_qstrip(qs, rq.stream);
   }
diff --git a/deepsphere-cosmo-tf2_amd/csrc/cheb_qstrip.hip b/deepsphere-cosmo-tf2_amd/csrc/cheb_qstrip.hip
--- a/deepsphere-cosmo-tf2_amd/csrc/cheb_qstrip.hip
+++ b/deepsphere-cosmo-tf2_amd/csrc/cheb_qstrip.hip
@@ -28,6 +28,36 @@
     const WfElem p = wf_elem16(e);
     wf_put(base, f16 ? WF_F16X3 : WF_BF16X3, p.l, p.j, have ? wf_gather(w, 32 * kb + p.inner, 16 * oq + p.col, Fin, Fout, K, j, ld, sc) : 0.f);
   }
+}
+
+__global__ __launch_bounds__(256) void qstrip_cimage_kernel(const QStrip* __restrict__ strips, int nstrips, const int32_t* __restrict__ tab,
+                                                            const float* __restrict__ gvals8, const float* __restrict__ gdiag,
+                                                            int64_t rows, int dbl, float* __restrict__ out) {
+  for (int64_t r = blockIdx.x; r < rows; r += gridDim.x) {
+    int lo = 0, hi = nstrips;
+    while (hi - lo > 1) {
+      const int mid = (lo + hi) >> 1;
+      if ((int64_t)strips[mid].img <= r) lo = mid; else hi = mid;
+    }
+    const QStrip st = strips[lo];
+    const int y = st.ylo - 1 + (int)(r - st.img);
+    for (int e = threadIdx.x; e < QS_CROWB / 4; e += 256) {
+      const int v = e >> 6, p = (e >> 2) & 15, t = e & 3;
+      const int x = min(max(st.xs + 4 * p + t, st.xlo), st.xhi);
+      const size_t rid = (size_t)tab[st.tab + (y >> 4) * st.tws + (x >> 4)] + st_morton((unsigned)x & 15u, (unsigned)y & 15u);
+      const float c = v == 0 ? gdiag[rid] : gvals8[rid * 8 + (size_t)(v - 1)];
+      out[r * (QS_CROWB / 4) + e] = dbl ? c + c : c;
+    }
+  }
+}
+int64_t qstrip_cimage_rows(const QStrip& q) { return (int64_t)q.yhi - q.ylo + 8; }
+int launch_qstrip_cimage(const QStrip* d_strips, int nstrips, const int32_t* d_tab, const float* gvals8, const float* gdiag, int64_t rows,
+                         bool doubled, float* d_out, hipStream_t stream) {
+  if (rows <= 0) return DSPH_OK;
+  hipLaunchKernelGGL(qstrip_cimage_kernel, dim3((unsigned)std::min<int64_t>(rows, 1 << 16)), dim3(256), 0, stream, d_strips, nstrips, d_tab,
+                     gvals8, gdiag, rows, doubled ? 1 : 0, d_out);
+  DSPH_HIP(hipGetLastError());
+  return DSPH_OK;
 }
 
 bool qstrip_shape_ok(int32_t Fin, int32_t Fout, int32_t K) { return K == 5 && Fin == 64 && Fout == 64; }
@@ -66,9 +96,13 @@
   QStripArgs a;
   a.Fin = s.Fin;
   a.Fout = s.Fout;
+  a.cimg = s.cimg;
   const int grid = qtape_forward_args(a, s, QS_RUNIN);
-  void (*kern)(QStripArgs) = s.f16 ? (s.cheb ? cheb_qstrip5_kernel<true, true> : cheb_qstrip5_kernel<false, true>)
-                                   : (s.cheb ? cheb_qstrip5_kernel<true, false> : cheb_qstrip5_kernel<false, false>);
+  void (*kern)(QStripArgs);
+  if (s.cimg) kern = s.f16 ? (s.cheb ? cheb_qstrip5_kernel<true, true, true> : cheb_qstrip5_kernel<false, true, true>)
+                           : (s.cheb ? cheb_qstrip5_kernel<true, false, true> : cheb_qstrip5_kernel<false, false, true>);
+  else kern = s.f16 ? (s.cheb ? cheb_qstrip5_kernel<true, true, false> : cheb_qstrip5_kernel<false, true, false>)
+                    : (s.cheb ? cheb_qstrip5_kernel<true, false, false> : cheb_qstrip5_kernel<false, false, false>);
 #ifdef DSPH_QS_STAMPS
   static unsigned* d_stamps = nullptr;
   constexpr size_t NST = 8 * 4 * 10;
diff --git a/deepsphere-cosmo-tf2_amd/csrc/cheb_qstrip_kernel.h b/deepsphere-cosmo-tf2_amd/csrc/cheb_qstrip_kernel.h
--- a/deepsphere-cosmo-tf2_amd/csrc/cheb_qstrip_kernel.h
+++ b/deepsphere-cosmo-tf2_amd/csrc/cheb_qstrip_kernel.h
@@ -19,6 +19,7 @@
   const unsigned char* wimg;
   const float* gvals8;
   const float* gdiag;
+  const float* cimg;
   const QStrip* strips;
   const int32_t* tab;
   const int32_t* prefix;
@@ -149,7 +150,7 @@
 
 __host__ __device__ constexpr float qs_wsign(bool cheb, int j) { return cheb && ((j & 3) >= 2) ? -1.f : 1.f; }
 
-template <bool CHEB, bool F16>
+template <bool CHEB, bool F16, bool CIMG>
 __global__ __launch_bounds__(QS_THREADS, 2) void cheb_qstrip5_kernel(QStripArgs a) {
   constexpr int K = 5, D = QS_D, RING = K + 2;
 #ifdef DSPH_QS_NOH1
@@ -191,7 +192,7 @@
 #elif defined(DSPH_QS_XBYH)
   constexpr bool X_BY_H = true;
 #else
-  constexpr bool X_BY_H = !H1;
+  constexpr bool X_BY_H = !H1 || CIMG;
 #endif
   constexpr int XN = X_BY_H ? 4 : 2;
   const int xt = wave & 3, xpix = X_BY_H ? ((lane >> 1) & 15) : (((lane >> 1) & 7) + 8 * (wave >> 2));
@@ -252,6 +253,10 @@
       for (int d = 0; d < 4; ++d) *reinterpret_cast<float*>(q + (unsigned)(1 + 4 * q4 + d) * 256u) = cv[d];
     }
     if (q4 == 2) *reinterpret_cast<float*>(q) = cd;
+  };
+  const unsigned c_voff = (unsigned)oq * (QS_CROWB / 4) + lane16;
+  auto cdma = [&](int slot, const unsigned char* crow) __attribute__((always_inline)) {
+    qt_cdma(crow, c_voff, __builtin_amdgcn_readfirstlane((unsigned)LDS_C + (unsigned)slot * QS_CROWB + (unsigned)oq * (QS_CROWB / 4)), lane);
   };
   constexpr bool C_OFF = (QS_ABL & 1024) != 0;
   auto clo_read = [&](int slot) __attribute__((always_inline)) -> QCoefLo { return qt_clo_read<C_OFF>(smem + LDS_C, slot, p); };
@@ -338,17 +343,22 @@
           for (int t = 0; t < 4; ++t) R[i][s].t[t] = qs_f4{0.f, 0.f, 0.f, 0.f};
       int ytop = st.y0 - D, slot_top = 0, cs_top = 0;
       qt_step_barrier();
+      const unsigned char* crow = CIMG ? reinterpret_cast<const unsigned char*>(a.cimg) + (size_t)(st.img + (ytop - st.ylo)) * QS_CROWB : nullptr;
       {
         qs_f4 cv, xv[XN];
         float cd;
-        cfetch(qt_row_in(st, tab_lane(st, ciC, ytop - 1), mXc, ytop - 1), cv, cd);
+        if (CIMG) { cdma(CRING - 1, crow); crow += QS_CROWB; }
+        else cfetch(qt_row_in(st, tab_lane(st, ciC, ytop - 1), mXc, ytop - 1), cv, cd);
         xfetch(xmap, qt_row_in(st, tab_lane(st, ciF, ytop), mXf, ytop), xv);
-        cw_wait(cv, cd);
-        cstore(CRING - 1, cv, cd);
+        if (!CIMG) {
+          cw_wait(cv, cd);
+          cstore(CRING - 1, cv, cd);
+        }
         xw_wait(xv);
         xstore(0, xv);
+        if (CIMG) qt_wait_vm();
       }
-      unsigned bXf = tab_lane(st, ciF, ytop + 1), bXc = tab_lane(st, ciC, ytop);
+      unsigned bXf = tab_lane(st, ciF, ytop + 1), bXc = CIMG ? 0u : tab_lane(st, ciC, ytop);
       unsigned myX = my_of(ytop + 1), myC = my_of(ytop);
       qt_step_barrier();
       auto step = [&](auto ph_c) __attribute__((always_inline)) {
@@ -369,9 +379,10 @@
         QS_STAMP_DECL
         QS_STAMP(0);
         qs_f4 xv[XN];
-        constexpr bool XLATE = H1;
+        constexpr bool XLATE = H1 && !X_BY_H;
         if (myX == 0) bXf = tab_lane(st, ciF, ytop + 1);
-        if (myC == 0) bXc = tab_lane(st, ciC, ytop);
+        if (!CIMG && myC == 0) bXc = tab_lane(st, ciC, ytop);
+        if (CIMG) { cdma(cs_top, crow); crow += QS_CROWB; }
         if (!XLATE) xfetch(xmap, bXf + (mXf | myX), xv);
         const unsigned f0 = (unsigned)slot_top * ROWB + lane16, f1 = (unsigned)slot_ix(1) * ROWB + lane16, f2 = (unsigned)slot_ix(2) * ROWB + lane16;
         const unsigned f3 = (unsigned)slot_ix(3) * ROWB + lane16;
@@ -394,7 +405,7 @@
         qs_settle<1>(R[0][L0]);
         if (XLATE) xfetch(xmap, bXf + (mXf | myX), xv);
         QS_STAMP(2);
-        QS_CHAIN(R[0][L0], false, 2, f2, QS_UPR, { c2h = chi_read(cslot_ix(2)); cfetch(bXc + (mXc | myC), cv, cd); if (H1) { QS_FR0(f3) } },
+        QS_CHAIN(R[0][L0], false, 2, f2, QS_UPR, { c2h = chi_read(cslot_ix(2)); if (!CIMG) cfetch(bXc + (mXc | myC), cv, cd); if (H1) { QS_FR0(f3) } },
                  { QS_UNIT<false, N3>(R[1][L2], R[0][L2], qq, QS_HI(c3h)); })
         qs_settle<9>(R[0][L0]);
         qs_settle<1>(R[1][L2]);
@@ -419,9 +430,10 @@
         ++handed;
         QS_STAMP(5);
         xw_wait(xv);
-        cw_wait(cv, cd);
+        if (CIMG) qt_wait_vm();
+        else cw_wait(cv, cd);
         QS_STAMP(6);
-        cstore(cs_top, cv, cd);
+        if (!CIMG) cstore(cs_top, cv, cd);
         xstore(snew, xv);
         QS_STAMP(7);
         slot_top = snew;
diff --git a/deepsphere-cosmo-tf2_amd/csrc/cheb_qtape.h b/deepsphere-cosmo-tf2_amd/csrc/cheb_qtape.h
--- a/deepsphere-cosmo-tf2_amd/csrc/cheb_qtape.h
+++ b/deepsphere-cosmo-tf2_amd/csrc/cheb_qtape.h
@@ -26,7 +26,7 @@
   int32_t xlo, xhi;
   int32_t ylo, yhi;
   int32_t tab, tws;
-  int32_t pad[1];
+  int32_t img;
 };
 
 struct QTapePiece {
@@ -59,7 +59,7 @@
   {
     const QStrip g = strips[lo];
 #define QS_U(f) st.f = __builtin_amdgcn_readfirstlane(g.f)
-    QS_U(x0); QS_U(w); QS_U(xs); QS_U(y0); QS_U(y1); QS_U(xlo); QS_U(xhi); QS_U(ylo); QS_U(yhi); QS_U(tab); QS_U(tws);
+    QS_U(x0); QS_U(w); QS_U(xs); QS_U(y0); QS_U(y1); QS_U(xlo); QS_U(xhi); QS_U(ylo); QS_U(yhi); QS_U(tab); QS_U(tws); QS_U(img);
 #undef QS_U
   }
   const int h = st.y1 - st.y0;
@@ -141,6 +141,10 @@
   }
   if (q4 == 2) *reinterpret_cast<float*>(q) = cd;
 }
+__device__ __forceinline__ void qt_cdma(const unsigned char* row, unsigned voff, unsigned lds_dst, int lane) {
+  if (lane < QS_CROWB / 4 / 16) st_glds16_off(row, voff, lds_dst);
+}
+__device__ __forceinline__ void qt_wait_vm() { asm volatile("s_waitcnt vmcnt(0)" ::: "memory"); }
 __device__ __forceinline__ const unsigned char* qt_crow(const unsigned char* ring, int slot, int p) {
   return ring + (unsigned)slot * QS_CROWB + (unsigned)p * 16u;
 }
diff --git a/deepsphere-cosmo-tf2_amd/csrc/cheb_tiles.h b/deepsphere-cosmo-tf2_amd/csrc/cheb_tiles.h
--- a/deepsphere-cosmo-tf2_amd/csrc/cheb_tiles.h
+++ b/deepsphere-cosmo-tf2_amd/csrc/cheb_tiles.h
@@ -38,6 +38,9 @@
   int64_t n_tiles = 0;
   std::vector<QStrip> h_strips;
   std::vector<int32_t> h_tab;
+  mutable float* d_cimg[2] = {nullptr, nullptr};
+  mutable bool cimg_failed = false;
+  int64_t cimg_rows = 0;
 };
 
 struct FusedTiles {
@@ -103,6 +106,7 @@
 };
 
 const FusedTiles& get_tiles(const dsph_plan* plan, int D, bool full = false);
+const float* qstrip_cimage(const dsph_plan* plan, const FusedTiles& ft, bool cheb, hipStream_t stream);
 bool fused_symmetric(const dsph_plan* plan);
 int64_t strip_makespan(const std::vector<int32_t>& steps, int64_t N, int num_cu);
 
diff --git a/deepsphere-cosmo-tf2_amd/csrc/cheb_tiles.hip b/deepsphere-cosmo-tf2_amd/csrc/cheb_tiles.hip
--- a/deepsphere-cosmo-tf2_amd/csrc/cheb_tiles.hip
+++ b/deepsphere-cosmo-tf2_amd/csrc/cheb_tiles.hip
@@ -17,8 +17,17 @@
   return 0;
 }
 
+static void cimage_free(const QStripSet& s) {
+  for (float*& p : s.d_cimg) {
+    if (p) (void)hipFree(p);
+    p = nullptr;
+  }
+  s.cimg_failed = false;
+}
+
 void FusedTiles::release() {
   for (void* p : dev) (void)hipFree(p);
+  cimage_free(q5);
   *this = FusedTiles();
 }
 
@@ -60,6 +69,37 @@
   std::lock_guard<std::mutex> lock(fp->mu);
   for (auto& kv : fp->by_depth) kv.second.release();
   fp->by_depth.clear();
+}
+
+void fused_cimage_drop(FusedPlan* fp) {
+  if (!fp) return;
+  std::lock_guard<std::mutex> lock(fp->mu);
+  for (auto& kv : fp->by_depth) cimage_free(kv.second.q5);
+}
+
+const float* qstrip_cimage(const dsph_plan* plan, const FusedTiles& ft, bool cheb, hipStream_t stream) {
+  const QStripSet& s = ft.q5;
+  if (plan->opt.qstrip_image == 2 || s.n == 0 || s.cimg_rows == 0) return nullptr;
+  FusedPlan* fp = plan->fused;
+  std::lock_guard<std::mutex> lock(fp->mu);
+  float*& img = s.d_cimg[cheb ? 1 : 0];
+  if (img || s.cimg_failed) return img;
+  hipStreamCaptureStatus cs = hipStreamCaptureStatusNone;
+  if (stream && (hipStreamIsCapturing(stream, &cs) != hipSuccess || cs != hipStreamCaptureStatusNone)) return nullptr;
+  void* p = nullptr;
+  if (hipMalloc(&p, (size_t)s.cimg_rows * QS_CROWB) != hipSuccess) {
+    (void)hipGetLastError();
+    s.cimg_failed = true;
+    return nullptr;
+  }
+  if (launch_qstrip_cimage(s.d_strips, s.n, s.d_tab, fp->d_gvals8, fp->d_gdiag, s.cimg_rows, cheb, static_cast<float*>(p), nullptr) != DSPH_OK ||
+      hipStreamSynchronize(nullptr) != hipSuccess) {
+    (void)hipFree(p);
+    s.cimg_failed = true;
+    return nullptr;
+  }
+  img = static_cast<float*>(p);
+  return img;
 }
 
 static bool embed_tile(const dsph_plan* plan, const int32_t* cols, const float* vals, int W, int t, int D, int64_t out_rows,
@@ -906,6 +946,13 @@
   std::vector<QStrip> strips = s.h_strips;
   std::vector<int32_t> prefix(1, 0), tab = s.h_tab;
   for (const QStrip& q : strips) prefix.push_back(prefix.back() + (q.y1 - q.y0));
+  int64_t img_rows = 0;
+  for (size_t i = 0; i < strips.size(); ++i) {
+    if (img_rows + qstrip_cimage_rows(strips[i]) > INT32_MAX) { img_rows = 0; break; }
+    strips[i].img = s.h_strips[i].img = (int32_t)img_rows;
+    img_rows += qstrip_cimage_rows(strips[i]);
+  }
+  s.cimg_rows = img_rows;
   s.n = (int)strips.size();
   s.tape_rows = prefix.back();
   tab.resize(tab.size() + 8, 0);
@@ -1023,6 +1070,20 @@
   return n;
 }
 
+int64_t fused_strip_image(const dsph_plan* plan, int32_t basis, int64_t strip, float* out, int64_t cap) {
+  if (!plan->fused) return -1;
+  const FusedTiles& ft = get_tiles(plan, QS_D, false);
+  const QStripSet* s = ft.ok ? record_strips(plan, ft, 5) : nullptr;
+  if (!s || strip < 0 || strip >= (int64_t)s->h_strips.size()) return -1;
+  const float* img = qstrip_cimage(plan, ft, basis == DSPH_BASIS_CHEBYSHEV, nullptr);
+  if (!img) return -1;
+  const QStrip& q = s->h_strips[(size_t)strip];
+  const int64_t n = qstrip_cimage_rows(q) * (QS_CROWB / 4);
+  if (q.img < 0 || (int64_t)q.img + qstrip_cimage_rows(q) > s->cimg_rows) return -1;
+  if (n <= cap && hipMemcpy(out, img + (int64_t)q.img * (QS_CROWB / 4), (size_t)n * 4, hipMemcpyDeviceToHost) != hipSuccess) return -1;
+  return n;
+}
+
 bool fused_strip_split(const dsph_plan* plan, int64_t N, int32_t* grid, int32_t* pieces, int32_t* wg_per_piece, int64_t* tape_rows) {
   if (!plan->fused || N < 1) return false;
   const FusedTiles& ft = get_tiles(plan, QS_D, false);
diff --git a/deepsphere-cosmo-tf2_amd/csrc/dsphere_api.hip b/deepsphere-cosmo-tf2_amd/csrc/dsphere_api.hip
--- a/deepsphere-cosmo-tf2_amd/csrc/dsphere_api.hip
+++ b/deepsphere-cosmo-tf2_amd/csrc/dsphere_api.hip
@@ -158,6 +158,15 @@
       o.f16_xexp = (int)value;
       tables = false;
       break;
+    case DSPH_OPT_QSTRIP_IMAGE:
+      if (value < 0 || value > 2) { set_error("plan_set_option: DSPH_OPT_QSTRIP_IMAGE takes 0 (automatic), 1 (on), 2 (off)"); return DSPH_E_BADARG; }
+      o.qstrip_image = (int)value;
+      tables = false;
+      if (p->fused && o.qstrip_image != p->opt.qstrip_image) {
+        DeviceGuard guard(p->device);
+        fused_cimage_drop(p->fused);
+      }
+      break;
     default: set_error("plan_set_option: unknown option %d", (int)option); return DSPH_E_BADARG;
   }
   if (tables && p->fused) {
@@ -184,6 +193,18 @@
   if (!p || n < 0 || (n > 0 && (!xy || !rows))) { set_error("plan_strip_rows: bad arguments"); return DSPH_E_BADARG; }
   DeviceGuard guard(p->device);
   if (fused_strip_rows(p, K, strip, n, xy, rows) < 0) { set_error("plan_strip_rows: no strip record %lld for K = %d", (long long)strip, (int)K); return DSPH_E_UNSUPPORTED; }
+  return DSPH_OK;
+}
+
+int dsph_plan_strip_image(const dsph_plan* p, int32_t basis, int64_t strip, float* out, int64_t capacity, int64_t* n_floats) {
+  if (!p || !n_floats || capacity < 0 || (capacity > 0 && !out) || (basis != DSPH_BASIS_CHEBYSHEV && basis != DSPH_BASIS_MONOMIAL)) {
+    set_error("plan_strip_image: bad arguments");
+    return DSPH_E_BADARG;
+  }
+  DeviceGuard guard(p->device);
+  const int64_t n = fused_strip_image(p, basis, strip, out, capacity);
+  if (n < 0) { *n_floats = 0; set_error("plan_strip_image: no image of L~ for strip record %lld (no K = 5 quad strips, or DSPH_OPT_QSTRIP_IMAGE off)", (long long)strip); return DSPH_E_UNSUPPORTED; }
+  *n_floats = n;
   return DSPH_OK;
 }
 
diff --git a/deepsphere-cosmo-tf2_amd/csrc/dsphere_common.h b/deepsphere-cosmo-tf2_amd/csrc/dsphere_common.h
--- a/deepsphere-cosmo-tf2_amd/csrc/dsphere_common.h
+++ b/deepsphere-cosmo-tf2_amd/csrc/dsphere_common.h
@@ -43,6 +43,7 @@
   int strip_form = 0;
   bool pack = true;
   int f16_xexp = 0;
+  int qstrip_image = 0;
 };
 
 }
@@ -97,6 +98,8 @@
 int64_t fused_strip_pairs(const dsph_plan* plan, int32_t K, int32_t* out, int64_t cap);
 int64_t fused_strip_rows(const dsph_plan* plan, int32_t K, int64_t strip, int64_t n, const int32_t* xy, int64_t* rows);
 bool fused_strip_split(const dsph_plan* plan, int64_t N, int32_t* grid, int32_t* pieces, int32_t* wg_per_piece, int64_t* tape_rows);
+int64_t fused_strip_image(const dsph_plan* plan, int32_t basis, int64_t strip, float* out, int64_t cap);
+void fused_cimage_drop(FusedPlan* fp);
 struct FusedPool {
   float* y;
   int32_t type;
@@ -207,7 +210,11 @@
 
 struct QStripLaunch : QTapeLaunch {
   int32_t Fin, Fout;
-};
+  const float* cimg = nullptr;
+};
+int64_t qstrip_cimage_rows(const QStrip& q);
+int launch_qstrip_cimage(const QStrip* d_strips, int nstrips, const int32_t* d_tab, const float* gvals8, const float* gdiag, int64_t rows,
+                         bool doubled, float* d_out, hipStream_t stream);
 bool qstrip_shape_ok(int32_t Fin, int32_t Fout, int32_t K);
 size_t qstrip_wimg_bytes();
 int64_t qstrip_split(int num_cu, int64_t tape_rows, int64_t N, int64_t mean_height, int* grid, int* pieces, int* wg_per_piece);
diff --git a/deepsphere-cosmo-tf2_amd/deepsphere/_native.py b/deepsphere-cosmo-tf2_amd/deepsphere/_native.py
--- a/deepsphere-cosmo-tf2_amd/deepsphere/_native.py
+++ b/deepsphere-cosmo-tf2_amd/deepsphere/_native.py
@@ -21,6 +21,7 @@
 OPT_PACK = 10
 OPT_STRIP_FORM = 11
 OPT_F16_XEXP = 12
+OPT_QSTRIP_IMAGE = 13
 STRIP_FORM_QUAD, STRIP_FORM_PAIRS = 0, 1
 STRIPS_AUTO, STRIPS_ALWAYS, STRIPS_NEVER = 0, 1, 2
 SPLIT_AUTO, SPLIT_ALWAYS, SPLIT_NEVER = 0, 1, 2
@@ -40,6 +41,7 @@
     "dsph_plan_strip_split": (ctypes.c_int, [_c_vp, _c_i64, ctypes.POINTER(_c_i32), ctypes.POINTER(_c_i32), ctypes.POINTER(_c_i32),
                                              ctypes.POINTER(_c_i64)]),
     "dsph_plan_strip_rows": (ctypes.c_int, [_c_vp, _c_i32, _c_i64, _c_i64, _c_vp, _c_vp]),
+    "dsph_plan_strip_image": (ctypes.c_int, [_c_vp, _c_i32, _c_i64, _c_vp, _c_i64, ctypes.POINTER(_c_i64)]),
     "dsph_plan_rows": (_c_i64, [_c_vp]),
     "dsph_plan_cols": (_c_i64, [_c_vp]),
     "dsph_plan_ell_width": (_c_i32, [_c_vp]),
@@ -271,6 +273,14 @@
               "dsph_plan_strip_rows")
         return rows
 
+    def strip_image(self, strip, basis=0):
+        n = _c_i64(0)
+        check(lib().dsph_plan_strip_image(self.handle, int(basis), int(strip), _c_vp(), 0, ctypes.byref(n)), "dsph_plan_strip_image")
+        out = np.zeros(int(n.value), np.float32)
+        check(lib().dsph_plan_strip_image(self.handle, int(basis), int(strip), out.ctypes.data, int(n.value), ctypes.byref(n)),
+              "dsph_plan_strip_image")
+        return out.reshape(-1, 9, 16, 4)
+
     def strip_split(self, N):
         g, p, w, r = _c_i32(0), _c_i32(0), _c_i32(0), _c_i64(0)
         check(lib().dsph_plan_strip_split(self.handle, int(N), ctypes.byref(g), ctypes.byref(p), ctypes.byref(w), ctypes.byref(r)),
diff --git a/include/dsphere.h b/include/dsphere.h
--- a/include/dsphere.h
+++ b/include/dsphere.h
@@ -58,6 +58,7 @@
 #define DSPH_OPT_PACK 10
 #define DSPH_OPT_STRIP_FORM 11
 #define DSPH_OPT_F16_XEXP 12
+#define DSPH_OPT_QSTRIP_IMAGE 13
 int dsph_plan_set_option(dsph_plan* plan, int32_t option, int64_t value);
 
 int64_t dsph_plan_rows(const dsph_plan* plan);
@@ -75,6 +76,7 @@
 int dsph_plan_strip_pairs(const dsph_plan* plan, int32_t K, int32_t* out, int64_t capacity, int64_t* n_pairs);
 int dsph_plan_strip_split(const dsph_plan* plan, int64_t N, int32_t* grid, int32_t* pieces, int32_t* wg_per_piece, int64_t* tape_rows);
 int dsph_plan_strip_rows(const dsph_plan* plan, int32_t K, int64_t strip, int64_t n, const int32_t* xy, int64_t* rows);
+int dsph_plan_strip_image(const dsph_plan* plan, int32_t basis, int64_t strip, float* out, int64_t capacity, int64_t* n_floats);
 
 size_t dsph_workspace_bytes(const dsph_plan* plan, int64_t N, int32_t Fin, int32_t Fout,
                             int32_t K, int32_t precision, int32_t algo);
```

Result: faster. 307,300 (median of 6 runs) (+1.8%).
